# Oscar-W-Chen/gpu-ai-inference-server

Hardware: AMD Instinct MI355X
Metric: images/sec, DenseNet-121 fp32, batch 32 per GPU, device-resident inputs (higher is better)
Workload: dtype f32; 1 GPU; DenseNet-121 fp32 batch=32 per GPU, synthetic 3x224x224 inputs (BASELINE configs[1]); synthetic ONNX graph + seeded random weights (reference model file is not in the mount); global_batch=32, per_gpu_batch=32, parallelism=dp1 (independent batch shards)

## Files before the change

gpu-ai-inference-server_amd/build.py:

```python
from __future__ import annotations

import os
import shutil
import subprocess
import sys
from concurrent.futures import ThreadPoolExecutor

PKG = os.path.dirname(os.path.abspath(__file__))
ROOT = os.path.dirname(PKG)
CSRC = os.path.join(PKG, "csrc")
OBJ = os.path.join(PKG, "lib", "obj")
LIB = os.path.join(PKG, "lib", "libinference_engine.so")
HIPCC = os.environ.get("HIPCC", "/opt/rocm/bin/hipcc")
ARCH = "gfx950"

SOURCES = ["env.cpp", "onnx_reader.cpp", "plan.cpp", "repository.cpp", "config.cpp", "executor.cpp", "bridge.cpp", "bridge_load.cpp", "bridge_run.cpp", "kernels.hip", "kernels_f16.hip", "kernels_ws.hip", "kernels_ws32.hip", "kernels_stem.hip", "kernels_direct.hip", "kernels_f8.hip", "kernels_fused.hip", "kernels_wino.hip", "kernels_x6.hip", "kernels_block.hip", "kernels_ws8.hip", "kernels_dw.hip", "kernels_se.hip", "kernels_grouped.hip", "kernels_resize.hip", "kernels_convt.hip", "kernels_ln.hip", "kernels_attn.hip", "kernels_tokens.hip"]
COMMON = ["-std=c++17", "-O3", "-fPIC", "-Wall", "-Wextra", "-Wno-unused-parameter", "-Wno-unused-result",
          "-I" + os.path.join(ROOT, "include"), "-I" + CSRC]


def _deps(src: str) -> list[str]:
    d = [os.path.join(CSRC, src)]
    for f in os.listdir(CSRC):
        if f.endswith(".h"):
            d.append(os.path.join(CSRC, f))
    for f in os.listdir(os.path.join(ROOT, "include")):
        d.append(os.path.join(ROOT, "include", f))
    return d


def _stale(target: str, deps: list[str]) -> bool:
    if not os.path.exists(target):
        return True
    t = os.path.getmtime(target)
    return any(os.path.getmtime(d) > t for d in deps)


def _compile(src: str, force: bool) -> str:
    obj = os.path.join(OBJ, src + ".o")
    if force or _stale(obj, _deps(src)):
        cmd = [HIPCC, *COMMON, "-c", os.path.join(CSRC, src), "-o", obj]
        if src.endswith(".hip"):
            cmd[1:1] = ["--offload-arch=" + ARCH, "-mllvm", "-amdgpu-mfma-vgpr-form=1"]
        r = subprocess.run(cmd, capture_output=True, text=True)
        if r.returncode != 0:
            raise RuntimeError(f"hipcc failed for {src}:\n{r.stdout}\n{r.stderr}")
        if r.stderr.strip():
            sys.stderr.write(r.stderr)
    return obj


def build_library(force: bool = False) -> str:
    os.makedirs(OBJ, exist_ok=True)
    with ThreadPoolExecutor(max_workers=4) as ex:
        objs = list(ex.map(lambda s: _compile(s, force), SOURCES))
    if force or _stale(LIB, objs):
        cmd = [HIPCC, "--offload-arch=" + ARCH, "-shared", "-fPIC", *objs, "-o", LIB, "-lstdc++fs", "-lpthread",
               "-L/opt/rocm/lib", "-lrccl", "-Wl,-rpath,/opt/rocm/lib"]
        r = subprocess.run(cmd, capture_output=True, text=True)
        if r.returncode != 0:
            raise RuntimeError(f"link failed:\n{r.stdout}\n{r.stderr}")
        for d in (os.path.join(ROOT, "build", "inference_engine"), os.path.join(ROOT, "build", "inference_engine", "lib")):
            os.makedirs(d, exist_ok=True)
            shutil.copy2(LIB, os.path.join(d, "libinference_engine.so"))
    return LIB


def build_harness() -> str:
    src = os.path.join(CSRC, "harness", "replay_binding.c")
    out = os.path.join(PKG, "lib", "replay_binding")
    if _stale(out, [src, LIB, os.path.join(ROOT, "include", "inference_bridge.h")]):
        cmd = ["gcc", "-std=c11", "-O2", "-Wall", "-Wextra", "-I" + os.path.join(ROOT, "include"), src, "-o", out,
               "-L" + os.path.dirname(LIB), "-linference_engine", "-Wl,-rpath," + os.path.dirname(LIB), "-lm"]
        r = subprocess.run(cmd, capture_output=True, text=True)
        if r.returncode != 0:
            raise RuntimeError(f"harness build failed:\n{r.stdout}\n{r.stderr}")
    return out


if __name__ == "__main__":
    print(build_library("--force" in sys.argv))
    if os.path.exists(os.path.join(CSRC, "harness", "replay_binding.c")):
        print(build_harness())
```

gpu-ai-inference-server_amd/csrc/bridge.cpp:

```cpp
#include "bridge_internal.h"

static_assert(sizeof(Shape) == 16, "Shape layout");
static_assert(sizeof(TensorData) == 48 && offsetof(TensorData, data) == 32 && offsetof(TensorData, data_size) == 40, "TensorData layout");
static_assert(sizeof(ModelConfig) == 64 && offsetof(ModelConfig, dynamic_batching) == 56, "ModelConfig layout");
static_assert(sizeof(ModelMetadata) == 72 && offsetof(ModelMetadata, load_time_ns) == 64, "ModelMetadata layout");
static_assert(sizeof(ModelStats) == 32, "ModelStats layout");
static_assert(sizeof(CudaMemoryInfo) == 24, "CudaMemoryInfo layout");

using namespace ie_bridge;

extern "C" {

bool IsCudaAvailable(void) { return ie::HipDeviceCount() > 0; }
int GetDeviceCount(void) { return ie::HipDeviceCount(); }
const char* GetDeviceInfo(int device_id) {
    try { return dup_cstr(ie::HipDeviceInfo(device_id)); } catch (...) { return dup_cstr("Unknown device"); }
}
CudaMemoryInfo GetMemoryInfo(int device_id) {
    CudaMemoryInfo m{0, 0, 0};
    size_t total = 0, fr = 0;
    if (ie::HipMemoryInfo(device_id, &total, &fr)) { m.total = total; m.free = fr; m.used = total - fr; }
    return m;
}

// ... 138 lines not shown
bool ModelUnload(ModelHandle handle, ErrorMessage* error) {
    if (!handle) { set_error(error, "Invalid model handle"); return false; }
    try { handle->model->Unload(); return true; }
    catch (const std::exception& e) { set_error(error, e.what()); return false; }
    catch (...) { set_error(error, "unknown error"); return false; }
}

bool ModelIsLoaded(ModelHandle handle) {
    if (!handle) return false;
    try { return handle->model->loaded.load(); } catch (...) { return false; }
}

bool ModelInfer(ModelHandle handle, const TensorData* inputs, int num_inputs, TensorData* outputs, int num_outputs,
                ErrorMessage* error) {
    if (!handle) { set_error(error, "Invalid model handle"); return false; }
    ModelObj& M = *handle->model;
    if (!M.loaded.load()) { set_error(error, "Model not loaded"); return false; }
    if (!inputs || num_inputs <= 0 || !outputs || num_outputs <= 0) { set_error(error, "Invalid parameters"); return false; }
    try {
        ModelObj::Pending req;
        bool batched = false;
        {
            std::shared_lock<std::shared_mutex> g(M.life);
            if (!M.loaded.load() || M.lanes.empty()) { set_error(error, "Model not loaded"); return false; }
            auto failv = [&](const std::string& msg) { M.SetError(msg); set_error(error, msg); return false; };
            const auto& gin = M.info.inputs;
            if (size_t(num_inputs) != gin.size())
                return failv("Expected " + std::to_string(gin.size()) + " inputs, got " + std::to_string(num_inputs));
            for (int i = 0; i < num_inputs; ++i) {
                const std::string nm = inputs[i].name ? inputs[i].name : "";
                bool known = false;
                for (auto& vi : gin) if (vi.name == nm) known = true;
                if (!known) return failv("Unexpected input name: " + nm);
            }
            req.in_ptr.assign(gin.size(), nullptr);
            req.in_bytes.assign(gin.size(), 0);
            req.in_u8.assign(gin.size(), 0);
            req.shapes.assign(gin.size(), {});
            req.outputs = outputs;
            req.num_outputs = num_outputs;
            std::vector<char> provided(gin.size(), 0);
            for (int i = 0; i < num_inputs && req.err.empty(); ++i) {
                const TensorData& t = inputs[i];
                const std::string nm = t.name ? t.name : "";
                for (size_t k = 0; k < gin.size(); ++k) {
                    if (gin[k].name != nm) continue;
                    if (t.data_type != DATATYPE_FLOAT32 && t.data_type != DATATYPE_UINT8) { req.err = "Unsupported data type for input: " + nm; break; }
                    req.in_u8[k] = t.data_type == DATATYPE_UINT8 ? 1 : 0;
                    provided[k] = 1;
                    req.shapes[k].clear();
                    if (t.shape.dims && t.shape.num_dims > 0) req.shapes[k].assign(t.shape.dims, t.shape.dims + t.shape.num_dims);
                    req.in_ptr[k] = (t.data && t.data_size > 0) ? t.data : nullptr;
                    req.in_bytes[k] = req.in_ptr[k] ? t.data_size : 0;
                }
            }
            for (size_t k = 0; k < gin.size() && req.err.empty(); ++k)
                if (!provided[k]) req.err = "Required input tensor not provided: " + gin[k].name;
            batched = req.err.empty() && M.batchable && M.max_batch > 1;
            if (batched) {
                req.rows = req.shapes[0].empty() ? 0 : req.shapes[0][0];
                for (size_t k = 0; k < gin.size(); ++k)
                    if (req.shapes[k].size() != gin[k].dims.size() || req.shapes[k][0] != req.rows) batched = false;
                if (req.rows <= 0 || req.rows >= M.max_batch) batched = false;
                for (char u : req.in_u8) if (u) batched = false;
            }
            if (!batched) req.rows = 0;
        }
        const auto t0 = std::chrono::steady_clock::now();
        const RoctxRange range("ModelInfer:" + M.name);
        if (req.err.empty()) {
            if (batched) M.RunBatched(req);
            else { std::vector<ModelObj::Pending*> one{&req}; M.Execute(one); }
        }
        const int64_t ns = std::chrono::duration_cast<std::chrono::nanoseconds>(std::chrono::steady_clock::now() - t0).count();
        M.inference_count.fetch_add(1);
        M.total_ns.fetch_add(ns);
        M.last_ns.store(ns);
        if (!req.ok) {
            M.SetError(req.err);
            set_error(error, req.err);
            return false;
        }
        return true;
    } catch (const std::exception& e) { set_error(error, e.what()); return false; }
    catch (...) { set_error(error, "unknown error"); return false; }
}

}

namespace {
std::string describe_runtime(ModelObj& M, bool json, bool checksums = false) {
    double ms, fl, by;
    int64_t fw, im;
    { std::lock_guard<std::mutex> g(M.acct_mu); ms = M.acct_ms; fl = M.acct_flops; by = M.acct_bytes; fw = M.acct_forwards; im = M.acct_images; }
    const bool up = M.loaded.load() && !M.lanes.empty();
    const ie::Precision prec = up ? M.lanes[0]->precision() : ie::Precision::F32;
    const char* pname = prec == ie::Precision::F16 ? "fp16" : (prec == ie::Precision::F8 ? "fp8" : "fp32");
    const double mfma_peak = prec == ie::Precision::F16 ? 2500.0 : (prec == ie::Precision::F8 ? 5000.0 : 157.3);
    const double tflops = ms > 0 ? fl / (ms * 1e-3) / 1e12 : 0, gbs = ms > 0 ? by / (ms * 1e-3) / 1e9 : 0;
    int max_in_flight;
    { std::lock_guard<std::mutex> g(M.pool.mu); max_in_flight = M.pool.max_in_flight; }
    std::ostringstream o;
    o.precision(6);
    if (!json) {
        o << "mi355x-engine precision=" << pname << (up && !M.lanes.empty() && M.lanes[0]->fp32_split() ? "+bf16x6" : "") << " lanes=" << M.lanes.size() << " shards=" << (up ? M.num_shards : 0) << " forwards=" << fw
          << " images=" << im << " device_ms_avg=" << (fw ? ms / double(fw) : 0.0) << " achieved_tflops=" << tflops << " frac_mfma_peak=" << tflops / mfma_peak
          << " algorithmic_gbs=" << gbs << " frac_hbm_peak=" << gbs / 8000.0;
        return o.str();
    }
    o << "{\"loaded\":" << (up ? "true" : "false") << ",\"precision\":\"" << pname << "\",\"fp32_split\":" << (up && !M.lanes.empty() && M.lanes[0]->fp32_split() ? "true" : "false")
      << ",\"lanes\":" << M.lanes.size() << ",\"shards\":" << (up ? M.num_shards : 0)
      << ",\"lane_devices\":[";
    for (size_t i = 0; i < M.lanes.size(); ++i) o << (i ? "," : "") << M.lanes[i]->device();
    o << "],\"lane_shares_weights_with\":[";
    for (size_t i = 0; i < M.lanes.size(); ++i) {
        size_t first = i;
        for (size_t k = 0; k < i; ++k) if (M.lanes[k]->shared_weights() == M.lanes[i]->shared_weights()) { first = k; break; }
        o << (i ? "," : "") << first;
    }
    o << "],\"max_in_flight\":" << max_in_flight << ",\"rccl\":{\"used\":" << (M.rccl.used ? "true" : "false") << ",\"ranks\":" << M.rccl.ranks
      << ",\"weight_owners\":" << M.rccl.owners << ",\"bytes\":" << M.rccl.bytes << ",\"init_ms\":" << M.rccl.init_ms << ",\"broadcast_ms\":" << M.rccl.bcast_ms
      << "},\"forwards\":" << fw << ",\"images\":" << im << ",\"device_ms_total\":" << ms << ",\"achieved_tflops\":" << tflops
      << ",\"mfma_peak_tflops\":" << mfma_peak << ",\"algorithmic_gbs\":" << gbs << ",\"hbm_peak_gbs\":8000";
    if (up) {
        o << ",\"pipelined_calls\":[";
        for (size_t i = 0; i < M.lanes.size(); ++i) o << (i ? "," : "") << M.lanes[i]->pipelined_calls();
        o << "],\"last_chunks\":" << M.lanes[0]->last_chunks() << ",\"last_head_steps\":" << M.lanes[0]->last_head_steps();
    }
    if (up && prec == ie::Precision::F8) {
        const auto& W = *M.lanes[0]->shared_weights();
        o << ",\"f8_ready\":" << (W.f8_ready ? "true" : "false") << ",\"f8_act_scales\":[";
        o.precision(9);
        for (size_t i = 0; i < W.act_scale.size(); ++i) o << (i ? "," : "") << W.act_scale[i];
        o << "]";
        o.precision(6);
    }
    if (up && checksums) {
        o << ",\"weight_checksums\":[";
        for (size_t i = 0; i < M.lanes.size(); ++i) {
            std::vector<char> host(M.lanes[i]->weight_bytes());
            try { M.lanes[i]->CopySync(host.data(), M.lanes[i]->weights(), host.size(), hipMemcpyDeviceToHost, "hipMemcpy(weight checksum)"); }
            catch (const std::exception&) { (void)hipGetLastError(); host.clear(); }
            o << (i ? "," : "") << "\"" << std::hex << fnv1a64(host.data(), host.size()) << std::dec << "\"";
        }
        o << "],\"mirror_checksums\":[";
        for (size_t i = 0; i < M.lanes.size(); ++i) {
            o << (i ? "," : "") << "{";
            bool first = true;
            for (const auto& kv : M.lanes[i]->MirrorChecksums()) {
                o << (first ? "" : ",") << "\"" << kv.first << "\":\"" << std::hex << kv.second << std::dec << "\"";
                first = false;
            }
            o << "}";
        }
        o << "]";
    }
    o << "}";
    return o.str();
}

struct Lane0 {
    ModelObj& M;
    std::shared_lock<std::shared_mutex> lk;
    bool ok = false;
    explicit Lane0(ModelObj& m) : M(m), lk(m.life) {
        if (M.loaded.load() && !M.lanes.empty()) { M.pool.AcquireOne(0); ok = true; }
    }
    ~Lane0() { if (ok) M.pool.Release(0, 1); }
    ie::DeviceModel* dev() const { return ok ? M.lanes[0].get() : nullptr; }
};
}

extern "C" {

ModelMetadata* ModelGetMetadata(ModelHandle handle) {
    if (!handle) return nullptr;
    try {
        ModelObj& M = *handle->model;
        std::shared_lock<std::shared_mutex> g(M.life);
        auto* md = static_cast<ModelMetadata*>(std::calloc(1, sizeof(ModelMetadata)));
        md->name = dup_cstr(M.name);
        md->version = dup_cstr(M.version);
        md->model_type = M.type;
        md->description = dup_cstr(describe_runtime(M, false));
        md->load_time_ns = M.load_time_ns;
        auto fill = [](const std::vector<std::string>& v, const char*** arr, int* n) {
            *n = int(v.size());
            *arr = nullptr;
            if (v.empty()) return;
            *arr = static_cast<const char**>(std::malloc(sizeof(char*) * v.size()));
            for (size_t i = 0; i < v.size(); ++i) (*arr)[i] = dup_cstr(v[i]);
        };
        fill(M.input_names, &md->inputs, &md->num_inputs);
        fill(M.output_names, &md->outputs, &md->num_outputs);
        return md;
    } catch (...) { return nullptr; }
}

void ModelFreeMetadata(ModelMetadata* md) {
    if (!md) return;
    std::free(const_cast<char*>(md->name));
    std::free(const_cast<char*>(md->version));
    std::free(const_cast<char*>(md->description));
    if (md->inputs) { for (int i = 0; i < md->num_inputs; ++i) std::free(const_cast<char*>(md->inputs[i])); std::free(md->inputs); }
    if (md->outputs) { for (int i = 0; i < md->num_outputs; ++i) std::free(const_cast<char*>(md->outputs[i])); std::free(md->outputs); }
    std::free(md);
}

ModelStats* ModelGetStats(ModelHandle handle) {
    if (!handle) return nullptr;
    try {
        ModelObj& M = *handle->model;
        auto* s = static_cast<ModelStats*>(std::calloc(1, sizeof(ModelStats)));
        s->inference_count = M.inference_count.load();
        s->total_inference_time_ns = M.total_ns.load();
        s->last_inference_time_ns = M.last_ns.load();
        s->memory_usage_bytes = M.memory_usage_bytes.load();
        return s;
    } catch (...) { return nullptr; }
}

void ModelFreeStats(ModelStats* stats) { std::free(stats); }

void FreeErrorMessage(ErrorMessage error) { std::free(error); }

ModelHandle GetModelHandle(InferenceManagerHandle handle, const char* model_name, const char* , ErrorMessage* error) {
    if (!handle || !model_name) { set_error(error, "Invalid handle or model name"); return nullptr; }
    try {
        std::lock_guard<std::mutex> g(handle->mu);
        auto it = handle->models.find(model_name);
        if (it == handle->models.end()) { set_error(error, "Model not found in loaded models"); return nullptr; }
        return new Model_t{it->second};
    } catch (const std::exception& e) { set_error(error, e.what()); return nullptr; }
    catch (...) { set_error(error, "unknown error"); return nullptr; }
}

static void json_vi(std::ostringstream& o, const std::vector<ie::OnnxValueInfo>& v) {
    o << "[";
    for (size_t i = 0; i < v.size(); ++i) {
        o << (i ? "," : "") << "{\"name\":\"" << v[i].name << "\",\"elem_type\":" << v[i].elem_type << ",\"dims\":[";
        for (size_t k = 0; k < v[i].dims.size(); ++k) o << (k ? "," : "") << v[i].dims[k];
        o << "]}";
    }
    o << "]";
}

char* EngineDescribeModel(const char* path, int batch, ErrorMessage* error) {
    if (!path) { set_error(error, "Invalid parameters"); return nullptr; }
    try {
        std::string file = path;
        std::error_code ec;
        if (std::filesystem::is_directory(file, ec)) file += "/model.onnx";
        if (!std::filesystem::exists(file, ec)) { set_error(error, "ONNX model file not found: " + file); return nullptr; }
        ie::OnnxModel m = ie::LoadOnnxFile(file);
        ie::ModelInfo info = ie::DescribeModel(m);
        std::ostringstream o;
        o << "{\"ir_version\":" << m.ir_version << ",\"opset\":" << m.opset << ",\"producer\":\"" << m.producer
          << "\",\"num_nodes\":" << m.nodes.size() << ",\"num_initializers\":" << m.initializers.size()
          << ",\"memory_usage_bytes\":" << info.memory_usage_bytes << ",\"inputs\":";
        json_vi(o, info.inputs);
        o << ",\"outputs\":";
        json_vi(o, info.outputs);
        if (std::filesystem::is_directory(path, ec)) {
            const ie::EngineConfig c = ie::LoadEngineConfig(path);
            auto esc = [](const std::string& t) { std::string r; for (char ch : t) { if (ch == '"' || ch == '\\') r += '\\'; if (static_cast<unsigned char>(ch) >= 0x20) r += ch; } return r; };
            auto io = [&](const std::vector<ie::IoConfig>& v) {
                o << "[";
                for (size_t i = 0; i < v.size(); ++i) {
                    o << (i ? "," : "") << "{\"name\":\"" << esc(v[i].name) << "\",\"data_type\":\"" << esc(v[i].data_type) << "\",\"label_filename\":\""
                      << esc(v[i].label_filename) << "\",\"dims\":[";
                    for (size_t k = 0; k < v[i].dims.size(); ++k) o << (k ? "," : "") << v[i].dims[k];
                    o << "],\"shape\":[";
                    for (size_t k = 0; k < v[i].shape.size(); ++k) o << (k ? "," : "") << v[i].shape[k];
                    o << "]}";
                }
                o << "]";
            };
            o << ",\"config\":{\"present\":" << (c.present ? "true" : "false") << ",\"name\":\"" << esc(c.name) << "\",\"version\":\"" << esc(c.version)
              << "\",\"platform\":\"" << esc(c.platform) << "\",\"precision\":\"" << esc(c.precision) << "\",\"gpus\":" << c.gpus
              << ",\"uint8_scale\":" << c.uint8_scale << ",\"uint8_bias\":" << c.uint8_bias << ",\"dynamic_batching\":" << (c.dynamic_batching ? "true" : "false")
              << ",\"max_batch_size\":" << c.max_batch_size << ",\"batch_window_us\":" << c.batch_window_us << ",\"instance_count\":" << c.instance_count
              << ",\"fp32_split\":" << (c.fp32_split ? "true" : "false") << ",\"tune_batches\":[";
            for (size_t k = 0; k < c.tune_batches.size(); ++k) o << (k ? "," : "") << c.tune_batches[k];
            o << "],\"inputs\":";
            io(c.inputs);
            o << ",\"outputs\":";
            io(c.outputs);
            o << "}";
        }
        if (batch > 0) {
            std::vector<std::vector<int64_t>> shapes;
            for (auto& vi : info.inputs) {
                std::vector<int64_t> s = vi.dims;
                for (size_t k = 0; k < s.size(); ++k) if (s[k] <= 0) s[k] = (k == 0 ? batch : 1);
                shapes.push_back(s);
            }
            ie::Precision prec = ie::Precision::F32;
            const ie::Env env = ie::Env::Read();
            if (const char* e = env.get("IE_PRECISION")) {
                std::string w = e;
                if (w == "fp16" || w == "f16" || w == "half") prec = ie::Precision::F16;
                else if (w == "fp8" || w == "f8" || w == "e4m3") prec = ie::Precision::F8;
            }
            o << ",\"plan\":" << ie::PlanToJson(ie::BuildPlan(m, shapes, prec));
        }
        o << "}";
        return dup_cstr(o.str());
    } catch (const std::exception& e) { set_error(error, e.what()); return nullptr; }
    catch (...) { set_error(error, "unknown error"); return nullptr; }
}

float* EnginePlanWeights(const char* path, int batch, size_t* count, ErrorMessage* error) {
    if (!path || !count || batch <= 0) { set_error(error, "Invalid parameters"); return nullptr; }
    try {
        std::string file = path;
        std::error_code ec;
        if (std::filesystem::is_directory(file, ec)) file += "/model.onnx";
        if (!std::filesystem::exists(file, ec)) { set_error(error, "ONNX model file not found: " + file); return nullptr; }
        ie::OnnxModel m = ie::LoadOnnxFile(file);
        std::vector<std::vector<int64_t>> shapes;
        for (auto& vi : m.inputs) {
            std::vector<int64_t> s = vi.dims;
            for (size_t k = 0; k < s.size(); ++k) if (s[k] <= 0) s[k] = (k == 0 ? batch : 1);
            shapes.push_back(s);
        }
        ie::Plan p = ie::BuildPlan(m, shapes, ie::Precision::F32);
        float* out = static_cast<float*>(std::malloc(std::max<size_t>(p.weights.size(), 1) * sizeof(float)));
        if (!out) { set_error(error, "out of memory"); return nullptr; }
        std::memcpy(out, p.weights.data(), p.weights.size() * sizeof(float));
        *count = p.weights.size();
        return out;
    } catch (const std::exception& e) { set_error(error, e.what()); return nullptr; }
    catch (...) { set_error(error, "unknown error"); return nullptr; }
}

bool EnginePrepare(ModelHandle handle, const Shape* input_shapes, int num_inputs, void** d_inputs, void** d_outputs,
                   int num_outputs, ErrorMessage* error) {
    if (!handle) { set_error(error, "Invalid model handle"); return false; }
    try {
        ModelObj& M = *handle->model;
        Lane0 L0(M);
        if (!L0.dev()) { set_error(error, "Model not loaded"); return false; }
        if (!input_shapes || num_inputs <= 0) { set_error(error, "Invalid parameters"); return false; }
        std::vector<std::vector<int64_t>> shapes;
        for (int i = 0; i < num_inputs; ++i) {
            if (!input_shapes[i].dims || input_shapes[i].num_dims <= 0) { set_error(error, "Invalid parameters"); return false; }
            shapes.emplace_back(input_shapes[i].dims, input_shapes[i].dims + input_shapes[i].num_dims);
        }
        ie::PlanInstance& pi = L0.dev()->Prepare(shapes, true);
        for (int i = 0; d_inputs && i < num_inputs && size_t(i) < pi.plan.inputs.size(); ++i)
            d_inputs[i] = pi.buffers[size_t(pi.plan.inputs[size_t(i)].view.buf)];
        for (int i = 0; d_outputs && i < num_outputs && size_t(i) < pi.plan.outputs.size(); ++i)
            d_outputs[i] = pi.buffers[size_t(pi.plan.outputs[size_t(i)].view.buf)];
        return true;
    } catch (const std::exception& e) { set_error(error, e.what()); return false; }
    catch (...) { set_error(error, "unknown error"); return false; }
}

bool EngineRunPrepared(ModelHandle handle, int iters, int sync, ErrorMessage* error) {
    if (!handle) { set_error(error, "Invalid model handle"); return false; }
    try {
        ModelObj& M = *handle->model;
        Lane0 L0(M);
        if (!L0.dev() || !L0.dev()->current()) { set_error(error, "Model not prepared"); return false; }
        const int cap = L0.dev()->max_inflight_replays();
        for (int i = 0; i < iters; ++i) {
            L0.dev()->Enqueue(*L0.dev()->current());
            if (cap > 0 && (i + 1) % cap == 0) L0.dev()->Synchronize();
        }
        if (sync) L0.dev()->Synchronize();
        return true;
    } catch (const std::exception& e) { set_error(error, e.what()); return false; }
    catch (...) { set_error(error, "unknown error"); return false; }
}

bool EngineSynchronize(ModelHandle handle, ErrorMessage* error) {
    if (!handle) { set_error(error, "Invalid model handle"); return false; }
    try {
        ModelObj& M = *handle->model;
        Lane0 L0(M);
        if (!L0.dev()) { set_error(error, "Model not loaded"); return false; }
        L0.dev()->Synchronize();
        return true;
    } catch (const std::exception& e) { set_error(error, e.what()); return false; }
    catch (...) { set_error(error, "unknown error"); return false; }
}

void* EngineGetStream(ModelHandle handle) {
    if (!handle) return nullptr;
    try {
        ModelObj& M = *handle->model;
        std::shared_lock<std::shared_mutex> g(M.life);
        return M.lanes.empty() ? nullptr : static_cast<void*>(M.lanes[0]->stream());
    } catch (...) { return nullptr; }
}

char* EngineProfile(ModelHandle handle, int iters, ErrorMessage* error) {
    if (!handle) { set_error(error, "Invalid model handle"); return nullptr; }
    try {
        ModelObj& M = *handle->model;
        Lane0 L0(M);
        if (!L0.dev() || !L0.dev()->current()) { set_error(error, "Model not prepared"); return nullptr; }
        auto t = L0.dev()->Profile(*L0.dev()->current(), iters > 0 ? iters : 1);
        std::ostringstream o;
        o.precision(9);
        o << "[";
        for (size_t i = 0; i < t.size(); ++i) {
            std::string nm;
            for (char c : t[i].name) if (c != '"' && c != '\\') nm += c;
            o << (i ? "," : "") << "{\"name\":\"" << nm << "\",\"kernel\":\"" << t[i].kernel << "\",\"ms\":" << t[i].ms
              << ",\"flops\":" << t[i].flops << ",\"bytes\":" << t[i].bytes << "}";
        }
        o << "]";
        return dup_cstr(o.str());
    } catch (const std::exception& e) { set_error(error, e.what()); return nullptr; }
    catch (...) { set_error(error, "unknown error"); return nullptr; }
}

bool EngineGetWeightBlob(ModelHandle handle, void** d_ptr, size_t* bytes, ErrorMessage* error) {
    if (!handle || !d_ptr || !bytes) { set_error(error, "Invalid parameters"); return false; }
    try {
        ModelObj& M = *handle->model;
        Lane0 L0(M);
        if (!L0.dev()) { set_error(error, "Model not loaded"); return false; }
        *d_ptr = L0.dev()->weights();
        *bytes = L0.dev()->weight_bytes();
        return true;
    } catch (const std::exception& e) { set_error(error, e.what()); return false; }
    catch (...) { set_error(error, "unknown error"); return false; }
}

bool EngineWeightsUpdated(ModelHandle handle, ErrorMessage* error) {
    if (!handle) { set_error(error, "Invalid parameters"); return false; }
    try {
        ModelObj& M = *handle->model;
        std::shared_lock<std::shared_mutex> g(M.life);
        if (!M.loaded.load() || M.lanes.empty()) { set_error(error, "Model not loaded"); return false; }
        const int n = int(M.lanes.size());
        M.pool.AcquireRange(n);
        try {
            for (auto& l : M.lanes) l->Synchronize();
            M.lanes[0]->WeightsArrived();
            M.BroadcastWeights();
        } catch (...) { M.pool.Release(0, n); throw; }
        M.pool.Release(0, n);
        return true;
    } catch (const std::exception& e) { set_error(error, e.what()); return false; }
    catch (...) { set_error(error, "unknown error"); return false; }
}

int EngineGetPrecision(ModelHandle handle) {
    if (!handle) return -1;
    ModelObj& M = *handle->model;
    std::shared_lock<std::shared_mutex> g(M.life);
    if (!M.loaded.load() || M.lanes.empty()) return -1;
    return int(M.lanes[0]->precision());
}

bool EngineMemcpy(ModelHandle handle, void* dst, const void* src, size_t bytes, int kind, ErrorMessage* error) {
    if (!handle || !dst || !src || kind < 1 || kind > 3) { set_error(error, "Invalid parameters"); return false; }
    try {
        ModelObj& M = *handle->model;
        Lane0 L0(M);
        if (!L0.dev()) { set_error(error, "Model not loaded"); return false; }
        L0.dev()->Synchronize();
        hipMemcpyKind k = kind == 1 ? hipMemcpyHostToDevice : (kind == 2 ? hipMemcpyDeviceToHost : hipMemcpyDeviceToDevice);
        hipError_t e = hipMemcpy(dst, src, bytes, k);
        if (e != hipSuccess) { set_error(error, std::string("HIP error in hipMemcpy: ") + hipGetErrorString(e)); return false; }
        return true;
    } catch (const std::exception& e) { set_error(error, e.what()); return false; }
    catch (...) { set_error(error, "unknown error"); return false; }
}

double EngineMfmaPeak(int nacc, int blocks_per_cu, int iters) {
    if (ie::HipDeviceCount() <= 0) return -1.0;
    try { return ie::MfmaPeakTflops(nacc, blocks_per_cu, iters); } catch (...) { return -1.0; }
}

bool EngineGetBatcherStats(ModelHandle handle, int64_t* device_batches, int64_t* coalesced_requests, int* max_batch) {
    if (!handle) return false;
    ModelObj& M = *handle->model;
    if (device_batches) *device_batches = M.device_batches.load();
    if (coalesced_requests) *coalesced_requests = M.coalesced_requests.load();
    if (max_batch) *max_batch = (M.batchable && M.max_batch > 1) ? M.max_batch : 0;
    return true;
}

bool EngineGetShardStats(ModelHandle handle, int* num_shards, int64_t* sharded_calls) {
    if (!handle) return false;
    ModelObj& M = *handle->model;
    std::shared_lock<std::shared_mutex> g(M.life);
    if (num_shards) *num_shards = M.lanes.empty() ? 0 : M.num_shards;
    if (sharded_calls) *sharded_calls = M.shard_calls.load();
    return true;
}

char* EngineGetRuntimeInfo(ModelHandle handle, int with_checksums, ErrorMessage* error) {
    if (!handle) { set_error(error, "Invalid model handle"); return nullptr; }
    try {
        ModelObj& M = *handle->model;
        std::shared_lock<std::shared_mutex> g(M.life);
        if (with_checksums && M.loaded.load() && !M.lanes.empty()) {
            M.pool.AcquireRange(int(M.lanes.size()));
            std::string r;
            try { r = describe_runtime(M, true, true); } catch (...) { M.pool.Release(0, int(M.lanes.size())); throw; }
            M.pool.Release(0, int(M.lanes.size()));
            return dup_cstr(r);
        }
        return dup_cstr(describe_runtime(M, true, false));
    } catch (const std::exception& e) { set_error(error, e.what()); return nullptr; }
    catch (...) { set_error(error, "unknown error"); return nullptr; }
}

bool EngineE4m3RoundTrip(const float* src, float* dst, unsigned char* codes, size_t n, float scale, ErrorMessage* error) {
    if (!src || !dst || !(scale > 0.f)) { set_error(error, "Invalid parameters"); return false; }
    if (ie::HipDeviceCount() <= 0) { set_error(error, "No HIP device available"); return false; }
    if (n == 0) return true;
    float *ds = nullptr, *dd = nullptr;
    unsigned char* dc = nullptr;
    bool ok = hipMalloc(reinterpret_cast<void**>(&ds), n * 4) == hipSuccess && hipMalloc(reinterpret_cast<void**>(&dd), n * 4) == hipSuccess &&
              hipMalloc(reinterpret_cast<void**>(&dc), n) == hipSuccess && hipMemcpy(ds, src, n * 4, hipMemcpyHostToDevice) == hipSuccess &&
              ie::LaunchE4m3RoundTrip(ds, dd, dc, scale, int64_t(n), nullptr) == hipSuccess && hipDeviceSynchronize() == hipSuccess &&
              hipMemcpy(dst, dd, n * 4, hipMemcpyDeviceToHost) == hipSuccess && (!codes || hipMemcpy(codes, dc, n, hipMemcpyDeviceToHost) == hipSuccess);
    if (ds) (void)hipFree(ds);
    if (dd) (void)hipFree(dd);
    if (dc) (void)hipFree(dc);
    if (!ok) { (void)hipGetLastError(); set_error(error, "HIP error in EngineE4m3RoundTrip"); }
    return ok;
}

bool EngineVectorAdd(const float* a, const float* b, float* result, size_t n, ErrorMessage* error) {
    if (!a || !b || !result) { set_error(error, "Invalid parameters"); return false; }
    if (ie::HipDeviceCount() <= 0) { set_error(error, "No HIP device available"); return false; }
    float *da = nullptr, *db = nullptr, *dr = nullptr;
    bool ok = false;
    std::string msg;
    auto chk = [&](hipError_t e, const char* what) {
        if (e != hipSuccess) { msg = std::string("HIP error in ") + what + ": " + hipGetErrorString(e); return false; }
        return true;
    };
    const size_t bytes = n * sizeof(float);
    if (n == 0) return true;
    if (chk(hipMalloc(reinterpret_cast<void**>(&da), bytes), "hipMalloc") && chk(hipMalloc(reinterpret_cast<void**>(&db), bytes), "hipMalloc") &&
        chk(hipMalloc(reinterpret_cast<void**>(&dr), bytes), "hipMalloc") && chk(hipMemcpy(da, a, bytes, hipMemcpyHostToDevice), "hipMemcpy") &&
        chk(hipMemcpy(db, b, bytes, hipMemcpyHostToDevice), "hipMemcpy") && chk(ie::LaunchVectorAdd(da, db, dr, int64_t(n), nullptr), "vector_add") &&
        chk(hipDeviceSynchronize(), "hipDeviceSynchronize") && chk(hipMemcpy(result, dr, bytes, hipMemcpyDeviceToHost), "hipMemcpy"))
        ok = true;
    if (da) (void)hipFree(da);
    if (db) (void)hipFree(db);
    if (dr) (void)hipFree(dr);
    if (!ok) set_error(error, msg);
    return ok;
}

}
```

gpu-ai-inference-server_amd/csrc/env.cpp:

```cpp
#include "env.h"

#include <atomic>
#include <cstdlib>

namespace ie {

namespace {
const char* const kNames[] = {
    "IE_PRECISION",
    "IE_FP32_SPLIT",
    "IE_DEVICE_ID",
    "IE_GPUS",
    "IE_SHARD_DEVICES",
    "IE_SHARD_PRIVATE_WEIGHTS",
    "IE_INSTANCES",
    "IE_DYNAMIC_BATCH",
    "IE_BATCH_WINDOW_US",
    "IE_VERSION_ORDER",
    "IE_ROCTX",
    "IE_NO_POOL_SWAP", "IE_NO_DENSE_FUSE", "IE_NO_DENSE_BLOCK", "IE_DENSE_BAND", "IE_NO_DUAL_F8", "IE_NO_STEM_POOL", "IE_FUSE_MAX_M", "IE_FUSE_PB",
    "IE_NO_SE_FUSE",
    "IE_GROUPED_CONV",
    "IE_FORCE_ALGO", "IE_FORCE_TILE", "IE_FORCE_SPLITK",
    "IE_AUTOTUNE", "IE_TUNE_CACHE", "IE_TUNE_BATCHES", "IE_TUNE_ON_DEMAND", "IE_TUNE_HOT", "IE_TUNE_LOG",
    "IE_DISABLE_GRAPH", "IE_SPLITK_IN_LAUNCH", "IE_PIPELINE_CHUNKS", "IE_PIPELINE_HEAD", "IE_MAX_PLANS", "IE_NO_FRAG_WEIGHTS",
    "IE_F8_CALIB_BATCH", "IE_F8_MARGIN",
    "IE_MAX_INFLIGHT_REPLAYS",
    "IE_DEBUG_ABLATE", "IE_AS_PAD", "IE_NO_PERSISTENT",
    nullptr};

LaunchKnobs g_knobs;
std::atomic<bool> g_knobs_set{false};
}

Env Env::Read() {
    Env e;
    for (const char* const* n = kNames; *n; ++n)
        if (const char* v = std::getenv(*n)) e.kv_[*n] = v;
    return e;
}

int Env::integer(const char* name, int dflt) const {
    const char* v = get(name);
    return v ? std::atoi(v) : dflt;
}

const char* const* Env::Names() { return kNames; }

const LaunchKnobs& Knobs() { return g_knobs; }

void SetLaunchKnobs(const Env& env) {
    LaunchKnobs k;
    k.debug_ablate = env.integer("IE_DEBUG_ABLATE", 0);
    const int pad = env.integer("IE_AS_PAD", 8);
    k.as_pad = (pad >= 4 && pad <= 68 && pad % 4 == 0) ? pad : 8;
    k.no_persistent = env.flag("IE_NO_PERSISTENT");
    g_knobs = k;
    g_knobs_set.store(true);
}

}
```

gpu-ai-inference-server_amd/csrc/executor.cpp:

```cpp
#include "executor.h"
#include "env.h"

#include <algorithm>
#include <cstdint>
#include <cstdlib>
#include <cmath>
#include <cstdio>
#include <cstring>
#include <fstream>
#include <unistd.h>
#include <sstream>
#include <stdexcept>

#include "igemm_tiles.h"
#include "kernels.h"

namespace ie {
namespace {

void check(hipError_t e, const char* what) {
    if (e != hipSuccess) throw std::runtime_error(std::string("HIP error in ") + what + ": " + hipGetErrorString(e));
}

TensorArg make_arg(const PlanInstance& pi, const View& v) {
    TensorArg t;
    char* base = reinterpret_cast<char*>(pi.buffers.at(size_t(v.buf)));
    t.n = int(v.n); t.h = int(v.h); t.w = int(v.w); t.c = int(v.c);
    t.f16 = v.f16 ? 1 : 0;
    t.f8 = v.f8 ? 1 : 0;
    const int64_t esize = v.esize();
    if (v.nchw) {
        t.sw = 1; t.sh = v.w; t.sc = v.h * v.w; t.sn = v.c * v.h * v.w;
        t.p = reinterpret_cast<float*>(base + pi.batch_off * t.sn * esize);
    } else {
        t.sc = 1; t.sw = v.pitch; t.sh = v.w * v.pitch; t.sn = v.h * v.w * v.pitch;
        t.p = reinterpret_cast<float*>(base + (v.c_off + pi.batch_off * t.sn) * esize);
    }
    return t;
}

TensorArg view_strides(const View& v) {
    TensorArg t;
    t.n = int(v.n); t.h = int(v.h); t.w = int(v.w); t.c = int(v.c);
    t.f16 = v.f16 ? 1 : 0;
    t.f8 = v.f8 ? 1 : 0;
    if (v.nchw) { t.sw = 1; t.sh = v.w; t.sc = v.h * v.w; t.sn = v.c * v.h * v.w; }
    else { t.sc = 1; t.sw = v.pitch; t.sh = v.w * v.pitch; t.sn = v.h * v.w * v.pitch; }
    return t;
}

ResizeArgs MakeResizeArgs(const PlanInstance& pi, const Step& s) {
    ResizeArgs a;
    a.in = make_arg(pi, s.in);
    a.out = make_arg(pi, s.out);
    a.mode = int(s.rs_mode);
    a.coord = int(s.rs_coord);
    a.nearest = int(s.rs_nearest);
    a.scale_h = s.rs_scale_h;
    a.scale_w = s.rs_scale_w;
    return a;
}

LnArgs MakeLnArgs(const PlanInstance& pi, const Step& s, const float* weights) {
    LnArgs a;
    a.in = make_arg(pi, s.in);
    a.out = make_arg(pi, s.out);
    a.gamma = s.w_off >= 0 ? weights + s.w_off : nullptr;
    a.beta = s.bias_off >= 0 ? weights + s.bias_off : nullptr;
    a.eps = s.ln_eps;
    return a;
}

AttnArgs MakeAttnArgs(const PlanInstance& pi, const Step& s) {
    AttnArgs a;
    a.in = make_arg(pi, s.in);
    a.out = make_arg(pi, s.out);
    a.heads = s.heads;
    a.head_dim = s.head_dim;
    a.scale = s.attn_scale;
    return a;
}

constexpr size_t kPinnedBytes = size_t(4) << 20;
constexpr int64_t kTuneWorkspaceFloats = int64_t(16) << 20;
constexpr int kNumCounters = 1 << 16;
constexpr int kMaxChunks = 8;
constexpr const char* kTuneFileTag = "# ie-tune-v2";

std::once_flag g_kernels_once;
hipError_t g_kernels_err = hipSuccess;

}

int HipDeviceCount() {
    int n = 0;
    if (hipGetDeviceCount(&n) != hipSuccess) { (void)hipGetLastError(); return 0; }
    return n;
}

std::string HipDeviceInfo(int device_id) {
    hipDeviceProp_t p;
    if (hipGetDeviceProperties(&p, device_id) != hipSuccess) { (void)hipGetLastError(); return "Unknown device"; }
    return "Device " + std::to_string(device_id) + ": " + p.name + " (Compute Capability " + std::to_string(p.major) + "." +
           std::to_string(p.minor) + ")";
}

bool HipMemoryInfo(int device_id, size_t* total, size_t* free_b) {
    int prev = 0;
    if (hipGetDevice(&prev) != hipSuccess) { (void)hipGetLastError(); return false; }
    if (hipSetDevice(device_id) != hipSuccess) { (void)hipGetLastError(); return false; }
    bool ok = hipMemGetInfo(free_b, total) == hipSuccess;
    if (!ok) (void)hipGetLastError();
    (void)hipSetDevice(prev);
    return ok;
}

DeviceWeights::~DeviceWeights() {
    (void)hipSetDevice(device);
    if (d_weights) (void)hipFree(d_weights);
    if (d_weights16) (void)hipFree(d_weights16);
    if (d_weights16_frag) (void)hipFree(d_weights16_frag);
    if (d_weights_frag) (void)hipFree(d_weights_frag);
    if (d_weights8) (void)hipFree(d_weights8);
    if (d_f8_aux) (void)hipFree(d_f8_aux);
    if (d_weights_wino) (void)hipFree(d_weights_wino);
    if (d_weights_x6) (void)hipFree(d_weights_x6);
    if (d_weights_wino_x6) (void)hipFree(d_weights_wino_x6);
}

namespace {

std::string tune_file_header() {
    std::ostringstream o;
    o << kTuneFileTag << ' ' << kNumIgemmTiles << ' ' << kNumConvRasterTiles << ' ' << kNumConvWs32Tiles << ' ' << kNumConvWs16Tiles << ' ' << kNumConvWs3Tiles << ' '
      << kNumConvDirectTiles << ' ' << kNumConvWinoTiles << ' ' << kNumConvX6Tiles << ' ' << kNumConvWs8Tiles << ' ' << kNumConvWs38Tiles << ' ' << kNumConvDenseFusedTiles;
    return o.str();
}

constexpr int kLnTuneCode = 1000;
bool ln_tune_code(int t) { return t >= kLnTuneCode && t < kLnTuneCode + kNumLnTiles; }
struct TuneFamily { int base; ConvAlgo algo; int tiles; };
constexpr TuneFamily kTuneFamilies[] = {
    {0, ConvAlgo::IgemmVec, kNumIgemmTiles},          {100, ConvAlgo::Raster3x3, kNumConvRasterTiles},
    {200, ConvAlgo::Ws1x1, std::max(kNumConvWs16Tiles, kNumConvWs32Tiles)},
    {300, ConvAlgo::Ws3x3, kNumConvWs3Tiles},         {400, ConvAlgo::Direct, kNumConvDirectTiles},
    {500, ConvAlgo::Wino3x3, kNumConvWinoTiles},      {600, ConvAlgo::X6, kNumConvX6Tiles},
    {700, ConvAlgo::Depthwise, kNumConvDwTiles},      {800, ConvAlgo::Grouped, kNumConvGroupedTiles},
    {900, ConvAlgo::Transposed, kNumConvtTiles},
};

const TuneFamily& tune_family(int code) {
    const TuneFamily* f = &kTuneFamilies[0];
    for (const auto& g : kTuneFamilies) if (code >= g.base) f = &g;
    return *f;
}

int tune_code(ConvAlgo algo, int tile) {
    for (const auto& g : kTuneFamilies) if (g.base != 0 && g.algo == algo) return g.base + tile;
    return tile;
}

bool tune_code_valid(int t) {
    return (t >= 0 && t - tune_family(t).base < tune_family(t).tiles) || ln_tune_code(t) || (t >= kWs8Code && t < kWs8Code + kNumConvWs8Tiles) ||
           (t >= kWs38Code && t < kWs38Code + kNumConvWs38Tiles);
}

void load_tune_file(const std::string& path, std::map<std::vector<int64_t>, std::pair<int, int>>& cache) {
    std::ifstream f(path);
    std::string line;
    if (!f || !std::getline(f, line) || line != tune_file_header()) return;
    while (std::getline(f, line)) {
        std::istringstream is(line);
        std::vector<int64_t> key;
        std::string tok;
        bool ok = true;
        while (is >> tok && tok != ":") {
            char* endp = nullptr;
            const long long v = std::strtoll(tok.c_str(), &endp, 10);
            if (!endp || *endp) { ok = false; break; }
            key.push_back(v);
        }
        int t = -1, sp = 0;
        if (ok && (is >> t >> sp) && tune_code_valid(t) && sp >= 1 && sp <= 64 &&
            key.size() >= 6)
            cache[key] = {t, sp};
    }
}

}

DeviceModel::DeviceModel(std::shared_ptr<const OnnxModel> model, int device_id, const DeviceModelOptions& opt)
    : model_(std::move(model)), device_(device_id), precision_(opt.precision) {
    env_ = Env::Read();
    SetLaunchKnobs(env_);
    max_inflight_replays_ = std::max(0, env_.integer("IE_MAX_INFLIGHT_REPLAYS", 0));
    int n = HipDeviceCount();
    if (n <= 0) throw std::runtime_error("No HIP device available: the MI355X engine has no CPU fallback");
    if (device_id < 0 || device_id >= n) throw std::runtime_error("Invalid device id " + std::to_string(device_id));
    check(hipSetDevice(device_), "hipSetDevice");
    std::call_once(g_kernels_once, [] {
        g_kernels_err = InitKernels();
        if (g_kernels_err == hipSuccess) g_kernels_err = InitKernelsF16();
        if (g_kernels_err == hipSuccess) g_kernels_err = InitKernelsWs();
        if (g_kernels_err == hipSuccess) g_kernels_err = InitKernelsWs32();
        if (g_kernels_err == hipSuccess) g_kernels_err = InitKernelsWs3();
        if (g_kernels_err == hipSuccess) g_kernels_err = InitKernelsStem();
        if (g_kernels_err == hipSuccess) g_kernels_err = InitKernelsDirect();
        if (g_kernels_err == hipSuccess) g_kernels_err = InitKernelsF8();
        if (g_kernels_err == hipSuccess) g_kernels_err = InitKernelsFused();
        if (g_kernels_err == hipSuccess) g_kernels_err = InitKernelsWino();
        if (g_kernels_err == hipSuccess) g_kernels_err = InitKernelsX6();
        if (g_kernels_err == hipSuccess) g_kernels_err = InitKernelsBlock();
        if (g_kernels_err == hipSuccess) g_kernels_err = InitKernelsWs8();
        if (g_kernels_err == hipSuccess) g_kernels_err = InitKernelsAttn();
    });
    check(g_kernels_err, "InitKernels");
    fp32_split_ = opt.fp32_split && opt.precision == Precision::F32;
    if (const char* e = env_.get("IE_FP32_SPLIT")) fp32_split_ = std::atoi(e) != 0 && opt.precision == Precision::F32;
    if (opt.share) {
        if (opt.share->device != device_) throw std::runtime_error("internal error: shared weights live on another device");
        w_ = opt.share;
    } else {
        w_ = std::make_shared<DeviceWeights>();
        w_->device = device_;
        w_->uploaded = false;
        owns_weights_ = true;
        std::string path = opt.tune_cache_path;
        if (const char* tc = env_.get("IE_TUNE_CACHE")) path = (tc[0] == 0 || (tc[0] == '0' && tc[1] == 0)) ? std::string() : std::string(tc);
        if (fp32_split_ && !path.empty()) path += ".x6";
        w_->tune_cache_path = path;
        if (!path.empty()) load_tune_file(path, w_->tune_cache);
    }
    upload_weights_ = opt.upload_weights;
    check(hipStreamCreateWithFlags(&stream_, hipStreamNonBlocking), "hipStreamCreate");
    check(hipStreamCreateWithFlags(&copy_stream_, hipStreamNonBlocking), "hipStreamCreate");
    h2d_events_.resize(kMaxChunks, nullptr);
    for (auto& e : h2d_events_) check(hipEventCreateWithFlags(&e, hipEventDisableTiming), "hipEventCreate");
    check(hipEventCreate(&t0_event_), "hipEventCreate");
    check(hipEventCreate(&t1_event_), "hipEventCreate");
    const char* ng = env_.get("IE_DISABLE_GRAPH");
    use_graph_ = !(ng && ng[0] == '1');
    const char* at = env_.get("IE_AUTOTUNE");
    const char* tp = env_.get("IE_SPLITK_IN_LAUNCH");
    two_pass_splitk_ = !(tp && tp[0] == '1');
    autotune_ = !(at && at[0] == '0') && !env_.get("IE_FORCE_TILE") && !env_.get("IE_FORCE_SPLITK") && !env_.get("IE_FORCE_ALGO");
    if (const char* od = env_.get("IE_TUNE_ON_DEMAND")) tune_on_demand_ = od[0] == '1';
    if (const char* pc = env_.get("IE_PIPELINE_CHUNKS")) pipeline_chunks_ = std::max(0, std::min(kMaxChunks, std::atoi(pc)));
    if (const char* ph = env_.get("IE_PIPELINE_HEAD")) pipeline_head_ = std::max(0, std::atoi(ph));
    if (const char* mp = env_.get("IE_MAX_PLANS")) max_plans_ = size_t(std::max(1, std::atoi(mp)));
    pinned_bytes_ = kPinnedBytes;
    check(hipHostMalloc(&pinned_, pinned_bytes_, hipHostMallocDefault), "hipHostMalloc");
}

DeviceModel::~DeviceModel() {
    (void)hipSetDevice(device_);
    if (stream_) (void)hipStreamSynchronize(stream_);
    if (copy_stream_) (void)hipStreamSynchronize(copy_stream_);
    for (auto& kv : plans_) FreeInstance(*kv.second);
    for (auto e : h2d_events_) if (e) (void)hipEventDestroy(e);
    if (t0_event_) (void)hipEventDestroy(t0_event_);
    if (t1_event_) (void)hipEventDestroy(t1_event_);
    if (pinned_) (void)hipHostFree(pinned_);
    if (copy_stream_) (void)hipStreamDestroy(copy_stream_);
    if (stream_) (void)hipStreamDestroy(stream_);
}

void DeviceModel::FreeInstance(PlanInstance& pi) {
    for (auto& ch : pi.chunks) FreeInstance(*ch);
    pi.chunks.clear();
    if (pi.graph_exec) (void)hipGraphExecDestroy(pi.graph_exec);
    if (pi.tail_exec) (void)hipGraphExecDestroy(pi.tail_exec);
    pi.graph_exec = nullptr;
    pi.tail_exec = nullptr;
    for (size_t i = 0; i < pi.buffers.size(); ++i)
        if (pi.buffers[i] && pi.owned[i]) (void)hipFree(pi.buffers[i]);
    pi.buffers.clear();
    if (pi.workspace && pi.owns_workspace) (void)hipFree(pi.workspace);
    if (pi.counters && pi.owns_workspace) (void)hipFree(pi.counters);
    pi.workspace = nullptr;
    pi.counters = nullptr;
    for (void* p : pi.u8_stage) if (p) (void)hipFree(p);
    pi.u8_stage.clear();
}

void DeviceModel::CopySync(void* dst, const void* src, size_t bytes, hipMemcpyKind kind, const char* what) {
    if (bytes == 0) return;
    check(hipMemcpyAsync(dst, src, bytes, kind, stream_), what);
    check(hipStreamSynchronize(stream_), what);
}

void DeviceModel::ZeroSync(void* dst, size_t bytes, const char* what) {
    if (bytes == 0) return;
    check(hipMemsetAsync(dst, 0, bytes, stream_), what);
    check(hipStreamSynchronize(stream_), what);
}

void DeviceModel::BuildInstance(PlanInstance& pi, const std::vector<std::vector<int64_t>>& shapes) {
    pi.plan = BuildPlan(*model_, shapes, precision_);
    {
        std::lock_guard<std::mutex> g(w_->tune_mu);
        if (!w_->d_weights) {
            w_->weight_floats = pi.plan.weights.size();
            check(hipMalloc(reinterpret_cast<void**>(&w_->d_weights), std::max<size_t>(w_->weight_floats, 4) * sizeof(float)), "hipMalloc(weights)");
            w_->device_bytes += w_->weight_floats * sizeof(float);
            if (upload_weights_) {
                CopySync(w_->d_weights, pi.plan.weights.data(), w_->weight_floats * sizeof(float), hipMemcpyHostToDevice, "hipMemcpy(weights)");
                w_->uploaded = true;
            } else {
                ZeroSync(w_->d_weights, w_->weight_floats * sizeof(float), "hipMemset(weights)");
            }
            if (precision_ == Precision::F16 || precision_ == Precision::F8) {
                check(hipMalloc(&w_->d_weights16, std::max<size_t>(w_->weight_floats, 8) * 2), "hipMalloc(weights16)");
                w_->device_bytes += w_->weight_floats * 2;
                if (precision_ == Precision::F16) {
                    auto add16 = [&](const Step& st) {
                        if (st.kind != StepKind::Conv || IsGroupConv(st.algo) || st.w_off < 0 || st.in.nchw || st.sh != 1 || st.sw != 1) return;
                        const bool one = st.kh == 1 && st.kw == 1 && st.out.c == 128 && st.in.c % 32 == 0;
                        const bool three = st.kh == 3 && st.kw == 3 && st.out.c == 32 && st.in.c == 128;
                        if (one || three) w_->frag16_regions.push_back({st.w_off, int(st.out.c), int(st.kh * st.kw * st.in.c)});
                    };
                    for (const Step& st : pi.plan.steps) {
                        if (st.parts.empty()) add16(st);
                        else for (const Step& q : st.parts) add16(q);
                    }
                    if (!w_->frag16_regions.empty()) {
                        check(hipMalloc(&w_->d_weights16_frag, std::max<size_t>(w_->weight_floats, 8) * 2), "hipMalloc(weights16_frag)");
                        w_->device_bytes += w_->weight_floats * 2;
                    }
                }
                if (precision_ == Precision::F8) {
                    check(hipMalloc(&w_->d_weights8, std::max<size_t>(w_->weight_floats, 16)), "hipMalloc(weights8)");
                    ZeroSync(w_->d_weights8, std::max<size_t>(w_->weight_floats, 16), "hipMemset(weights8)");
                    w_->device_bytes += w_->weight_floats;
                    int64_t aux = 0;
                    auto add8 = [&](const Step& st, int i) {
                        if (st.kind != StepKind::Conv || st.algo != ConvAlgo::IgemmF8) return;
                        w_->f8_convs.push_back({i, st.w_off, int(st.out.c), int(st.kh * st.kw * st.in.c), st.in_src, aux});
                        aux += 2 * ((st.out.c + 3) / 4 * 4);
                    };
                    for (size_t i = 0; i < pi.plan.steps.size(); ++i) {
                        const Step& st = pi.plan.steps[i];
                        if (st.parts.empty()) add8(st, int(i));
                        else for (const Step& q : st.parts) add8(q, int(i));
                    }
                    check(hipMalloc(reinterpret_cast<void**>(&w_->d_f8_aux), size_t(std::max<int64_t>(aux, 4)) * sizeof(float)), "hipMalloc(f8 aux)");
                    w_->f8_aux_floats = size_t(aux);
                    w_->device_bytes += size_t(aux) * sizeof(float);
                    w_->act_scale.assign(pi.plan.steps.size(), 0.f);
                }
            } else if (const char* nf = env_.get("IE_NO_FRAG_WEIGHTS"); !(nf && std::atoi(nf) != 0)) {
                auto add_region = [&](const Step& st) {
                    if (st.kind == StepKind::Conv && !IsGroupConv(st.algo) && st.w_off >= 0 && st.out.c % 16 == 0 && st.in.c % 16 == 0 && st.kh * st.kw <= 49)
                        w_->frag_regions.push_back({st.w_off, int(st.out.c), st.kh * st.kw, int(st.in.c)});
                };
                for (const Step& st : pi.plan.steps) {
                    if (st.parts.empty()) add_region(st);
                    else for (const Step& q : st.parts) add_region(q);
                }
                if (!w_->frag_regions.empty()) {
                    check(hipMalloc(reinterpret_cast<void**>(&w_->d_weights_frag), w_->weight_floats * sizeof(float)), "hipMalloc(weights_frag)");
                    w_->device_bytes += w_->weight_floats * sizeof(float);
                }
                int64_t utot = 0;
                auto add_wino = [&](const Step& st) {
                    if (st.kind == StepKind::Conv && !IsGroupConv(st.algo) && st.w_off >= 0 && st.kh == 3 && st.kw == 3 && st.sh == 1 && st.sw == 1 && st.pt == 1 && st.pl == 1 &&
                        st.out.c == 32 && st.in.c % 32 == 0 && !st.in.nchw) {
                        w_->wino_regions.push_back({st.w_off, utot, 32, int(st.in.c)});
                        utot += int64_t(16) * 32 * st.in.c;
                    }
                };
                for (const Step& st : pi.plan.steps) {
                    if (st.parts.empty()) add_wino(st);
                    else for (const Step& q : st.parts) add_wino(q);
                }
                if (utot > 0) {
                    check(hipMalloc(reinterpret_cast<void**>(&w_->d_weights_wino), size_t(utot) * sizeof(float)), "hipMalloc(weights_wino)");
                    w_->wino_floats = size_t(utot);
                    w_->device_bytes += size_t(utot) * sizeof(float);
                }
                const bool split = fp32_split_;
                w_->fp32_split = split;
                if (split) {
                    int64_t xtot = 0;
                    auto add_x6 = [&](const Step& st) {
                        if (st.kind == StepKind::Conv && !IsGroupConv(st.algo) && st.w_off >= 0 && st.kh == 1 && st.kw == 1 && st.sh == 1 && st.sw == 1 && st.out.c % 128 == 0 && st.in.c % 32 == 0 &&
                            !st.in.nchw) {
                            w_->x6_regions.push_back({st.w_off, xtot, int(st.out.c), int(st.in.c)});
                            xtot += int64_t(3) * st.out.c * st.in.c * 2;
                        }
                    };
                    for (const Step& st : pi.plan.steps) {
                        if (st.parts.empty()) add_x6(st);
                        else for (const Step& q : st.parts) add_x6(q);
                    }
                    if (xtot > 0) {
                        check(hipMalloc(&w_->d_weights_x6, size_t(xtot)), "hipMalloc(weights_x6)");
                        w_->x6_bytes = size_t(xtot);
                        w_->device_bytes += size_t(xtot);
                    }
                    if (utot > 0) {
                        check(hipMalloc(&w_->d_weights_wino_x6, size_t(utot) * 6), "hipMalloc(weights_wino_x6)");
                        w_->device_bytes += size_t(utot) * 6;
                    }
                }
            }
            if (w_->uploaded) WeightsArrived();
        } else if (pi.plan.weights.size() != w_->weight_floats) {
            throw std::runtime_error("internal error: weight blob layout depends on the input shape");
        }
    }
    std::vector<float>().swap(pi.plan.weights);
    AllocInstance(pi);
}

void DeviceModel::AllocInstance(PlanInstance& pi) {
    pi.buffers.assign(pi.plan.buffer_floats.size(), nullptr);
    pi.owned.assign(pi.plan.buffer_floats.size(), 0);
    for (size_t i = 0; i < pi.plan.buffer_floats.size(); ++i) {
        float* p = nullptr;
        const int dt = pi.plan.buffer_f16[i];
        size_t bytes = size_t(std::max<int64_t>(pi.plan.buffer_floats[i], 16)) * (dt == 2 ? 1 : (dt == 1 ? 2 : 4));
        check(hipMalloc(reinterpret_cast<void**>(&p), bytes), "hipMalloc(activations)");
        check(hipMemsetAsync(p, 0, bytes, stream_), "hipMemset(activations)");
        device_bytes_ += bytes;
        pi.buffers[i] = p;
        pi.owned[i] = 1;
    }
    pi.workspace_floats = std::max<int64_t>(2 * pi.plan.workspace_floats, kTuneWorkspaceFloats);
    size_t bytes = size_t(pi.workspace_floats) * sizeof(float);
    check(hipMalloc(reinterpret_cast<void**>(&pi.workspace), bytes), "hipMalloc(workspace)");
    pi.owns_workspace = true;
    device_bytes_ += bytes;
    if (!two_pass_splitk_) {
        check(hipMalloc(reinterpret_cast<void**>(&pi.counters), kNumCounters * sizeof(int)), "hipMalloc(counters)");
        check(hipMemsetAsync(pi.counters, 0, kNumCounters * sizeof(int), stream_), "hipMemset(counters)");
    }
}

void DeviceModel::Capture(PlanInstance& pi, size_t first, size_t last, hipGraphExec_t* exec) {
    hipGraph_t graph = nullptr;
    check(hipStreamBeginCapture(stream_, hipStreamCaptureModeThreadLocal), "hipStreamBeginCapture");
    try {
        RunSteps(pi, first, last, nullptr);
    } catch (...) {
        (void)hipStreamEndCapture(stream_, &graph);
        if (graph) (void)hipGraphDestroy(graph);
        throw;
    }
    check(hipStreamEndCapture(stream_, &graph), "hipStreamEndCapture");
    hipError_t e = hipGraphInstantiate(exec, graph, nullptr, nullptr, 0);
    (void)hipGraphDestroy(graph);
    check(e, "hipGraphInstantiate");
}

PlanInstance& DeviceModel::Prepare(const std::vector<std::vector<int64_t>>& shapes, bool allow_tune) {
    std::vector<int64_t> key;
    for (auto& s : shapes) { key.push_back(int64_t(s.size())); key.insert(key.end(), s.begin(), s.end()); }
    auto touch = [&](const std::vector<int64_t>& k) {
        for (size_t i = 0; i < lru_.size(); ++i) if (lru_[i] == k) { lru_.erase(lru_.begin() + long(i)); break; }
        lru_.push_back(k);
    };
    check(hipSetDevice(device_), "hipSetDevice");
    auto it = plans_.find(key);
    if (it != plans_.end()) {
        touch(key);
        current_ = it->second.get();
        if (allow_tune) EnsurePipeline(*current_, true);
        return *current_;
    }
    while (plans_.size() >= max_plans_ && !lru_.empty()) {
        check(hipStreamSynchronize(stream_), "hipStreamSynchronize");
        auto old = plans_.find(lru_.front());
        if (old != plans_.end()) {
            if (current_ == old->second.get()) current_ = nullptr;
            FreeInstance(*old->second);
            plans_.erase(old);
        }
        lru_.erase(lru_.begin());
    }

    auto pi = std::make_unique<PlanInstance>();
    try {
        BuildInstance(*pi, shapes);
        check(hipStreamSynchronize(stream_), "hipStreamSynchronize");
        if (autotune_) Autotune(*pi, pi->plan.steps.size(), allow_tune || tune_on_demand_);
        if (use_graph_ && !(precision_ == Precision::F8 && !w_->f8_ready)) {
            pi->captured_gen = w_->f8_gen.load();
            Capture(*pi, 0, pi->plan.steps.size(), &pi->graph_exec);
            pi->graph_ready = true;
        }
        if (allow_tune) EnsurePipeline(*pi, true);
    } catch (...) {
        FreeInstance(*pi);
        throw;
    }
    current_ = pi.get();
    plans_[key] = std::move(pi);
    touch(key);
    return *current_;
}

void DeviceModel::WeightsArrived(const std::vector<float>* adopt_act_scales) {
    check(hipSetDevice(device_), "hipSetDevice");
    w_->uploaded = true;
    if (w_->d_weights_x6)
        for (const auto& xr : w_->x6_regions)
            check(LaunchSplitWeightsX6(w_->d_weights + xr.w_off, static_cast<char*>(w_->d_weights_x6) + xr.byte_off, xr.cout, xr.k, stream_), "split_weights_x6");
    if (w_->d_weights_wino) {
        check(hipSetDevice(device_), "hipSetDevice");
        for (const auto& wr : w_->wino_regions) {
            check(LaunchWinogradWeights(w_->d_weights + wr.w_off, w_->d_weights_wino + wr.u_off, wr.cout, wr.cin, stream_), "winograd_weights");
            if (w_->d_weights_wino_x6)
                check(LaunchWinogradWeightsX6(w_->d_weights + wr.w_off, static_cast<char*>(w_->d_weights_wino_x6) + wr.u_off * 6, wr.cout, wr.cin, stream_), "winograd_weights_x6");
        }
        check(hipStreamSynchronize(stream_), "hipStreamSynchronize");
    }
    if (!w_->d_weights16 && !w_->d_weights_frag) return;
    check(hipSetDevice(device_), "hipSetDevice");
    w_->f8_ready = false;
    if (w_->d_weights16) check(LaunchConvertF32ToF16(w_->d_weights, w_->d_weights16, int64_t(w_->weight_floats), stream_), "convert_f32_f16");
    if (w_->d_weights16_frag)
        for (const auto& fr : w_->frag16_regions)
            check(LaunchPermuteWeightsFrag16(static_cast<const char*>(w_->d_weights16) + fr.w_off * 2, static_cast<char*>(w_->d_weights16_frag) + fr.w_off * 2, fr.rows, fr.k,
                                             stream_), "permute_weights_frag16");
    if (w_->d_weights_frag)
        for (const DeviceWeights::FragRegion& fr : w_->frag_regions)
            check(LaunchPermuteWeightsFrag(w_->d_weights + fr.w_off, w_->d_weights_frag + fr.w_off, fr.cout, fr.kk, fr.cin, stream_), "permute_weights_frag");
    check(hipStreamSynchronize(stream_), "hipStreamSynchronize");
    if (precision_ == Precision::F8) PrepareF8(adopt_act_scales);
}

std::vector<std::pair<std::string, uint64_t>> DeviceModel::MirrorChecksums() {
    check(hipSetDevice(device_), "hipSetDevice");
    check(hipStreamSynchronize(stream_), "hipStreamSynchronize");
    const DeviceWeights& W = *w_;
    std::vector<std::pair<std::string, uint64_t>> out;
    std::vector<char> host;
    auto fnv = [](uint64_t h, const char* p, size_t n) { for (size_t i = 0; i < n; ++i) { h ^= uint8_t(p[i]); h *= 0x100000001B3ull; } return h; };
    auto pull = [&](const void* dev, size_t bytes) {
        host.resize(bytes);
        if (bytes) CopySync(host.data(), dev, bytes, hipMemcpyDeviceToHost, "hipMemcpy(mirror)");
    };
    constexpr uint64_t kBasis = 0xCBF29CE484222325ull;
    if (W.d_weights16) { pull(W.d_weights16, W.weight_floats * 2); out.push_back({"half", fnv(kBasis, host.data(), host.size())}); }
    if (W.d_weights16_frag) {
        uint64_t h = kBasis;
        for (const auto& fr : W.frag16_regions) { pull(static_cast<const char*>(W.d_weights16_frag) + fr.w_off * 2, size_t(fr.rows) * size_t(fr.k) * 2); h = fnv(h, host.data(), host.size()); }
        out.push_back({"half_fragment_major", h});
    }
    if (W.d_weights_frag) {
        uint64_t h = kBasis;
        for (const auto& fr : W.frag_regions) {
            pull(W.d_weights_frag + fr.w_off, size_t(fr.cout) * size_t(fr.kk) * size_t(fr.cin) * sizeof(float));
            h = fnv(h, host.data(), host.size());
        }
        out.push_back({"fragment_major", h});
    }
    if (W.d_weights_wino) { pull(W.d_weights_wino, W.wino_floats * sizeof(float)); out.push_back({"winograd_u", fnv(kBasis, host.data(), host.size())}); }
    if (W.d_weights_x6) { pull(W.d_weights_x6, W.x6_bytes); out.push_back({"bf16x6", fnv(kBasis, host.data(), host.size())}); }
    if (W.d_weights8) {
        uint64_t h = kBasis;
        for (const auto& fc : W.f8_convs) { pull(static_cast<const char*>(W.d_weights8) + fc.w_off, size_t(fc.cout) * size_t(fc.k)); h = fnv(h, host.data(), host.size()); }
        out.push_back({"e4m3", h});
        pull(W.d_f8_aux, W.f8_aux_floats * sizeof(float));
        out.push_back({"e4m3_scales", fnv(kBasis, host.data(), host.size())});
        out.push_back({"act_scales", fnv(kBasis, reinterpret_cast<const char*>(W.act_scale.data()), W.act_scale.size() * sizeof(float))});
    }
    return out;
}

namespace {

uint64_t rng_mix(uint64_t z) {
    z ^= z >> 30; z *= 0xBF58476D1CE4E5B9ull;
    z ^= z >> 27; z *= 0x94D049BB133111EBull;
    z ^= z >> 31;
    return z;
}
uint64_t rng_key(uint64_t seed, const std::string& stream) {
    uint64_t h = 0xCBF29CE484222325ull;
    for (unsigned char b : stream) { h ^= b; h *= 0x100000001B3ull; }
    return rng_mix(seed * 0x9E3779B97F4A7C15ull + h);
}
float rng_uniform(uint64_t key, uint64_t i) {
    return float(double(rng_mix(key + (i + 1) * 0x9E3779B97F4A7C15ull) >> 40) * (1.0 / 16777216.0));
}
std::vector<float> synthetic_images(int64_t b, int64_t c, int64_t h, int64_t w, const std::string& stream) {
    std::vector<float> x(size_t(b * c * h * w));
    const uint64_t kf = rng_key(20250704, stream), kc = rng_key(20250704, stream + "/coarse");
    if (h < 8 || w < 8) {
        for (size_t i = 0; i < x.size(); ++i) x[i] = rng_uniform(kf, i);
        return x;
    }
    const int64_t cell = std::max<int64_t>(h / 7, 1), gh = (h + cell - 1) / cell, gw = (w + cell - 1) / cell;
    for (int64_t n = 0; n < b; ++n)
        for (int64_t ch = 0; ch < c; ++ch)
            for (int64_t y = 0; y < h; ++y)
                for (int64_t xx = 0; xx < w; ++xx) {
                    const uint64_t i = uint64_t(((n * c + ch) * h + y) * w + xx);
                    const uint64_t j = uint64_t(((n * c + ch) * gh + y / cell) * gw + xx / cell);
                    x[i] = 0.6f * rng_uniform(kc, j) + 0.4f * rng_uniform(kf, i);
                }
    return x;
}

}

void DeviceModel::PrepareF8(const std::vector<float>* adopt) {
    DeviceWeights& W = *w_;
    if (W.f8_ready || !W.uploaded) return;
    if (adopt && adopt->size() != W.act_scale.size()) adopt = nullptr;
    check(hipSetDevice(device_), "hipSetDevice");
    for (const auto& fc : W.f8_convs)
        check(LaunchQuantizeRowsE4m3(W.d_weights + fc.w_off, static_cast<char*>(W.d_weights8) + fc.w_off, W.d_f8_aux + fc.aux_off, fc.cout, fc.k, stream_),
              "quantize_rows_e4m3");
    if (adopt) W.act_scale = *adopt;
    else {
    int64_t nc = 8;
    if (const char* e = env_.get("IE_F8_CALIB_BATCH")) nc = std::max(1, std::min(64, std::atoi(e)));
    float margin = 2.0f;
    if (const char* e = env_.get("IE_F8_MARGIN")) margin = std::max(1.0f, float(std::atof(e)));
    std::vector<std::vector<int64_t>> shapes;
    for (const auto& vi : model_->inputs) {
        std::vector<int64_t> sh = vi.dims;
        for (size_t k = 0; k < sh.size(); ++k) if (sh[k] <= 0) sh[k] = (k == 0 ? nc : 1);
        shapes.push_back(sh);
    }
    PlanInstance cal;
    cal.plan = BuildPlan(*model_, shapes, Precision::F16, true);
    if (cal.plan.steps.size() != W.act_scale.size()) throw std::runtime_error("fp8 calibration: the fp16 plan of the graph has a different step list");
    std::vector<float>().swap(cal.plan.weights);
    float* d_amax = nullptr;
    try {
        AllocInstance(cal);
        check(hipMalloc(reinterpret_cast<void**>(&d_amax), cal.plan.steps.size() * sizeof(float)), "hipMalloc(amax)");
        check(hipMemsetAsync(d_amax, 0, cal.plan.steps.size() * sizeof(float), stream_), "hipMemset(amax)");
        for (size_t i = 0; i < cal.plan.inputs.size(); ++i) {
            const View& v = cal.plan.inputs[i].view;
            const std::vector<float> x = synthetic_images(v.n, v.c, v.h, v.w, "calibration/" + cal.plan.inputs[i].name);
            check(hipMemcpyAsync(cal.buffers[size_t(v.buf)], x.data(), x.size() * sizeof(float), hipMemcpyHostToDevice, stream_), "hipMemcpy(calibration input)");
            check(hipStreamSynchronize(stream_), "hipStreamSynchronize");
        }
        for (size_t i = 0; i < cal.plan.steps.size(); ++i) {
            LaunchStep(cal, cal.plan.steps[i], stream_);
            check(LaunchAbsMax(make_arg(cal, cal.plan.steps[i].out), d_amax + i, stream_), "absmax");
        }
        std::vector<float> amax(cal.plan.steps.size());
        check(hipMemcpyAsync(amax.data(), d_amax, amax.size() * sizeof(float), hipMemcpyDeviceToHost, stream_), "hipMemcpy(amax)");
        check(hipStreamSynchronize(stream_), "hipStreamSynchronize");
        for (size_t i = 0; i < amax.size(); ++i) {
            const Step& st = cal.plan.steps[i];
            float sc = (amax[i] > 0.f ? amax[i] : 1.f) * margin / 448.0f;
            if (st.kind == StepKind::Pool && st.pool_max && st.in_src >= 0 && W.act_scale[size_t(st.in_src)] > 0.f) sc = W.act_scale[size_t(st.in_src)];
            W.act_scale[i] = sc;
        }
    } catch (...) {
        if (d_amax) (void)hipFree(d_amax);
        FreeInstance(cal);
        throw;
    }
    (void)hipFree(d_amax);
    FreeInstance(cal);
    }
    for (const auto& fc : W.f8_convs) {
        if (fc.in_src < 0) throw std::runtime_error("fp8 precision: a conv reads a tensor whose producer is unknown");
        const int64_t half = (fc.cout + 3) / 4 * 4;
        check(LaunchScaleVector(W.d_f8_aux + fc.aux_off, W.d_f8_aux + fc.aux_off + half, W.act_scale[size_t(fc.in_src)], fc.cout, stream_), "scale_vector");
    }
    check(hipStreamSynchronize(stream_), "hipStreamSynchronize");
    W.f8_gen.fetch_add(1);
    W.f8_ready = true;
}

void DeviceModel::EnsurePipeline(PlanInstance& pi, bool allow_tune) {
    if (pi.pipeline_tried) return;
    pi.pipeline_tried = true;
    if (pipeline_chunks_ < 2 || pi.plan.inputs.empty() || pi.plan.steps.size() < 4) return;
    const int64_t B = pi.plan.inputs[0].dims.empty() ? 0 : pi.plan.inputs[0].dims[0];
    for (auto& d : pi.plan.inputs) if (d.dims.empty() || d.dims[0] != B || d.view.n != B) return;
    for (auto& d : pi.plan.outputs) if (d.dims.empty() || d.dims[0] != B) return;
    int C = pipeline_chunks_;
    while (C > 1 && (B % C != 0 || B / C < 4)) C /= 2;
    if (C < 2) return;
    const int64_t Bc = B / C;
    std::vector<std::vector<int64_t>> sub_shapes;
    for (auto& d : pi.plan.inputs) { sub_shapes.push_back(d.dims); sub_shapes.back()[0] = Bc; }
    Plan sub;
    try {
        sub = BuildPlan(*model_, sub_shapes, precision_);
    } catch (const std::exception&) {
        return;
    }
    const Plan& full = pi.plan;
    if (sub.steps.size() != full.steps.size() || sub.weights.size() != w_->weight_floats || 2 * sub.workspace_floats > pi.workspace_floats) return;
    auto same_view = [&](const View& a, const View& b) {
        return a.buf == b.buf && a.c == b.c && a.h == b.h && a.w == b.w && a.c_off == b.c_off && a.pitch == b.pitch && a.nchw == b.nchw && a.f16 == b.f16 &&
               a.n * C == b.n;
    };
    auto image_stride = [](const View& v) { return v.nchw ? v.c * v.h * v.w : v.h * v.w * v.pitch; };
    size_t head = 0;
    {
        double in_bytes = 0;
        for (auto& d : full.inputs) in_bytes += double(d.view.numel()) * 4.0;
        const double t_h2d = in_bytes * double(C - 1) / double(C) / 40e9;
        const double peak = precision_ == Precision::F32 ? 0.45 * 157.3e12 : 0.3 * 2.5e15;
        double total = 0;
        std::vector<double> est(full.steps.size());
        for (size_t i = 0; i < full.steps.size(); ++i) { est[i] = std::max(full.steps[i].flops / peak, full.steps[i].bytes / 2.5e12) + 4e-6; total += est[i]; }
        const double want = std::min(t_h2d, 0.6 * total);
        double acc = 0;
        while (head < full.steps.size() - 1 && acc < want) acc += est[head++];
        if (pipeline_head_ >= 0) head = std::min<size_t>(size_t(pipeline_head_), full.steps.size() - 1);
    }
    auto valid = [&](size_t h) {
        for (size_t i = 0; i < h; ++i) {
            const Step &a = sub.steps[i], &b = full.steps[i];
            if (a.kind != b.kind || !same_view(a.in, b.in) || !same_view(a.out, b.out) || a.has_in2 != b.has_in2 || (a.has_in2 && !same_view(a.in2, b.in2)) ||
                a.w_off != b.w_off || a.bias_off != b.bias_off || a.pre_scale_off != b.pre_scale_off || a.pre_shift_off != b.pre_shift_off ||
                a.parts.size() != b.parts.size())
                return false;
            for (size_t q = 0; q < a.parts.size(); ++q)
                if (!same_view(a.parts[q].in, b.parts[q].in) || !same_view(a.parts[q].out, b.parts[q].out) || a.parts[q].w_off != b.parts[q].w_off) return false;
        }
        std::map<int, int64_t> head_stride;
        auto note = [&](const View& v) {
            auto f = head_stride.find(v.buf);
            if (f == head_stride.end()) head_stride[v.buf] = image_stride(v);
            else if (f->second != image_stride(v)) f->second = -1;
        };
        for (size_t i = 0; i < h; ++i) {
            note(full.steps[i].in); note(full.steps[i].out);
            if (full.steps[i].has_in2) note(full.steps[i].in2);
            for (const Step& q : full.steps[i].parts) { note(q.in); note(q.out); }
        }
        std::vector<const View*> tail_written;
        auto covered = [&](const View& v) {
            int64_t pos = v.c_off;
            const int64_t end = v.c_off + v.c;
            bool progress = true;
            while (pos < end && progress) {
                progress = false;
                for (const View* w : tail_written)
                    if (w->buf == v.buf && w->nchw == v.nchw && image_stride(*w) == image_stride(v) && w->c_off <= pos && w->c_off + w->c > pos) {
                        pos = w->c_off + w->c;
                        progress = true;
                    }
            }
            return pos >= end;
        };
        for (size_t i = h; i < full.steps.size(); ++i) {
            for (const View* v : {&full.steps[i].in, full.steps[i].has_in2 ? &full.steps[i].in2 : nullptr}) {
                if (!v || covered(*v)) continue;
                auto f = head_stride.find(v->buf);
                if (f != head_stride.end() && (f->second == -1 || f->second != image_stride(*v))) return false;
            }
            for (const Step& q : full.steps[i].parts) {
                if (!covered(q.in)) {
                    auto f = head_stride.find(q.in.buf);
                    if (f != head_stride.end() && (f->second == -1 || f->second != image_stride(q.in))) return false;
                }
                tail_written.push_back(&q.out);
            }
            tail_written.push_back(&full.steps[i].out);
        }
        return true;
    };
    while (head > 0 && !valid(head)) --head;
    if (head == 0) return;
    std::vector<float>().swap(sub.weights);
    for (int c = 0; c < C; ++c) {
        auto ch = std::make_unique<PlanInstance>();
        ch->plan = sub;
        ch->buffers = pi.buffers;
        ch->owned.assign(pi.buffers.size(), 0);
        ch->workspace = pi.workspace;
        ch->workspace_floats = pi.workspace_floats;
        ch->counters = pi.counters;
        ch->batch_off = int64_t(c) * Bc;
        pi.chunks.push_back(std::move(ch));
    }
    try {
        if (autotune_) {
            Autotune(*pi.chunks[0], head, allow_tune || tune_on_demand_);
            for (int c = 1; c < C; ++c)
                for (size_t i = 0; i < head; ++i) {
                    Step& d = pi.chunks[size_t(c)]->plan.steps[i];
                    const Step& s0 = pi.chunks[0]->plan.steps[i];
                    d.algo = s0.algo; d.tile = s0.tile; d.splitk = s0.splitk;
                }
        }
        if (use_graph_ && !(precision_ == Precision::F8 && !w_->f8_ready) && pi.graph_ready) {
            for (auto& ch : pi.chunks) { Capture(*ch, 0, head, &ch->graph_exec); ch->graph_ready = true; }
            Capture(pi, head, pi.plan.steps.size(), &pi.tail_exec);
        }
    } catch (...) {
        for (auto& ch : pi.chunks) FreeInstance(*ch);
        pi.chunks.clear();
        if (pi.tail_exec) { (void)hipGraphExecDestroy(pi.tail_exec); pi.tail_exec = nullptr; }
        throw;
    }
    pi.head_steps = int(head);
}

struct DeviceModel::TuneContext {
    DeviceWeights& w;
    bool allow_search, log;
    hipEvent_t e0 = nullptr, e1 = nullptr;
    void* scrub = nullptr;
    bool searched = false;
    static constexpr size_t kScrubBytes = size_t(64) << 20;
    ~TuneContext() {
        if (e0) (void)hipEventDestroy(e0);
        if (e1) (void)hipEventDestroy(e1);
        if (scrub) (void)hipFree(scrub);
    }
    bool lookup(const std::vector<int64_t>& key, std::pair<int, int>* choice) {
        std::lock_guard<std::mutex> g(w.tune_mu);
        auto hit = w.tune_cache.find(key);
        if (hit == w.tune_cache.end()) return false;
        *choice = hit->second;
        return true;
    }
    void store(const std::vector<int64_t>& key, int code, int splitk) {
        std::lock_guard<std::mutex> g(w.tune_mu);
        w.tune_cache[key] = {code, splitk};
        w.tune_dirty = true;
        searched = true;
    }
};

void DeviceModel::Autotune(PlanInstance& pi, size_t nsteps, bool allow_search) {
    TuneContext ctx{*w_, allow_search, env_.flag("IE_TUNE_LOG")};
    check(hipEventCreate(&ctx.e0), "hipEventCreate");
    check(hipEventCreate(&ctx.e1), "hipEventCreate");
    if (const char* e = env_.get("IE_TUNE_HOT"); allow_search && !(e && std::atoi(e) != 0))
        if (hipMalloc(&ctx.scrub, TuneContext::kScrubBytes) != hipSuccess) { ctx.scrub = nullptr; (void)hipGetLastError(); }
    for (size_t si = 0; si < nsteps && si < pi.plan.steps.size(); ++si) TuneStep(ctx, pi, pi.plan.steps[si]);
    if (ctx.searched) SaveTuneCache();
}

float DeviceModel::TimeTrial(TuneContext& ctx, const PlanInstance& pi, const Step& trial) {
    auto timed = [&](int launches) {
        check(hipEventRecord(ctx.e0, stream_), "hipEventRecord");
        for (int r = 0; r < launches; ++r) LaunchStep(pi, trial, stream_);
        check(hipEventRecord(ctx.e1, stream_), "hipEventRecord");
        check(hipEventSynchronize(ctx.e1), "hipEventSynchronize");
        float ms = 0;
        check(hipEventElapsedTime(&ms, ctx.e0, ctx.e1), "hipEventElapsedTime");
        return ms;
    };
    LaunchStep(pi, trial, stream_);
    float best = 1e30f;
    for (int rep = 0; rep < (ctx.scrub ? 3 : 2); ++rep) {
        if (ctx.scrub) check(hipMemsetAsync(ctx.scrub, 0, TuneContext::kScrubBytes, stream_), "hipMemsetAsync(scrub)");
        best = std::min(best, timed(ctx.scrub ? 1 : 3));
    }
    if (ctx.log)
        std::fprintf(stderr, "[ie-tune] M=%lld N=%lld K=%lld algo=%d tile=%d splitk=%d: %.4f ms\n", static_cast<long long>(trial.out.n * trial.out.h * trial.out.w),
                     static_cast<long long>(trial.out.c), static_cast<long long>(trial.kh * trial.kw * trial.in.c), int(trial.algo), trial.tile, trial.splitk, best);
    return best;
}

void DeviceModel::TuneStep(TuneContext& ctx, const PlanInstance& pi, Step& s) {
    if (s.kind == StepKind::LayerNorm) {
        const std::vector<int64_t> key = {s.in.n * s.in.h * s.in.w, s.in.c, s.in.pitch, s.out.pitch, s.in.c_off, s.out.c_off, int64_t(s.in.f16), int64_t(s.out.f16), kLnTuneCode,
                                          s.bias_off >= 0};
        std::pair<int, int> hit{-1, 0};
        if (ctx.lookup(key, &hit)) {
            if (ln_tune_code(hit.first)) s.tile = hit.first - kLnTuneCode;
            return;
        }
        if (!ctx.allow_search) return;
        const LnArgs a = MakeLnArgs(pi, s, w_->d_weights);
        float best = 1e30f;
        int best_t = s.tile;
        for (int t = 0; t < kNumLnTiles; ++t)
            if (LayerNormEligible(a, t)) {
                Step trial = s;
                trial.tile = t;
                if (const float ms = TimeTrial(ctx, pi, trial); ms < best) { best = ms; best_t = t; }
            }
        s.tile = best_t;
        ctx.store(key, kLnTuneCode + best_t, 1);
        return;
    }
    if (s.kind != StepKind::Conv || s.algo == ConvAlgo::Naive || s.algo == ConvAlgo::Stem) return;
    std::pair<int, int> hit{-1, 0};
    auto cached_tile = [&](const std::vector<int64_t>& key) { return ctx.lookup(key, &hit) ? hit.first : -1; };
    auto time_tile = [&](int t) {
        Step trial = s;
        trial.tile = t;
        return TimeTrial(ctx, pi, trial);
    };
    if (s.algo == ConvAlgo::DualF8) {
        if (!s.in.f8) return;
        const std::vector<int64_t> key = {s.out.n * s.out.h * s.out.w, s.out.c, s.in.c, s.parts.size() == 2 ? s.parts[0].in.c : 0, s.parts.size() == 2 ? s.parts[0].sh : 0,
                                          s.in.pitch, s.out.pitch, int64_t(ConvAlgo::DualF8), s.bias_off >= 0};
        if (ctx.lookup(key, &hit)) { s.tile = hit.first; return; }
        if (!ctx.allow_search || !w_->f8_ready) return;
        const ConvArgs a = MakeConvArgs(pi, s);
        float best = 1e30f;
        int best_t = kWs8Code + 1;
        for (int t = 1; t < kNumConvWs8Tiles; ++t)
            if (ConvWs8Eligible(a, t))
                if (const float ms = time_tile(kWs8Code + t); ms < best) { best = ms; best_t = kWs8Code + t; }
        s.tile = best_t;
        ctx.store(key, best_t, 1);
        return;
    }
    if (s.algo == ConvAlgo::StemPool) {
        const std::vector<int64_t> key = {s.in.n, s.in.h, s.in.w, s.out.c, s.out.pitch, s.out.f8 ? 2 : (s.out.f16 ? 1 : 0), int64_t(ConvAlgo::StemPool)};
        int choice = cached_tile(key);
        const bool can = ConvStemPoolEligible(MakeConvArgs(pi, s));
        if (choice < 0 && ctx.allow_search && can && !(s.out.f8 && !w_->f8_ready)) {
            const float two = time_tile(0), one = time_tile(1);
            choice = one <= two * 1.05f ? 1 : 0;
            ctx.store(key, choice, 1);
        }
        if (!can) choice = 0;
        if (choice >= 0) s.tile = choice;
        return;
    }
    if (s.algo == ConvAlgo::DenseBlock || s.algo == ConvAlgo::DenseFused)
        for (Step& q : s.parts) TuneStep(ctx, pi, q);
    if (s.algo == ConvAlgo::DenseBlock) {
        const std::vector<int64_t> key = {s.in.n * s.in.h * s.in.w, int64_t(s.parts.size()), s.in.c, s.in.h, s.in.w, s.in.pitch, s.in.c_off, int64_t(ConvAlgo::DenseBlock),
                                          s.pre_scale_off >= 0, s.bias_off >= 0};
        int choice = cached_tile(key);
        DenseBlockArgs b;
        const bool can = MakeBlockArgs(pi, s, &b) && DenseBlockEligible(b);
        if (choice < 0 && ctx.allow_search && can) {
            const float parts = time_tile(0), chain = time_tile(1);
            choice = chain <= parts ? 1 : 0;
            ctx.store(key, choice, 1);
        }
        if (!can) choice = 0;
        if (choice >= 0) s.tile = choice;
        return;
    }
    if (s.algo == ConvAlgo::DenseFused) {
        const Step& p3 = s.parts[0];
        const std::vector<int64_t> key = {s.out.n * s.out.h * s.out.w, s.out.c, s.in.c, 1, 1, 1, 1, 0, 0, s.in.h, s.in.w, s.in.pitch, s.out.pitch, 0, int64_t(ConvAlgo::DenseFused),
                                          s.pre_scale_off >= 0, s.bias_off >= 0, p3.in.c, p3.in.pitch};
        int choice = cached_tile(key);
        if (choice < 0 && ctx.allow_search) {
            FusedArgs f;
            f.in3 = make_arg(pi, p3.in);
            f.out3 = make_arg(pi, p3.out);
            f.wfrag3 = w_->d_weights_frag && p3.w_off >= 0 ? w_->d_weights_frag + p3.w_off : nullptr;
            const ConvArgs a1 = MakeConvArgs(pi, s);
            float best = 1e30f;
            choice = 0;
            for (int t = 0; t <= kNumConvDenseFusedTiles; ++t)
                if (t == 0 || ConvDenseFusedEligible(a1, f, t))
                    if (const float ms = time_tile(t); ms < best) { best = ms; choice = t; }
            ctx.store(key, choice, 1);
        }
        if (choice >= 0) s.tile = choice;
        return;
    }
    if (s.algo == ConvAlgo::Depthwise) {
        const std::vector<int64_t> key = {s.out.n * s.out.h * s.out.w, s.out.c, s.kh, s.kw, s.sh, s.sw, s.pt, s.pl, s.in.h, s.in.w, s.in.pitch, s.out.pitch,
                                          s.in.nchw ? 2 : int64_t(s.in.f16), int64_t(ConvAlgo::Depthwise), s.pre_scale_off >= 0, s.has_in2};
        if (ctx.lookup(key, &hit)) {
            if (tune_family(hit.first).algo == ConvAlgo::Depthwise) s.tile = hit.first - tune_family(hit.first).base;
            return;
        }
        if (!ctx.allow_search) return;
        const DwArgs a = MakeDwArgs(pi, s);
        float best = 1e30f;
        int best_t = s.tile;
        for (int t = 0; t < kNumConvDwTiles; ++t)
            if (ConvDwEligible(a, t))
                if (const float ms = time_tile(t); ms < best) { best = ms; best_t = t; }
        s.tile = best_t;
        ctx.store(key, tune_code(ConvAlgo::Depthwise, best_t), 1);
        return;
    }
    if (s.algo == ConvAlgo::Grouped) {
        const std::vector<int64_t> key = {s.out.n * s.out.h * s.out.w, s.out.c, s.in.c, s.group, s.kh, s.kw, s.sh, s.sw, s.pt, s.pl, s.in.h, s.in.w, s.in.pitch,
                                          s.out.pitch, s.in.nchw ? 2 : int64_t(s.in.f16), int64_t(ConvAlgo::Grouped), s.pre_scale_off >= 0, s.has_in2};
        if (ctx.lookup(key, &hit)) {
            if (tune_family(hit.first).algo == ConvAlgo::Grouped) s.tile = hit.first - tune_family(hit.first).base;
            return;
        }
        if (!ctx.allow_search) return;
        const GroupedArgs a = MakeGroupedArgs(pi, s);
        float best = 1e30f;
        int best_t = s.tile;
        for (int t = 0; t < kNumConvGroupedTiles; ++t)
            if (ConvGroupedEligible(a, t))
                if (const float ms = time_tile(t); ms < best) { best = ms; best_t = t; }
        s.tile = best_t;
        ctx.store(key, tune_code(ConvAlgo::Grouped, best_t), 1);
        return;
    }
    if (s.algo == ConvAlgo::Transposed) {
        const std::vector<int64_t> key = {s.in.n * s.in.h * s.in.w, s.out.c, s.in.c, s.kh, s.kw, s.sh, s.sw, s.pt, s.pl, s.pb, s.pr, s.oph, s.opw, s.in.h, s.in.w,
                                          s.in.pitch, s.out.pitch, s.in.nchw ? 2 : int64_t(s.in.f16), int64_t(ConvAlgo::Transposed), s.bias_off >= 0};
        if (ctx.lookup(key, &hit)) {
            if (tune_family(hit.first).algo == ConvAlgo::Transposed) s.tile = hit.first - tune_family(hit.first).base;
            return;
        }
        if (!ctx.allow_search) return;
        const ConvtArgs a = MakeConvtArgs(pi, s);
        float best = 1e30f;
        int best_t = s.tile;
        for (int t = 0; t < kNumConvtTiles; ++t)
            if (ConvTransposedEligible(a, t))
                if (const float ms = time_tile(t); ms < best) { best = ms; best_t = t; }
        s.tile = best_t;
        ctx.store(key, tune_code(ConvAlgo::Transposed, best_t), 1);
        return;
    }
    const int64_t M = s.out.n * s.out.h * s.out.w, N = s.out.c;
    if (s.algo == ConvAlgo::IgemmF8) {
        const std::vector<int64_t> key = {M, N, s.in.c, s.kh, s.kw, s.sh, s.sw, s.pt, s.pl, s.in.h, s.in.w, s.in.pitch, s.out.pitch, 0, int64_t(s.algo), 0,
                                          s.bias_off >= 0, 8, s.has_in2};
        if (ctx.lookup(key, &hit)) { s.tile = hit.first; return; }
        if (!ctx.allow_search || !w_->f8_ready) return;
        const ConvArgs a = MakeConvArgs(pi, s);
        float best = 1e30f;
        int best_t = s.tile;
        auto consider = [&](int t) { if (const float ms = time_tile(t); ms < best) { best = ms; best_t = t; } };
        for (int t = 0; t < kNumConvF8Tiles; ++t) if (!(kIgemmTiles[t].bn > 32 && N <= 32)) consider(t);
        for (int t = 0; t < kNumConvWs8Tiles; ++t) if (ConvWs8Eligible(a, t)) consider(kWs8Code + t);
        for (int t = 0; t < kNumConvWs38Tiles; ++t) if (ConvWs38Eligible(a, t)) consider(kWs38Code + t);
        s.tile = best_t;
        ctx.store(key, best_t, 1);
        return;
    }
    const Step planned = s;
    if (s.algo == ConvAlgo::Ws1x1 || s.algo == ConvAlgo::Ws3x3 || s.algo == ConvAlgo::Direct || s.algo == ConvAlgo::Raster3x3 || s.algo == ConvAlgo::Wino3x3 || s.algo == ConvAlgo::X6) {
        s.algo = ConvAlgo::IgemmVec;
        s.tile = s.base_tile;
        s.splitk = 1;
    }
    const int64_t bk = s.in.f16 ? 2 * kIgemmBK : kIgemmBK;
    const int64_t KT = s.algo == ConvAlgo::IgemmVec ? int64_t(s.kh) * s.kw * ((s.in.c + bk - 1) / bk)
                                                   : (int64_t(s.kh) * s.kw * s.in.c + kIgemmBK - 1) / kIgemmBK;
    std::vector<int64_t> key = {M, N, s.in.c, s.kh, s.kw, s.sh, s.sw, s.pt, s.pl, s.in.h, s.in.w, s.in.pitch, s.out.pitch,
                                s.in.nchw, int64_t(s.algo), s.pre_scale_off >= 0, s.bias_off >= 0};
    if (s.in.f16 || s.out.f16) { key.push_back(s.in.f16); key.push_back(s.out.f16); }
    if (s.has_in2) key.push_back(1);
    const bool dil = s.dh != 1 || s.dw != 1;
    if (dil) key.insert(key.end(), {-1, s.dh, s.dw});
    auto igemm_split_ok = [&](const IgemmTile& T, int sp) {
        const int64_t wgs = ((M + T.bm - 1) / T.bm) * ((N + T.bn - 1) / T.bn);
        if (T.kg > 1 && ((!two_pass_splitk_ && !s.in.f16) || KT / (sp * T.kg) < 2)) return false;
        return KT / sp >= 2 && int64_t(sp) * wgs * T.bm * T.bn <= pi.workspace_floats && wgs <= kNumCounters && wgs * sp <= 8192 && wgs < 1024;
    };
    auto raster_split_ok = [&](int sp) {
        const int64_t chunks = (s.in.c + kIgemmBK - 1) / kIgemmBK, Mr = s.in.n * (s.in.h + 1) * (s.in.w + 1);
        return sp <= chunks && Mr / 64 * sp <= 16384 && int64_t(sp) * (M + 256) * (N + 64) * 2 <= pi.workspace_floats;
    };
    bool exact = ctx.lookup(key, &hit);
    if (!exact && !ctx.allow_search) {
        double best_d = 1.0;
        std::lock_guard<std::mutex> g(w_->tune_mu);
        for (const auto& kv : w_->tune_cache) {
            if (kv.first.size() != key.size() || !std::equal(kv.first.begin() + 1, kv.first.end(), key.begin() + 1)) continue;
            const double d = std::fabs(std::log2(double(kv.first[0]) / double(M)));
            if (d <= best_d) { best_d = d; hit = kv.second; }
        }
    }
    if (exact || hit.first >= 0) {
        const TuneFamily& f = tune_family(hit.first);
        int sp = hit.second;
        if (!exact && sp > 1 && !(f.base == 0 ? igemm_split_ok(kIgemmTiles[hit.first], sp) : f.algo == ConvAlgo::Raster3x3 && raster_split_ok(sp)))
            sp = 1;
        if (f.base != 0) s.algo = f.algo;
        s.tile = hit.first - f.base;
        s.splitk = sp;
        return;
    }
    if (!ctx.allow_search) { s = planned; return; }
    float best = 1e30f;
    Step chosen = s;
    auto consider = [&](ConvAlgo algo, int t, int sp) {
        Step trial = s;
        trial.algo = algo;
        trial.tile = t;
        trial.splitk = sp;
        if (const float ms = TimeTrial(ctx, pi, trial); ms < best) { best = ms; chosen = trial; }
    };
    if (!dil && !s.in.f16 && !s.out.f16 && s.algo == ConvAlgo::IgemmVec && s.kh == 3 && s.kw == 3 && s.sh == 1 && s.sw == 1 && s.pt == 1 && s.pl == 1 && s.pb == 1 &&
        s.pr == 1 && s.pre_scale_off < 0) {
        ConvArgs probe;
        probe.in = make_arg(pi, s.in);
        probe.out = make_arg(pi, s.out);
        probe.w = w_->d_weights + s.w_off;
        probe.kh = 3; probe.kw = 3; probe.pt = 1; probe.pl = 1;
        for (int t = 0; t < kNumConvRasterTiles; ++t) {
            if (!ConvRasterEligible(probe, t) || (ConvRasterTileBn(t) > 32 && N <= 32)) continue;
            for (int sp : {1, 2, 4, 8})
                if (sp == 1 || raster_split_ok(sp)) consider(ConvAlgo::Raster3x3, t, sp);
        }
    }
    if (!dil && !s.in.f16 && !s.out.f16 && s.algo == ConvAlgo::IgemmVec && s.kh == 3 && s.kw == 3 && s.out.c == 32 && !s.has_in2) {
        Step probe_step = s;
        probe_step.algo = ConvAlgo::Wino3x3;
        ConvArgs probe = MakeConvArgs(pi, probe_step);
        for (int t = 0; t < kNumConvWinoTiles; ++t) {
            if (!ConvWinoEligible(probe, t)) {
                if (ctx.log)
                    std::fprintf(stderr, "[ie-tune] M=%lld wino tile %d ineligible: wfrag=%p in(c=%d h=%d w=%d sw=%lld sh=%lld sn=%lld p=%p) out(c=%d sw=%lld p=%p) bias=%p pre=%p\n",
                                 static_cast<long long>(M), t, (const void*)probe.wfrag, probe.in.c, probe.in.h, probe.in.w, (long long)probe.in.sw, (long long)probe.in.sh,
                                 (long long)probe.in.sn, (void*)probe.in.p, probe.out.c, (long long)probe.out.sw, (void*)probe.out.p, (const void*)probe.bias, (const void*)probe.pre_scale);
                continue;
            }
            consider(ConvAlgo::Wino3x3, t, 1);
        }
    }
    if (!dil && w_->d_weights_x6 && !s.in.f16 && !s.out.f16 && s.algo == ConvAlgo::IgemmVec && s.kh == 1 && s.kw == 1 && !s.has_in2) {
        Step probe_step = s;
        probe_step.algo = ConvAlgo::X6;
        ConvArgs probe = MakeConvArgs(pi, probe_step);
        for (int t = 0; t < kNumConvX6Tiles; ++t)
            if (ConvX6Eligible(probe, t)) consider(ConvAlgo::X6, t, 1);
    }
    if (!dil && s.algo == ConvAlgo::IgemmVec) {
        ConvArgs probe = MakeConvArgs(pi, s);
        probe.res = TensorArg();
        for (int t = 0; t < kNumConvDirectTiles; ++t)
            if (ConvDirectEligible(probe, t)) consider(ConvAlgo::Direct, t, 1);
    }
    if (!dil && s.algo == ConvAlgo::IgemmVec && s.kh == 1 && s.kw == 1) {
        ConvArgs probe = MakeConvArgs(pi, s);
        for (int t = 0; t < (s.in.f16 ? kNumConvWs16Tiles : kNumConvWs32Tiles); ++t)
            if (s.in.f16 ? ConvWsEligible(probe, t) : ConvWs32Eligible(probe, t)) consider(ConvAlgo::Ws1x1, t, 1);
    }
    if (!dil && s.in.f16 && s.algo == ConvAlgo::IgemmVec && s.kh == 3 && s.kw == 3) {
        ConvArgs probe = MakeConvArgs(pi, s);
        for (int t = 0; t < kNumConvWs3Tiles; ++t)
            if (ConvWs3Eligible(probe, t)) consider(ConvAlgo::Ws3x3, t, 1);
    }
    static const int kSplits[] = {1, 2, 3, 4, 6, 8, 12, 16, 24};
    for (int t = 0; t < kNumIgemmTiles; ++t) {
        const IgemmTile& T = kIgemmTiles[t];
        if (dil && t >= kNumIgemmBaseTiles) continue;
        if ((T.bn > 32 && N <= 32) || (T.bn > 64 && N <= 64)) continue;
        if ((T.kg > 1 || T.deep) && (s.algo != ConvAlgo::IgemmVec || KT < 2 * T.kg)) continue;
        if (T.deep && s.in.f16) continue;
        if (T.deep && ((M + T.bm - 1) / T.bm) * ((N + T.bn - 1) / T.bn) > 1024) continue;
        for (int sp : kSplits)
            if (sp == 1 || igemm_split_ok(T, sp)) consider(s.algo, t, sp);
    }
    s = chosen;
    ctx.store(key, tune_code(s.algo, s.tile), s.splitk);
}

void DeviceModel::SaveTuneCache() {
    std::lock_guard<std::mutex> g(w_->tune_mu);
    if (w_->tune_cache_path.empty() || !w_->tune_dirty) return;
    const std::string tmp = w_->tune_cache_path + ".tmp" + std::to_string(long(getpid())) + "." + std::to_string(device_);
    {
        std::ofstream f(tmp, std::ios::trunc);
        if (!f) return;
        f << tune_file_header() << '\n';
        for (auto& kv : w_->tune_cache) {
            for (auto v : kv.first) f << v << ' ';
            f << ": " << kv.second.first << ' ' << kv.second.second << '\n';
// ... 187 lines not shown
            return with_tile(ConvDwEligible(MakeDwArgs(pi, s), s.tile) ? s.tile : 0);
        case ConvAlgo::Grouped:
            return with_tile(ConvGroupedEligible(MakeGroupedArgs(pi, s), s.tile) ? s.tile : 0);
        case ConvAlgo::Transposed:
            return with_tile(ConvTransposedEligible(MakeConvtArgs(pi, s), s.tile) ? s.tile : 0);
        case ConvAlgo::StemPool:
            return with_tile(s.tile != 0 && ConvStemPoolEligible(MakeConvArgs(pi, s)) ? s.tile : 0);
        case ConvAlgo::DenseBlock: {
            DenseBlockArgs b;
            return with_tile(s.tile != 0 && MakeBlockArgs(pi, s, &b) && DenseBlockEligible(b) ? s.tile : 0);
        }
        case ConvAlgo::DenseFused: {
            if (s.tile == 0) return s;
            const Step& s3 = s.parts.at(0);
            FusedArgs f;
            f.in3 = make_arg(pi, s3.in);
            f.out3 = make_arg(pi, s3.out);
            f.wfrag3 = w_->d_weights_frag && s3.w_off >= 0 ? w_->d_weights_frag + s3.w_off : nullptr;
            f.bias3 = s3.bias_off >= 0 ? w_->d_weights + s3.bias_off : nullptr;
            f.relu3 = s3.relu;
            return with_tile(ConvDenseFusedEligible(MakeConvArgs(pi, s), f, s.tile) ? s.tile : 0);
        }
        case ConvAlgo::IgemmF8: {
            const int t8 = s.tile;
            if (t8 < kWs8Code) return s;
            const ConvArgs a = MakeConvArgs(pi, s);
            const bool ok = t8 >= kWs38Code ? ConvWs38Eligible(a, t8 - kWs38Code) : ConvWs8Eligible(a, t8 - kWs8Code);
            return with_tile(ok ? t8 : (s.base_tile < kNumConvF8Tiles ? s.base_tile : 3));
        }
        case ConvAlgo::Ws1x1: case ConvAlgo::Ws3x3: case ConvAlgo::Direct: case ConvAlgo::Raster3x3: case ConvAlgo::Wino3x3: case ConvAlgo::X6:
        case ConvAlgo::Stem: {
            const ConvArgs a = MakeConvArgs(pi, s);
            ConvArgs plain = a;
            plain.res = TensorArg();
            bool ok = true;
            switch (s.algo) {
                case ConvAlgo::Ws1x1: ok = s.in.f16 ? ConvWsEligible(a, s.tile) : ConvWs32Eligible(a, s.tile); break;
                case ConvAlgo::Ws3x3: ok = ConvWs3Eligible(plain, s.tile); break;
                case ConvAlgo::Direct: ok = ConvDirectEligible(plain, s.tile); break;
                case ConvAlgo::Raster3x3: ok = ConvRasterEligible(plain, s.tile); break;
                case ConvAlgo::Wino3x3: ok = ConvWinoEligible(plain, s.tile); break;
                case ConvAlgo::X6: ok = ConvX6Eligible(plain, s.tile); break;
                default: ok = ConvStemEligible(a); break;
            }
            if (ok) return s;
            scratch = s;
            scratch.algo = s.algo == ConvAlgo::Stem ? ConvAlgo::IgemmScalar : ConvAlgo::IgemmVec;
            scratch.tile = s.base_tile;
            scratch.splitk = 1;
            return scratch;
        }
        default: return s;
    }
}

void DeviceModel::LaunchStep(const PlanInstance& pi, const Step& s_in, hipStream_t stream_) {
    Step handed;
    const Step& s = LaunchedStep(pi, s_in, handed);
    const float* wb = w_->d_weights;
    auto wp = [&](int64_t off) -> const float* { return off >= 0 ? wb + off : nullptr; };
    switch (s.kind) {
        case StepKind::Conv: {
            if (s.algo == ConvAlgo::DualF8) {
                if (s.in.f8) {
                    if (!w_->f8_ready) throw std::runtime_error("fp8 precision: scales are not calibrated yet");
                    const ConvArgs a = MakeConvArgs(pi, s);
                    const int t = s.tile >= kWs8Code ? s.tile - kWs8Code : 1;
                    if (a.in2.p == nullptr || !ConvWs8Eligible(a, t)) throw std::runtime_error("fp8 precision: the projection-shortcut step " + s.name + " cannot run on the dual 1x1 kernel");
                    check(LaunchConvWs1x1F8(a, t, stream_), "conv1x1_ws_f8(dual)");
                } else {
                    for (const Step& q : s.parts) LaunchStep(pi, q, stream_);
                }
                break;
            }
            if (s.algo == ConvAlgo::Depthwise) {
                check(LaunchConvDw(MakeDwArgs(pi, s), s.tile, stream_), "conv_dw");
                break;
            }
            if (s.algo == ConvAlgo::Grouped) {
                check(LaunchConvGrouped(MakeGroupedArgs(pi, s), s.tile, stream_), "conv_grouped");
                break;
            }
            if (s.algo == ConvAlgo::Transposed) {
                if (s.has_in2 || s.pre_scale_off >= 0) throw std::runtime_error("internal error: transposed conv " + s.name + " with a prologue or a residual");
                check(LaunchConvTransposed(MakeConvtArgs(pi, s), s.tile, stream_), "conv_transposed");
                break;
            }
            if (s.algo == ConvAlgo::StemPool) {
                if (s.tile != 0) check(LaunchConvStemPool(MakeConvArgs(pi, s), stream_), "conv_stem_pool");
                else for (const Step& q : s.parts) LaunchStep(pi, q, stream_);
                break;
            }
            if (s.algo == ConvAlgo::DenseBlock) {
                DenseBlockArgs b;
                if (s.tile != 0 && MakeBlockArgs(pi, s, &b)) check(LaunchDenseBlockF16(b, stream_), "dense_block_f16");
                else for (const Step& q : s.parts) LaunchStep(pi, q, stream_);
                break;
            }
            if (s.algo == ConvAlgo::DenseFused) {
                const Step& s3 = s.parts.at(0);
                ConvArgs a1 = MakeConvArgs(pi, s);
                FusedArgs f;
                f.in3 = make_arg(pi, s3.in);
                f.out3 = make_arg(pi, s3.out);
                f.wfrag3 = w_->d_weights_frag && s3.w_off >= 0 ? w_->d_weights_frag + s3.w_off : nullptr;
                f.bias3 = wp(s3.bias_off);
                f.relu3 = s3.relu;
                if (s.tile != 0) check(LaunchConvDenseFused(a1, f, s.tile, stream_), "conv_dense_fused");
                else {
                    LaunchStep(pi, s.parts[0], stream_);
                    LaunchStep(pi, s.parts[1], stream_);
                }
                break;
            }
            ConvArgs a = MakeConvArgs(pi, s);
            if (s.algo == ConvAlgo::IgemmF8) {
                if (!w_->f8_ready) throw std::runtime_error("fp8 precision: scales are not calibrated yet");
                const int t8 = s.tile;
                if (t8 >= kWs38Code) check(LaunchConvWs3x3F8(a, t8 - kWs38Code, stream_), "conv3x3_ws_f8");
                else if (t8 >= kWs8Code) check(LaunchConvWs1x1F8(a, t8 - kWs8Code, stream_), "conv1x1_ws_f8");
                else check(LaunchConvIgemmF8(a, t8, stream_), "conv_igemm_f8");
                break;
            }
            if (a.in.f8 || a.res.f8 || (a.out.f8 && s_in.algo != ConvAlgo::Stem)) throw std::runtime_error("internal error: fp8 tensor reached a non-fp8 conv kernel");
            if ((s.dh != 1 || s.dw != 1) && !DilationOk(s.algo)) throw std::runtime_error("internal error: dilated conv " + s.name + " reached a kernel without dilation");
            const TensorArg res = a.res;
            const int relu = a.relu;
            const bool split_res = res.p != nullptr && s.algo != ConvAlgo::Ws1x1;
            if (split_res) { a.res = TensorArg(); a.relu = 0; }
            if (s.algo == ConvAlgo::Naive) check(LaunchConvNaive(a, stream_), "conv_naive");
            else if (s.algo == ConvAlgo::Raster3x3) check(LaunchConvRaster3x3(a, s.tile, s.splitk, stream_), "conv3x3_raster");
            else if (s.algo == ConvAlgo::Ws1x1 && s.in.f16) check(LaunchConvWs1x1F16(a, s.tile, stream_), "conv1x1_ws_f16");
            else if (s.algo == ConvAlgo::Ws1x1) check(LaunchConvWs1x1F32(a, s.tile, stream_), "conv1x1_ws_f32");
            else if (s.algo == ConvAlgo::Ws3x3) check(LaunchConvWs3x3F16(a, s.tile, stream_), "conv3x3_ws_f16");
            else if (s.algo == ConvAlgo::Stem) check(LaunchConvStem(a, stream_), "conv_stem");
            else if (s.algo == ConvAlgo::Wino3x3) check(LaunchConvWino3x3(a, s.tile, stream_), "conv3x3_wino");
            else if (s.algo == ConvAlgo::X6) check(LaunchConvX6(a, s.tile, stream_), "conv1x1_x6");
            else if (s.algo == ConvAlgo::Direct) check(LaunchConvDirect(a, s.tile, stream_), "conv_direct");
            else if (s.in.f16) check(LaunchConvIgemmF16(a, s.tile, s.splitk, stream_), "conv_igemm_f16");
            else check(LaunchConvIgemm(a, s.tile, s.algo == ConvAlgo::IgemmVec ? 1 : 0, s.splitk, stream_), "conv_igemm");
            if (split_res) {
                EltArgs e;
                e.a = a.out; e.b = res; e.out = a.out; e.relu = relu;
                check(LaunchEltwise(e, stream_), "eltwise(residual)");
            }
            break;
        }
        case StepKind::Pool: {
            PoolArgs a;
            a.in = make_arg(pi, s.in);
            a.out = make_arg(pi, s.out);
            a.kh = s.kh; a.kw = s.kw; a.sh = s.sh; a.sw = s.sw; a.pt = s.pt; a.pl = s.pl; a.pb = s.pb; a.pr = s.pr;
            a.is_max = s.pool_max; a.count_include_pad = s.count_include_pad;
            a.pre_scale = wp(s.pre_scale_off); a.pre_shift = wp(s.pre_shift_off); a.pre_relu = s.pre_relu;
            if (a.in.f8 || a.out.f8) {
                const DeviceWeights& W = *w_;
                auto scale_of = [&](int step) { return step >= 0 && size_t(step) < W.act_scale.size() && W.act_scale[size_t(step)] > 0.f ? W.act_scale[size_t(step)] : 1.f; };
                a.in_scale = scale_of(s.in_src);
                a.out_qscale = 1.0f / scale_of(s.idx);
                check(LaunchPoolF8(a, stream_), "pool_f8");
                break;
            }
            check(LaunchPool(a, stream_), "pool");
            break;
        }
        case StepKind::GlobalAvgPool:
            if (s.in.f8) {
                const DeviceWeights& W = *w_;
                const float sc = s.in_src >= 0 && size_t(s.in_src) < W.act_scale.size() && W.act_scale[size_t(s.in_src)] > 0.f ? W.act_scale[size_t(s.in_src)] : 1.f;
                check(LaunchGlobalAvgPoolF8(make_arg(pi, s.in), make_arg(pi, s.out), sc, stream_), "global_avg_pool_f8");
                break;
            }
            check(LaunchGlobalAvgPool(make_arg(pi, s.in), make_arg(pi, s.out), wp(s.pre_scale_off), wp(s.pre_shift_off),
                                      s.pre_relu, stream_, int(s.pre_act.kind), s.pre_act.a, s.pre_act.b), "global_avg_pool");
            break;
        case StepKind::Eltwise: {
            if (s.in.f8 || s.out.f8) throw std::runtime_error("internal error: fp8 tensor reached the eltwise kernel");
            EltArgs a;
            a.a = make_arg(pi, s.in);
            if (s.has_in2) a.b = make_arg(pi, s.in2);
            a.out = make_arg(pi, s.out);
            a.scale = wp(s.pre_scale_off);
            a.shift = wp(s.pre_shift_off);
            a.relu = s.relu;
            a.lo = s.lo;
            a.hi = s.hi;
            a.act = int(s.act.kind); a.act_a = s.act.a; a.act_b = s.act.b;
            a.b_mul = s.mul;
            a.b_bcast = s.has_in2 && s.in2.h * s.in2.w == 1 && s.out.h * s.out.w > 1;
            check(LaunchEltwise(a, stream_), "eltwise");
            break;
        }
        case StepKind::SqueezeExcite: {
            if (s.in.f8 || s.out.f8) throw std::runtime_error("internal error: fp8 tensor reached the squeeze-excite kernels");
            const SeArgs a = MakeSeArgs(pi, s);
            if (!SqueezeExciteEligible(a)) throw std::runtime_error("squeeze-excite step " + s.name + ": the kernels decline its operands");
            check(LaunchSqueezeExcite(a, stream_), "squeeze_excite");
            break;
        }
        case StepKind::Copy:
            if (s.in.f8 || s.out.f8) throw std::runtime_error("internal error: fp8 tensor reached the copy kernel");
            check(LaunchCopy(make_arg(pi, s.in), make_arg(pi, s.out), stream_), "copy");
            break;
        case StepKind::Resize: {
            if (s.in.f8 || s.out.f8) throw std::runtime_error("internal error: fp8 tensor reached the resize kernels");
            const ResizeArgs a = MakeResizeArgs(pi, s);
            check(LaunchResize(a, ResizePath(a), stream_), "resize");
            break;
        }
        case StepKind::LayerNorm:
            if (s.in.f8 || s.out.f8) throw std::runtime_error("internal error: fp8 tensor reached the layer-norm kernels");
            check(LaunchLayerNorm(MakeLnArgs(pi, s, wb), s.tile, stream_), "layer_norm");
            break;
        case StepKind::TokenAssemble: {
            if (s.in.f8 || s.out.f8) throw std::runtime_error("internal error: fp8 tensor reached the token kernels");
            TokenAssembleArgs a;
            a.in = make_arg(pi, s.in);
            a.out = make_arg(pi, s.out);
            a.cls = wp(s.w_off);
            a.pos = wp(s.bias_off);
            check(LaunchTokenAssemble(a, stream_), "token_assemble");
            break;
        }
        case StepKind::Attention:
            if (s.in.f8 || s.out.f8) throw std::runtime_error("internal error: fp8 tensor reached the attention kernels");
            check(LaunchAttention(MakeAttnArgs(pi, s), s.tile, stream_), "attention");
            break;
    }
}

static std::string kernel_label(const Step& s) {
    switch (s.kind) {
        case StepKind::Conv:
            if (s.algo == ConvAlgo::Naive) return "conv_naive_kernel";
            if (s.algo == ConvAlgo::Depthwise) {
                static const int px[kNumConvDwTiles] = {0, 1, 2, 4};
                const bool act = s.act.kind != ActKind::None || s.pre_act.kind != ActKind::None;
                return s.tile == 0 ? std::string("conv_dw_generic_kernel")
                                   : std::string("conv_dw_kernel<") + (s.out.f16 ? "f16,k" : "f32,k") + std::to_string(s.kh) + ",s" + std::to_string(s.sh) + ",px" +
                                         std::to_string(DwLanePixels(px[s.tile], s.out.f16, s.kh, s.sh, act)) + (act ? ",act>" : ">");
            }
            if (s.algo == ConvAlgo::Grouped) {
                const int cfg = GroupedCfgFor(s.in.c, s.out.c, s.group);
                if (s.tile == 0 || cfg < 0) return "conv_grouped_generic_kernel";
                const GroupedCfg& c = kGroupedCfgs[cfg];
                return std::string("conv_grouped_kernel<") + (s.out.f16 ? "f16,c" : "f32,c") + std::to_string(c.cpg) + ",o" + std::to_string(c.opb) + "x" +
                       std::to_string(c.gpb) + ",px" + std::to_string(kGroupedPx[s.tile]) + ">";
            }
            if (s.algo == ConvAlgo::Transposed)
                return s.tile == 0 ? std::string("convt_generic_kernel")
                                   : std::string("convt_phase_kernel<") + (s.out.f16 ? "f16,px" : "f32,px") + std::to_string(32 * kConvtPixelBlocks[s.tile]) + ">";
            if (s.algo == ConvAlgo::DenseBlock) return s.tile != 0 ? "dense_block_f16_kernel<" + std::to_string(s.parts.size() / 2) + " layers>" : "dense_block_parts<" + std::to_string(s.parts.size()) + " launches>";
            if (s.algo == ConvAlgo::DenseFused && s.tile == 0) return "dense_fused_parts<2 launches>";
            if (s.algo == ConvAlgo::DenseFused) return (s.tile == 4 || s.tile == 5 ? "conv_dense_fused_ws_kernel<t" : "conv_dense_fused_kernel<t") + std::to_string(s.tile) + ">";
            if (s.algo == ConvAlgo::DualF8) return s.in.f8 ? "conv1x1_ws_f8_kernel<dual,t" + std::to_string(s.tile >= kWs8Code ? s.tile - kWs8Code : 1) + ">" : "dual_f8_parts<2 launches>";
            if (s.algo == ConvAlgo::IgemmF8 && s.tile >= kWs38Code) return "conv3x3_ws_f8_kernel<t" + std::to_string(s.tile - kWs38Code) + ">";
            if (s.algo == ConvAlgo::IgemmF8 && s.tile >= kWs8Code) return "conv1x1_ws_f8_kernel<t" + std::to_string(s.tile - kWs8Code) + ">";
            if (s.algo == ConvAlgo::IgemmF8)
                return "conv_igemm_f8_kernel<" + std::to_string(kIgemmTiles[s.tile].bm) + "x" + std::to_string(kIgemmTiles[s.tile].bn) + ">";
            if (s.algo == ConvAlgo::Direct) {
                const char* k = s.tile >= 10 ? "conv1x1_as_kernel<f32,t" : s.tile >= kNumDirectBaseTiles ? "conv_win_kernel<f32,t"
                                             : s.in.f16 ? "conv_direct_kernel<f16,t" : "conv_direct_kernel<f32,t";
                return std::string(k) + std::to_string(s.tile) + ">";
            }
            if (s.algo == ConvAlgo::StemPool) return s.tile != 0 ? (s.out.f8 ? "conv_stem_kernel<f16,pool,e4m3 out>" : (s.out.f16 ? "conv_stem_kernel<f16,pool>" : "conv_stem_kernel<f32,pool>")) : "stem + pool (2 launches)";
            if (s.algo == ConvAlgo::Stem) return s.out.f8 ? "conv_stem_kernel<f16,e4m3 out>" : (s.out.f16 ? "conv_stem_kernel<f16>" : "conv_stem_kernel<f32>");
            if (s.algo == ConvAlgo::Ws1x1) return std::string(s.in.f16 ? "conv1x1_ws_f16_kernel<t" : "conv1x1_ws_f32_kernel<t") + std::to_string(s.tile) + ">";
            if (s.algo == ConvAlgo::Ws3x3) return "conv3x3_ws_f16_kernel<t" + std::to_string(s.tile) + ">";
            if (s.algo == ConvAlgo::Wino3x3) return std::string(s.tile >= 8 ? "conv3x3_wino_x6_kernel<t" : "conv3x3_wino_kernel<t") + std::to_string(s.tile) + ">";
            if (s.algo == ConvAlgo::X6) return "conv1x1_x6_kernel<t" + std::to_string(s.tile) + ">";
            if (s.algo == ConvAlgo::Raster3x3)
                return "conv3x3_raster_kernel<t" + std::to_string(s.tile) + (s.splitk > 1 ? ",splitk" + std::to_string(s.splitk) : std::string()) + ">";
            return std::string(s.in.f16 ? "conv_igemm_f16_kernel<" : "conv_igemm_kernel<") + std::to_string(kIgemmTiles[s.tile].bm) + "x" +
                   std::to_string(kIgemmTiles[s.tile].bn) + (kIgemmTiles[s.tile].kg > 1 ? "x" + std::to_string(kIgemmTiles[s.tile].kg) + "kg" : std::string()) +
                   (kIgemmTiles[s.tile].deep ? ",deep" : "") +
                   (s.algo == ConvAlgo::IgemmVec ? ",vec" : ",scalar") +
                   (s.splitk > 1 ? ",splitk" + std::to_string(s.splitk) : std::string()) + ">";
        case StepKind::Pool: return s.in.f8 ? "pool_f8_kernel" : "pool_kernel";
        case StepKind::GlobalAvgPool: return s.in.f8 ? "gap_f8_kernel" : "gap_kernel";
        case StepKind::Eltwise: return "eltwise_kernel";
        case StepKind::Copy: return "copy_kernel";
        case StepKind::Resize: {
            static const char* const names[3] = {"resize_generic_kernel", "resize_vec_kernel<", "resize_nchw_kernel<"};
            ResizeArgs a;
            a.in = view_strides(s.in);
            a.out = view_strides(s.out);
            if (s.in.c_off % (s.in.f16 ? 8 : 4)) a.in.p = reinterpret_cast<float*>(uintptr_t(4));
            if (s.out.c_off % (s.out.f16 ? 8 : 4)) a.out.p = reinterpret_cast<float*>(uintptr_t(4));
            const int path = ResizePath(a);
            return path == 0 ? std::string(names[0]) : std::string(names[path]) + (s.in.f16 ? "f16>" : "f32>");
        }
        case StepKind::LayerNorm:
            return s.tile == 0 ? std::string("layernorm_generic_kernel")
                               : std::string("layernorm_kernel<") + (s.out.f16 ? "f16," : "f32,") + std::to_string(kLnLanes[s.tile]) + ">";
        case StepKind::TokenAssemble: return std::string("token_assemble_kernel<") + (s.out.f16 ? "f16>" : "f32>");
        case StepKind::Attention:
            return s.tile == 0 ? std::string("attention_generic_kernel")
                               : std::string("attention_mfma_kernel<") + (s.out.f16 ? "f16," : "f32,") + std::to_string(s.head_dim) + ">";
        case StepKind::SqueezeExcite: return std::string("se_squeeze_kernel + se_fc1_kernel + se_fc2_kernel + se_apply_kernel<") + (s.out.f16 ? "f16>" : "f32>");
    }
    return "?";
}

void DeviceModel::RunSteps(PlanInstance& pi, size_t first, size_t last, std::vector<hipEvent_t>* events) {
    size_t k = 0;
    if (events) check(hipEventRecord((*events)[k++], stream_), "hipEventRecord");
    for (size_t i = first; i < last && i < pi.plan.steps.size(); ++i) {
        LaunchStep(pi, pi.plan.steps[i], stream_);
        if (events) check(hipEventRecord((*events)[k++], stream_), "hipEventRecord");
    }
}

void DeviceModel::RefreshGraphs(PlanInstance& pi) {
    if (!use_graph_) return;
    if (precision_ == Precision::F8 && !w_->f8_ready) throw std::runtime_error("fp8 precision: scales are not calibrated yet");
    const uint64_t gen = w_->f8_gen.load();
    if (pi.graph_ready && pi.captured_gen == gen) return;
    check(hipStreamSynchronize(stream_), "hipStreamSynchronize");
    auto drop = [](hipGraphExec_t& g) { if (g) (void)hipGraphExecDestroy(g); g = nullptr; };
    drop(pi.graph_exec);
    pi.graph_ready = false;
    Capture(pi, 0, pi.plan.steps.size(), &pi.graph_exec);
    pi.graph_ready = true;
    if (!pi.chunks.empty() && pi.head_steps > 0) {
        for (auto& ch : pi.chunks) {
            drop(ch->graph_exec);
            ch->graph_ready = false;
            Capture(*ch, 0, size_t(pi.head_steps), &ch->graph_exec);
            ch->graph_ready = true;
        }
        drop(pi.tail_exec);
        Capture(pi, size_t(pi.head_steps), pi.plan.steps.size(), &pi.tail_exec);
    }
    pi.captured_gen = gen;
}

void DeviceModel::Enqueue(PlanInstance& pi) {
    check(hipSetDevice(device_), "hipSetDevice");
    RefreshGraphs(pi);
    if (pi.graph_ready) check(hipGraphLaunch(pi.graph_exec, stream_), "hipGraphLaunch");
    else RunSteps(pi, 0, pi.plan.steps.size(), nullptr);
}

void DeviceModel::Synchronize() {
    check(hipSetDevice(device_), "hipSetDevice");
    check(hipStreamSynchronize(stream_), "hipStreamSynchronize");
}

std::vector<StepTiming> DeviceModel::Profile(PlanInstance& pi, int iters) {
    check(hipSetDevice(device_), "hipSetDevice");
    const size_t ns = pi.plan.steps.size();
    std::vector<hipEvent_t> ev(ns + 1);
    for (auto& e : ev) check(hipEventCreate(&e), "hipEventCreate");
    std::vector<StepTiming> out(ns);
    for (size_t i = 0; i < ns; ++i) {
        out[i].name = pi.plan.steps[i].name;
        Step handed;
        out[i].kernel = kernel_label(LaunchedStep(pi, pi.plan.steps[i], handed));
        out[i].flops = pi.plan.steps[i].flops;
        out[i].bytes = pi.plan.steps[i].bytes;
    }
    try {
        RunSteps(pi, 0, ns, nullptr);
        check(hipStreamSynchronize(stream_), "hipStreamSynchronize");
        std::vector<std::vector<float>> samples(ns);
        for (int it = 0; it < iters; ++it) {
            RunSteps(pi, 0, ns, &ev);
            check(hipStreamSynchronize(stream_), "hipStreamSynchronize");
            for (size_t i = 0; i < ns; ++i) {
                float ms = 0;
                check(hipEventElapsedTime(&ms, ev[i], ev[i + 1]), "hipEventElapsedTime");
                samples[i].push_back(ms);
            }
        }
        for (size_t i = 0; i < ns; ++i) {
            std::sort(samples[i].begin(), samples[i].end());
            const size_t n = samples[i].size();
            out[i].ms = n == 0 ? 0.0 : (n % 2 ? samples[i][n / 2] : 0.5 * (samples[i][n / 2 - 1] + samples[i][n / 2]));
        }
    } catch (...) {
        for (auto& e : ev) (void)hipEventDestroy(e);
        throw;
    }
    for (auto& e : ev) (void)hipEventDestroy(e);
    return out;
}

void DeviceModel::InferHost(PlanInstance& pi, const std::vector<const void*>& inputs, const std::vector<size_t>& in_bytes,
                            const std::vector<void*>& outputs, const std::vector<size_t>& out_bytes, const std::vector<char>& in_u8) {
    std::vector<std::vector<InSeg>> in(pi.plan.inputs.size());
    for (size_t i = 0; i < pi.plan.inputs.size(); ++i) {
        const bool u8 = i < in_u8.size() && in_u8[i];
        const size_t need = size_t(pi.plan.inputs[i].view.numel()) * (u8 ? 1 : sizeof(float));
        in[i].push_back({inputs[i], inputs[i] ? std::min(in_bytes[i], need) : 0, need, 0, u8});
    }
    std::vector<std::vector<OutSeg>> out(pi.plan.outputs.size());
    for (size_t i = 0; i < outputs.size() && i < pi.plan.outputs.size(); ++i) {
        if (!outputs[i] || out_bytes[i] == 0) continue;
        out[i].push_back({outputs[i], out_bytes[i], size_t(pi.plan.outputs[i].view.numel()) * sizeof(float), 0});
    }
    InferHostSegments(pi, in, out);
}

void DeviceModel::InferHostSegments(PlanInstance& pi, const std::vector<std::vector<InSeg>>& in, const std::vector<std::vector<OutSeg>>& out) {
    check(hipSetDevice(device_), "hipSetDevice");
    EnsurePipeline(pi, false);
    RefreshGraphs(pi);
    const int C = pi.chunks.empty() ? 1 : int(pi.chunks.size());
    struct Job { int chunk; char* dst; const char* src; size_t copy, zero; };
    std::vector<Job> jobs;
    struct U8 { size_t input; };
    std::vector<char> is_u8(pi.plan.inputs.size(), 0);
    try {
        for (size_t i = 0; i < pi.plan.inputs.size() && i < in.size(); ++i) {
            const View& v = pi.plan.inputs[i].view;
            char* base = reinterpret_cast<char*>(pi.buffers[size_t(v.buf)]);
            const bool u8 = !in[i].empty() && in[i][0].u8;
            is_u8[i] = u8 ? 1 : 0;
            if (u8) {
                if (pi.u8_stage.size() < pi.plan.inputs.size()) pi.u8_stage.resize(pi.plan.inputs.size(), nullptr);
                if (!pi.u8_stage[i]) {
                    check(hipMalloc(&pi.u8_stage[i], std::max<size_t>(size_t(v.numel()), 16)), "hipMalloc(u8 staging)");
                    device_bytes_ += size_t(v.numel());
                }
                base = static_cast<char*>(pi.u8_stage[i]);
            }
            const size_t total = size_t(v.numel()) * (u8 ? 1 : sizeof(float));
            const size_t per_chunk = total / size_t(C);
            for (const InSeg& sg : in[i]) {
                if (sg.u8 != u8) throw std::runtime_error("internal error: mixed UINT8 / FLOAT32 segments for one input");
                if (sg.dev_off + sg.need > total) throw std::runtime_error("internal error: input segment exceeds the planned tensor");
                const size_t have = sg.host ? std::min(sg.have, sg.need) : 0;
                size_t off = 0;
                while (off < sg.need) {
                    const size_t dev = sg.dev_off + off;
                    const int c = int(std::min<size_t>(dev / per_chunk, size_t(C - 1)));
                    const size_t end = std::min(sg.need, (size_t(c) + 1) * per_chunk - sg.dev_off);
                    const size_t nb = end - off;
                    const size_t cp = off < have ? std::min(nb, have - off) : 0;
                    jobs.push_back({c, base + dev, cp ? static_cast<const char*>(sg.host) + off : nullptr, cp, nb - cp});
                    off = end;
                }
            }
        }
        for (int c = 0; c < C; ++c) {
            for (const Job& j : jobs) {
                if (j.chunk != c) continue;
                if (j.copy) check(hipMemcpyAsync(j.dst, j.src, j.copy, hipMemcpyHostToDevice, copy_stream_), "hipMemcpyAsync(H2D)");
                if (j.zero) check(hipMemsetAsync(j.dst + j.copy, 0, j.zero, copy_stream_), "hipMemsetAsync");
            }
            for (size_t i = 0; i < pi.plan.inputs.size(); ++i) {
                if (!is_u8[i]) continue;
                const View& v = pi.plan.inputs[i].view;
                const int64_t n = v.numel() / C;
                check(LaunchConvertU8ToF32(static_cast<char*>(pi.u8_stage[i]) + int64_t(c) * n, pi.buffers[size_t(v.buf)] + int64_t(c) * n, n, u8_scale_, u8_bias_,
                                           copy_stream_), "convert_u8_f32");
            }
            check(hipEventRecord(h2d_events_[size_t(c)], copy_stream_), "hipEventRecord");
            check(hipStreamWaitEvent(stream_, h2d_events_[size_t(c)], 0), "hipStreamWaitEvent");
            if (c == 0) check(hipEventRecord(t0_event_, stream_), "hipEventRecord");
            if (C > 1) {
                PlanInstance& ch = *pi.chunks[size_t(c)];
                if (ch.graph_ready) check(hipGraphLaunch(ch.graph_exec, stream_), "hipGraphLaunch(head)");
                else RunSteps(ch, 0, size_t(pi.head_steps), nullptr);
            }
        }
        if (C > 1) {
            if (pi.tail_exec) check(hipGraphLaunch(pi.tail_exec, stream_), "hipGraphLaunch(tail)");
            else RunSteps(pi, size_t(pi.head_steps), pi.plan.steps.size(), nullptr);
            ++pipelined_calls_;
        } else {
            Enqueue(pi);
        }
        check(hipEventRecord(t1_event_, stream_), "hipEventRecord");
        last_chunks_ = C;
        last_head_steps_ = C > 1 ? pi.head_steps : 0;
        struct Scatter { size_t j, lo, stage_off; };
        std::vector<Scatter> staged;
        size_t stage_used = 0;
        for (size_t j = 0; j < pi.plan.outputs.size() && j < out.size(); ++j) {
            if (out[j].empty()) continue;
            const View& v = pi.plan.outputs[j].view;
            const char* src = reinterpret_cast<const char*>(pi.buffers[size_t(v.buf)]);
            const size_t total = size_t(v.numel()) * sizeof(float);
            size_t lo = SIZE_MAX, hi = 0;
            for (const OutSeg& sg : out[j]) {
                const size_t nb = std::min(sg.cap, sg.need);
                if (!nb) continue;
                if (sg.dev_off + nb > total) throw std::runtime_error("internal error: output segment exceeds the planned tensor");
                lo = std::min(lo, sg.dev_off);
                hi = std::max(hi, sg.dev_off + nb);
            }
            if (hi <= lo) continue;
            if (stage_used + (hi - lo) <= pinned_bytes_) {
                check(hipMemcpyAsync(static_cast<char*>(pinned_) + stage_used, src + lo, hi - lo, hipMemcpyDeviceToHost, stream_), "hipMemcpyAsync(D2H)");
                staged.push_back({j, lo, stage_used});
                stage_used += (hi - lo + 63) & ~size_t(63);
            } else {
                for (const OutSeg& sg : out[j]) {
                    const size_t nb = std::min(sg.cap, sg.need);
                    if (nb) check(hipMemcpyAsync(sg.host, src + sg.dev_off, nb, hipMemcpyDeviceToHost, stream_), "hipMemcpyAsync(D2H)");
                }
            }
        }
        check(hipStreamSynchronize(stream_), "hipStreamSynchronize");
        {
            float ms = 0;
            last_forward_ms_ = hipEventElapsedTime(&ms, t0_event_, t1_event_) == hipSuccess ? double(ms) : 0.0;
        }
        for (const Scatter& sc : staged)
            for (const OutSeg& sg : out[sc.j]) {
                const size_t nb = std::min(sg.cap, sg.need);
                if (nb) std::memcpy(sg.host, static_cast<char*>(pinned_) + sc.stage_off + (sg.dev_off - sc.lo), nb);
            }
        for (size_t j = 0; j < out.size(); ++j)
            for (const OutSeg& sg : out[j]) {
                const size_t nb = std::min(sg.cap, sg.need);
                if (sg.cap > nb) std::memset(static_cast<char*>(sg.host) + nb, 0, sg.cap - nb);
            }
    } catch (...) {
        (void)hipStreamSynchronize(copy_stream_);
        (void)hipStreamSynchronize(stream_);
        throw;
    }
}

}
```

gpu-ai-inference-server_amd/csrc/executor.h:

```cpp
#pragma once
#include <hip/hip_runtime.h>

#include <atomic>
#include <map>
#include <memory>
#include <mutex>
#include <string>
#include <utility>
#include <vector>

#include "kernels.h"
#include "onnx_reader.h"
#include "env.h"
#include "plan.h"

namespace ie {

struct StepTiming {
    std::string name, kernel;
    double ms = 0, flops = 0, bytes = 0;
};

struct DeviceWeights {
    int device = 0;
    float* d_weights = nullptr;
    void* d_weights16 = nullptr;
    void* d_weights16_frag = nullptr;
    struct Frag16Region { int64_t w_off; int rows, k; };
    std::vector<Frag16Region> frag16_regions;
    float* d_weights_frag = nullptr;
    void* d_weights8 = nullptr;
    float* d_f8_aux = nullptr;
    struct F8Conv { int step; int64_t w_off; int cout, k; int in_src; int64_t aux_off; };
    std::vector<F8Conv> f8_convs;
    std::vector<float> act_scale;
    bool f8_ready = false;
    std::atomic<uint64_t> f8_gen{0};
    float* d_weights_wino = nullptr;
    struct WinoRegion { int64_t w_off, u_off; int cout, cin; };
    std::vector<WinoRegion> wino_regions;
    void* d_weights_x6 = nullptr;
    void* d_weights_wino_x6 = nullptr;
    struct X6Region { int64_t w_off, byte_off; int cout, k; };
    std::vector<X6Region> x6_regions;
    bool fp32_split = false;
    struct FragRegion { int64_t w_off; int cout, kk, cin; };
    std::vector<FragRegion> frag_regions;
    size_t weight_floats = 0;
    size_t wino_floats = 0, x6_bytes = 0, f8_aux_floats = 0;
    bool uploaded = false;
    std::atomic<size_t> device_bytes{0};
    std::mutex tune_mu;
    std::map<std::vector<int64_t>, std::pair<int, int>> tune_cache;
    std::string tune_cache_path;
    bool tune_dirty = false;
    ~DeviceWeights();
};

struct PlanInstance {
    Plan plan;
    std::vector<float*> buffers;
    std::vector<char> owned;
    float* workspace = nullptr;
    bool owns_workspace = false;
    int64_t workspace_floats = 0;
    int* counters = nullptr;
    hipGraphExec_t graph_exec = nullptr;
    bool graph_ready = false;
    uint64_t captured_gen = 0;
    std::vector<void*> u8_stage;
    std::vector<std::unique_ptr<PlanInstance>> chunks;
    int64_t batch_off = 0;
    int head_steps = 0;
    hipGraphExec_t tail_exec = nullptr;
    bool pipeline_tried = false;
};

struct DeviceModelOptions {
    Precision precision = Precision::F32;
    std::shared_ptr<DeviceWeights> share;
    bool upload_weights = true;
    std::string tune_cache_path;
    bool fp32_split = false;
};

class DeviceModel {
public:
    DeviceModel(std::shared_ptr<const OnnxModel> model, int device_id, const DeviceModelOptions& opt);
    ~DeviceModel();
    DeviceModel(const DeviceModel&) = delete;
    DeviceModel& operator=(const DeviceModel&) = delete;

    PlanInstance& Prepare(const std::vector<std::vector<int64_t>>& shapes, bool allow_tune);
    void Enqueue(PlanInstance& pi);
    std::vector<StepTiming> Profile(PlanInstance& pi, int iters);
    void Synchronize();

    void InferHost(PlanInstance& pi, const std::vector<const void*>& inputs, const std::vector<size_t>& in_bytes,
                   const std::vector<void*>& outputs, const std::vector<size_t>& out_bytes, const std::vector<char>& in_u8 = {});
    void SetU8Transform(float scale, float bias) { u8_scale_ = scale; u8_bias_ = bias; }
    struct InSeg { const void* host; size_t have, need, dev_off; bool u8 = false; };
    struct OutSeg { void* host; size_t cap, need, dev_off; };
    void InferHostSegments(PlanInstance& pi, const std::vector<std::vector<InSeg>>& in, const std::vector<std::vector<OutSeg>>& out);

    hipStream_t stream() const { return stream_; }
    int device() const { return device_; }
    float* weights() const { return w_->d_weights; }
    const std::shared_ptr<DeviceWeights>& shared_weights() const { return w_; }
    Precision precision() const { return precision_; }
    bool fp32_split() const { return fp32_split_; }
    void WeightsArrived(const std::vector<float>* adopt_act_scales = nullptr);
    std::vector<float> f8_act_scales() const { return w_->act_scale; }
    std::vector<std::pair<std::string, uint64_t>> MirrorChecksums();
    void CopySync(void* dst, const void* src, size_t bytes, hipMemcpyKind kind, const char* what);
    void ZeroSync(void* dst, size_t bytes, const char* what);
    size_t weight_bytes() const { return w_->weight_floats * sizeof(float); }
    size_t device_bytes() const { return device_bytes_ + w_->device_bytes.load(); }
    PlanInstance* current() { return current_; }
    int64_t pipelined_calls() const { return pipelined_calls_; }
    int last_chunks() const { return last_chunks_; }
    int last_head_steps() const { return last_head_steps_; }
    double last_forward_ms() const { return last_forward_ms_; }
    int max_inflight_replays() const { return max_inflight_replays_; }

private:
    void RunSteps(PlanInstance& pi, size_t first, size_t last, std::vector<hipEvent_t>* events);
    void BuildInstance(PlanInstance& pi, const std::vector<std::vector<int64_t>>& shapes);
    void FreeInstance(PlanInstance& pi);
    void Capture(PlanInstance& pi, size_t first, size_t last, hipGraphExec_t* exec);
    void Autotune(PlanInstance& pi, size_t nsteps, bool allow_search);
    struct TuneContext;
    void TuneStep(TuneContext& ctx, const PlanInstance& pi, Step& s);
    float TimeTrial(TuneContext& ctx, const PlanInstance& pi, const Step& trial);
    void SaveTuneCache();
    void EnsurePipeline(PlanInstance& pi, bool allow_tune);
    void AllocInstance(PlanInstance& pi);
    void RefreshGraphs(PlanInstance& pi);
    void PrepareF8(const std::vector<float>* adopt_act_scales = nullptr);
    void LaunchStep(const PlanInstance& pi, const Step& s, hipStream_t stream);
    const Step& LaunchedStep(const PlanInstance& pi, const Step& s, Step& scratch) const;
    ConvArgs MakeConvArgs(const PlanInstance& pi, const Step& s) const;
    DwArgs MakeDwArgs(const PlanInstance& pi, const Step& s) const;
    GroupedArgs MakeGroupedArgs(const PlanInstance& pi, const Step& s) const;
    ConvtArgs MakeConvtArgs(const PlanInstance& pi, const Step& s) const;
    SeArgs MakeSeArgs(const PlanInstance& pi, const Step& s) const;
    bool MakeBlockArgs(const PlanInstance& pi, const Step& s, DenseBlockArgs* out) const;

    Env env_;
    std::shared_ptr<const OnnxModel> model_;
    int device_ = 0;
    hipStream_t stream_ = nullptr;
    hipStream_t copy_stream_ = nullptr;
    std::vector<hipEvent_t> h2d_events_;
    hipEvent_t t0_event_ = nullptr, t1_event_ = nullptr;
    std::shared_ptr<DeviceWeights> w_;
    bool owns_weights_ = false;
    bool upload_weights_ = true;
    bool fp32_split_ = false;
    Precision precision_ = Precision::F32;
    size_t device_bytes_ = 0;
    float u8_scale_ = 1.0f / 255.0f, u8_bias_ = 0.0f;
    bool use_graph_ = true;
    bool autotune_ = true;
    bool tune_on_demand_ = false;
    int pipeline_chunks_ = 2;
    int pipeline_head_ = -1;
    bool two_pass_splitk_ = true;
    std::map<std::vector<int64_t>, std::unique_ptr<PlanInstance>> plans_;
    std::vector<std::vector<int64_t>> lru_;
    size_t max_plans_ = 8;
    PlanInstance* current_ = nullptr;
    void* pinned_ = nullptr;
    size_t pinned_bytes_ = 0;
    int64_t pipelined_calls_ = 0;
    int last_chunks_ = 1, last_head_steps_ = 0;
    double last_forward_ms_ = 0;
    int max_inflight_replays_ = 0;
};

int HipDeviceCount();
std::string HipDeviceInfo(int device_id);
bool HipMemoryInfo(int device_id, size_t* total, size_t* free_b);

}
```

gpu-ai-inference-server_amd/csrc/kernels.h:

```cpp
#pragma once
#include <hip/hip_runtime.h>

#include <cmath>
#include <cstddef>
#include <cstdint>

namespace ie {

struct TensorArg {
    float* p = nullptr;
    int n = 0, h = 0, w = 0, c = 0;
    int64_t sn = 0, sh = 0, sw = 0, sc = 0;
    int f16 = 0;
    int f8 = 0;
};

__host__ __device__ inline float ApplyActBasic(int kind, float a, float b, float x) {
    switch (kind) {
        case 1: return 1.f / (1.f + expf(-x));
        case 2: return fminf(fmaxf(a * x + b, 0.f), 1.f);
        case 3: return x / (1.f + expf(-x));
        case 4: return x * fminf(fmaxf(a * x + b, 0.f), 1.f);
        case 5: return fmaxf(x, 0.f);
        default: return x;
    }
}
__host__ __device__ inline float ApplyAct(int kind, float a, float b, float x) {
    switch (kind) {
        case 6: return 0.5f * x * (1.f + erff(x * 0.70710678f));
        case 7: return 0.5f * x * (1.f + tanhf(0.79788456f * (x + 0.044715f * x * x * x)));
        default: return ApplyActBasic(kind, a, b, x);
    }
}

struct ConvArgs {
    TensorArg in, out;
    TensorArg res;
    const float* w = nullptr;
    const void* w16 = nullptr;
    const float* wfrag = nullptr;
    const float* bias = nullptr;
    const float* pre_scale = nullptr;
    const float* pre_shift = nullptr;
    const void* pre_scale16 = nullptr;
    const void* pre_shift16 = nullptr;
    int kh = 1, kw = 1, sh = 1, sw = 1, pt = 0, pl = 0;
    int pre_relu = 0, relu = 0;
    float* workspace = nullptr;
    int64_t workspace_floats = 0;
    int* counters = nullptr;
    int num_counters = 0;
    const void* w8 = nullptr;
    const float* escale = nullptr;
    float res_scale = 1.f, out_qscale = 1.f;
    TensorArg in2;
    const void* w8b = nullptr;
    const float* escale_b = nullptr;
    const float* bias_b = nullptr;
    int sh2 = 1, sw2 = 1;
    int64_t in2_bytes = 0;
    int debug = 0;
    int16_t dh = 1, dw = 1;
    int64_t in_bytes = 0;
};
static_assert(sizeof(ConvArgs) == 464 && offsetof(ConvArgs, in_bytes) == 456, "ConvArgs layout: the dilation must stay in the padding");

struct FusedConsts {
    unsigned mg20_c4n3 = 0, mg20_c4n = 0, mg20_w = 0, mg20_h = 0;
    unsigned hbig = 0x7fffffff;
    unsigned mg32_hw = 0, mg32_w = 0, mg32_cpt3 = 0;
    int wrpp = 0, wfull = 0, wlast = 0;
    int rpp = 0, xfull = 0, xlast = 0;
};

struct FusedArgs {
    TensorArg in3, out3;
    const float* wfrag3 = nullptr;
    const float* bias3 = nullptr;
    int relu3 = 0;
    FusedConsts k;
};

struct PoolArgs {
    TensorArg in, out;
    int kh = 1, kw = 1, sh = 1, sw = 1, pt = 0, pl = 0, pb = 0, pr = 0;
    int is_max = 0, count_include_pad = 0;
    const float* pre_scale = nullptr;
    const float* pre_shift = nullptr;
    int pre_relu = 0;
    float in_scale = 1.f, out_qscale = 1.f;
};

struct EltArgs {
    TensorArg a, b, out;
    const float* scale = nullptr;
    const float* shift = nullptr;
    int relu = 0;
    float lo = -__builtin_huge_valf(), hi = __builtin_huge_valf();
    int act = 0;
    float act_a = 0.f, act_b = 0.f;
    int b_mul = 0;
    int b_bcast = 0;
};

struct DwArgs {
    TensorArg in, out, res;
    const float* w = nullptr;
    const float* bias = nullptr;
    const float* pre_scale = nullptr;
    const float* pre_shift = nullptr;
    int pre_relu = 0;
    float pre_hi = __builtin_huge_valf();
    int kh = 1, kw = 1, sh = 1, sw = 1, pt = 0, pl = 0;
    int relu = 0;
    float lo = -__builtin_huge_valf(), hi = __builtin_huge_valf();
    int act = 0, pre_act = 0;
    float act_a = 0.f, act_b = 0.f, pre_act_a = 0.f, pre_act_b = 0.f;
};
constexpr int kNumConvDwTiles = 4;
constexpr int DwLanePixels(int px, bool f16, int k, int s, bool act) {
    return !act ? px : (px >= 4 && k * (3 * s + k) * (f16 ? 8 : 4) <= 200 ? 4 : (px >= 2 && k * (s + k) * (f16 ? 8 : 4) <= 200 ? 2 : 1));
}
bool ConvDwEligible(const DwArgs& a, int tile);
hipError_t LaunchConvDw(const DwArgs& a, int tile, hipStream_t stream);

struct GroupedArgs : DwArgs {
    const void* w16 = nullptr;
    int groups = 1;
};
struct GroupedCfg { int cpg, opb, gpb; };
inline constexpr GroupedCfg kGroupedCfgs[] = {{1, 2, 8}, {2, 2, 8}, {4, 4, 4}, {8, 8, 2}, {8, 8, 1}, {16, 16, 1}, {32, 16, 1}, {64, 16, 1}};
inline constexpr int kNumGroupedCfgs = int(sizeof(kGroupedCfgs) / sizeof(kGroupedCfgs[0]));
constexpr int kNumConvGroupedTiles = 4;
inline constexpr int kGroupedPx[kNumConvGroupedTiles] = {0, 1, 2, 4};
constexpr int GroupedCfgFor(int64_t cin, int64_t cout, int64_t groups) {
    if (groups < 2 || cin % groups || cout % groups) return -1;
    const int64_t cpg = cin / groups, opg = cout / groups;
    for (int i = 0; i < kNumGroupedCfgs; ++i) {
        const GroupedCfg& c = kGroupedCfgs[i];
        if (c.cpg == cpg && (c.gpb > 1 ? opg == c.opb && groups % c.gpb == 0 : opg % c.opb == 0)) return i;
    }
    return -1;
}
constexpr bool GroupedTileFits(int cfg, bool f16, int tile) {
    if (cfg < 0 || tile < 1 || tile >= kNumConvGroupedTiles) return false;
    const GroupedCfg& c = kGroupedCfgs[cfg];
    const int in_regs = f16 && c.cpg % 2 == 0 ? c.cpg * c.gpb / 2 : c.cpg * c.gpb;
    return kGroupedPx[tile] * (c.opb * c.gpb + in_regs) <= 128;
}
bool ConvGroupedEligible(const GroupedArgs& a, int tile);
hipError_t LaunchConvGrouped(const GroupedArgs& a, int tile, hipStream_t stream);

struct ConvtArgs {
    TensorArg in, out;
    const float* w = nullptr;
    const void* w16 = nullptr;
    const float* bias = nullptr;
    int kh = 1, kw = 1, sh = 1, sw = 1, pt = 0, pl = 0, pb = 0, pr = 0, oph = 0, opw = 0;
    int relu = 0;
};
constexpr int kNumConvtTiles = 3;
inline constexpr int kConvtPixelBlocks[kNumConvtTiles] = {0, 1, 2};
bool ConvTransposedEligible(const ConvtArgs& a, int tile);
hipError_t LaunchConvTransposed(const ConvtArgs& a, int tile, hipStream_t stream);

struct LnArgs {
    TensorArg in, out;
    const float* gamma = nullptr;
    const float* beta = nullptr;
    float eps = 1e-5f;
};
constexpr int kNumLnTiles = 5;
inline constexpr int kLnLanes[kNumLnTiles] = {0, 8, 16, 32, 64};
constexpr int kLnMaxVectors = 6;
constexpr bool LnTileFits(int64_t c, bool f16, int tile) {
    const int64_t V = f16 ? 8 : 4;
    return tile >= 1 && tile < kNumLnTiles && c % V == 0 && c / V <= int64_t(kLnLanes[tile]) * kLnMaxVectors;
}
constexpr int LnDefaultTile(int64_t c, bool f16) {
    for (int t = 1; t < kNumLnTiles; ++t) if (LnTileFits(c, f16, t) && c / (f16 ? 8 : 4) <= 3 * kLnLanes[t]) return t;
    for (int t = 1; t < kNumLnTiles; ++t) if (LnTileFits(c, f16, t)) return t;
    return 0;
}
bool LayerNormEligible(const LnArgs& a, int tile);
hipError_t LaunchLayerNorm(const LnArgs& a, int tile, hipStream_t stream);

struct AttnArgs {
    TensorArg in, out;
    int heads = 0, head_dim = 0;
    float scale = 1.f;
};
constexpr int kNumAttnTiles = 2;
constexpr int64_t kAttnLdsBudget = 160 * 1024;
constexpr int64_t AttnLdsBytes(int64_t L, int hd, bool f16) {
    return 2 * ((L + 31) / 32 * 32) * (int64_t(hd) * (f16 ? 2 : 4) + 16);
}
constexpr bool AttnMfmaFits(int64_t L, int hd, bool f16, int64_t c_in, int64_t pitch_in, int64_t off_in, int64_t c_out, int64_t pitch_out, int64_t off_out) {
    const int64_t V = f16 ? 8 : 4;
    return (hd == 32 || hd == 64) && L >= 1 && c_in % V == 0 && pitch_in % V == 0 && off_in % V == 0 && c_out % V == 0 && pitch_out % V == 0 && off_out % V == 0 &&
           AttnLdsBytes(L, hd, f16) <= kAttnLdsBudget;
}
bool AttentionEligible(const AttnArgs& a, int tile);
hipError_t LaunchAttention(const AttnArgs& a, int tile, hipStream_t stream);
hipError_t InitKernelsAttn();

struct TokenAssembleArgs {
    TensorArg in, out;
    const float* cls = nullptr;
    const float* pos = nullptr;
};
hipError_t LaunchTokenAssemble(const TokenAssembleArgs& a, hipStream_t stream);
bool TokenAssembleVectorised(const TokenAssembleArgs& a);

struct SeArgs {
    TensorArg in, out;
    const float* w1 = nullptr;
    const float* b1 = nullptr;
    const float* w2t = nullptr;
    const float* b2 = nullptr;
    int mid = 0;
    int act1 = 0, act = 0;
    float act1_a = 0.f, act1_b = 0.f, act_a = 0.f, act_b = 0.f;
    int chunks = 1;
    float* workspace = nullptr;
    int64_t workspace_floats = 0;
};
inline int SeSqueezeChunks(int64_t n, int64_t hw) {
    int64_t want = (1024 + n - 1) / n;
    int64_t by_px = hw / 64;
    int64_t c = want < by_px ? want : by_px;
    return int(c < 1 ? 1 : (c > 64 ? 64 : c));
}
inline int64_t SeWorkspaceFloats(int64_t n, int64_t c, int64_t mid, int chunks) { return int64_t(chunks) * n * c + n * mid + n * c + 64; }
bool SqueezeExciteEligible(const SeArgs& a);
hipError_t LaunchSqueezeExcite(const SeArgs& a, hipStream_t stream);
hipError_t LaunchSqueezeExcitePhase(const SeArgs& a, int phase, hipStream_t stream);

bool SplitKWorkspaceOk(int64_t workspace_floats, int num_counters, int splitk, int64_t num_tiles, int tile_elems);
struct ResizeArgs {
    TensorArg in, out;
    int mode = 0;
    int coord = 0;
    int nearest = 0;
    double scale_h = 1.0, scale_w = 1.0;
};
int ResizePath(const ResizeArgs& a);
hipError_t LaunchResize(const ResizeArgs& a, int path, hipStream_t stream);
hipError_t LaunchConvIgemm(const ConvArgs& a, int tile, int vec, int splitk, hipStream_t stream);
constexpr int kNumConvRasterTiles = 8;
bool ConvRasterEligible(const ConvArgs& a, int tile);
int ConvRasterTileBn(int tile);
hipError_t LaunchConvRaster3x3(const ConvArgs& a, int tile, int splitk, hipStream_t stream);
hipError_t LaunchConvNaive(const ConvArgs& a, hipStream_t stream);
hipError_t LaunchSplitKReduce(const ConvArgs& a, int splitk, hipStream_t stream);
hipError_t LaunchConvIgemmF16(const ConvArgs& a, int tile, int splitk, hipStream_t stream);
hipError_t InitKernelsF16();
constexpr int kNumConvWsTiles = 12;
constexpr int kNumConvWs16Tiles = 18;
bool ConvWsEligible(const ConvArgs& a, int tile);
hipError_t LaunchConvWs1x1F16(const ConvArgs& a, int tile, hipStream_t stream);
hipError_t InitKernelsWs();
constexpr int kNumConvWs32Tiles = kNumConvWsTiles + 2 + 6;
bool ConvWs32Eligible(const ConvArgs& a, int tile);
hipError_t LaunchConvWs1x1F32(const ConvArgs& a, int tile, hipStream_t stream);
hipError_t InitKernelsWs32();
constexpr int kNumConvWs3Tiles = 5;
bool ConvWs3Eligible(const ConvArgs& a, int tile);
hipError_t LaunchConvWs3x3F16(const ConvArgs& a, int tile, hipStream_t stream);
hipError_t InitKernelsWs3();
constexpr int kNumDirectBaseTiles = 6;
constexpr int kNumConvDirectTiles = 15;
hipError_t LaunchPermuteWeightsFrag(const float* src, float* dst, int Cout, int KK, int Cin, hipStream_t stream);
bool ConvDirectEligible(const ConvArgs& a, int tile);
hipError_t LaunchConvDirect(const ConvArgs& a, int tile, hipStream_t stream);
hipError_t InitKernelsDirect();
int ResidentPerCu(const void* kernel, int block, size_t lds);

bool ConvStemEligible(const ConvArgs& a);
hipError_t LaunchConvStem(const ConvArgs& a, hipStream_t stream);
bool ConvStemPoolEligible(const ConvArgs& a);
hipError_t LaunchConvStemPool(const ConvArgs& a, hipStream_t stream);
hipError_t InitKernelsStem();
constexpr int kNumConvWinoTiles = 12;
bool ConvWinoEligible(const ConvArgs& a, int tile);
hipError_t LaunchConvWino3x3(const ConvArgs& a, int tile, hipStream_t stream);
hipError_t LaunchWinogradWeights(const float* w, float* u, int Cout, int Cin, hipStream_t stream);
hipError_t LaunchWinogradWeightsX6(const float* w, void* dst, int Cout, int Cin, hipStream_t stream);
hipError_t InitKernelsWino();
constexpr int kNumConvX6Tiles = 2;
bool ConvX6Eligible(const ConvArgs& a, int tile);
hipError_t LaunchConvX6(const ConvArgs& a, int tile, hipStream_t stream);
hipError_t LaunchSplitWeightsX6(const float* w, void* dst, int Cout, int K, hipStream_t stream);
hipError_t InitKernelsX6();
constexpr int kNumConvDenseFusedTiles = 6;
bool ConvDenseFusedEligible(const ConvArgs& a, const FusedArgs& f, int tile);
hipError_t LaunchConvDenseFused(const ConvArgs& a, const FusedArgs& f, int tile, hipStream_t stream);
hipError_t InitKernelsFused();
struct DenseBlockLayer {
    int K = 0;
    int out_coff = 0;
    unsigned w1 = 0, w3 = 0;
    unsigned ps = 0xffffffffu, pt = 0xffffffffu;
    unsigned b1 = 0xffffffffu, b3 = 0xffffffffu;
    int flags = 0;
};
constexpr int kMaxBlockLayers = 24;
struct DenseBlockArgs {
    _Float16* x = nullptr;
    int pitch = 0, in_coff = 0;
    int n = 0, h = 0, w = 0;
    const _Float16* wfrag16 = nullptr;
    const _Float16* w16 = nullptr;
    uint64_t w16_bytes = 0;
    const float* w32 = nullptr;
    int nlayers = 0;
    int band_rows = 0;
    int strip_rows = 0;
    long long* dbg = nullptr;
    DenseBlockLayer layer[kMaxBlockLayers];
};
bool DenseBlockEligible(const DenseBlockArgs& a);
hipError_t LaunchDenseBlockF16(const DenseBlockArgs& a, hipStream_t stream);
hipError_t LaunchPermuteWeightsFrag16(const void* src, void* dst, int rows, int K, hipStream_t stream);
hipError_t InitKernelsBlock();
constexpr int kNumConvF8Tiles = 7;
bool ConvF8Eligible(const ConvArgs& a, int tile);
hipError_t LaunchConvIgemmF8(const ConvArgs& a, int tile, hipStream_t stream);
hipError_t InitKernelsF8();
constexpr int kNumConvWs8Tiles = 10;
bool ConvWs8Eligible(const ConvArgs& a, int tile);
hipError_t LaunchConvWs1x1F8(const ConvArgs& a, int tile, hipStream_t stream);
hipError_t InitKernelsWs8();
constexpr int kNumConvWs38Tiles = 8;
constexpr int kWs8Code = 100;
constexpr int kWs38Code = 200;
bool ConvWs38Eligible(const ConvArgs& a, int tile);
hipError_t LaunchConvWs3x3F8(const ConvArgs& a, int tile, hipStream_t stream);
hipError_t LaunchQuantizeRowsE4m3(const float* w, void* w8, float* wscale, int rows, int K, hipStream_t stream);
hipError_t LaunchScaleVector(const float* src, float* dst, float s, int n, hipStream_t stream);
hipError_t LaunchPoolF8(const PoolArgs& a, hipStream_t stream);
hipError_t LaunchGlobalAvgPoolF8(const TensorArg& in, const TensorArg& out, float in_scale, hipStream_t stream);
hipError_t LaunchAbsMax(const TensorArg& t, float* result, hipStream_t stream);
hipError_t LaunchE4m3RoundTrip(const float* src, float* dst, void* codes, float scale, int64_t n, hipStream_t stream);
hipError_t LaunchConvertF32ToF16(const float* src, void* dst, int64_t n, hipStream_t stream);
hipError_t LaunchConvertU8ToF32(const void* src, float* dst, int64_t n, float scale, float bias, hipStream_t stream);
hipError_t LaunchPool(const PoolArgs& a, hipStream_t stream);
hipError_t LaunchGlobalAvgPool(const TensorArg& in, const TensorArg& out, const float* pre_scale, const float* pre_shift,
                               int pre_relu, hipStream_t stream, int pre_act = 0, float pre_act_a = 0.f, float pre_act_b = 0.f);
hipError_t LaunchEltwise(const EltArgs& a, hipStream_t stream);
hipError_t LaunchCopy(const TensorArg& in, const TensorArg& out, hipStream_t stream);
hipError_t LaunchVectorAdd(const float* a, const float* b, float* result, int64_t n, hipStream_t stream);

double MfmaPeakTflops(int nacc, int blocks_per_cu, int iters);

hipError_t InitKernels();

}
```

Before: 16170 images/sec.

## Fuse DenseNet transition avg-pool into following 1x1 conv and chain next conv

Adds a new kernel family that computes a 2x2 stride-2 average pool, with an optional BN/ReLU prologue, directly inside a 1x1 fp32 conv. It can also chain the next block's first 1x1 conv, with its BN prologue, in the same launch. A plan analysis finds eligible pool→conv(→conv) step runs, and PairTransitions assigns them launch roles, either through autotuning or through the IE_POOL_CONV override. The aim is to remove the pooled tensor's round trip through memory and the extra launches at each transition. The cost is a large amount of new, complex kernel code and extra tune-cache codes.

```diff
diff --git a/gpu-ai-inference-server_amd/build.py b/gpu-ai-inference-server_amd/build.py
--- a/gpu-ai-inference-server_amd/build.py
+++ b/gpu-ai-inference-server_amd/build.py
@@ -14,7 +14,7 @@
 HIPCC = os.environ.get("HIPCC", "/opt/rocm/bin/hipcc")
 ARCH = "gfx950"
 
-SOURCES = ["env.cpp", "onnx_reader.cpp", "plan.cpp", "repository.cpp", "config.cpp", "executor.cpp", "bridge.cpp", "bridge_load.cpp", "bridge_run.cpp", "kernels.hip", "kernels_f16.hip", "kernels_ws.hip", "kernels_ws32.hip", "kernels_stem.hip", "kernels_direct.hip", "kernels_f8.hip", "kernels_fused.hip", "kernels_wino.hip", "kernels_x6.hip", "kernels_block.hip", "kernels_ws8.hip", "kernels_dw.hip", "kernels_se.hip", "kernels_grouped.hip", "kernels_resize.hip", "kernels_convt.hip", "kernels_ln.hip", "kernels_attn.hip", "kernels_tokens.hip"]
+SOURCES = ["env.cpp", "onnx_reader.cpp", "plan.cpp", "repository.cpp", "config.cpp", "executor.cpp", "bridge.cpp", "bridge_load.cpp", "bridge_run.cpp", "kernels.hip", "kernels_f16.hip", "kernels_ws.hip", "kernels_ws32.hip", "kernels_stem.hip", "kernels_direct.hip", "kernels_f8.hip", "kernels_fused.hip", "kernels_wino.hip", "kernels_x6.hip", "kernels_block.hip", "kernels_ws8.hip", "kernels_dw.hip", "kernels_se.hip", "kernels_grouped.hip", "kernels_resize.hip", "kernels_convt.hip", "kernels_ln.hip", "kernels_attn.hip", "kernels_tokens.hip", "kernels_trans.hip"]
 COMMON = ["-std=c++17", "-O3", "-fPIC", "-Wall", "-Wextra", "-Wno-unused-parameter", "-Wno-unused-result",
           "-I" + os.path.join(ROOT, "include"), "-I" + CSRC]
 
diff --git a/gpu-ai-inference-server_amd/csrc/bridge.cpp b/gpu-ai-inference-server_amd/csrc/bridge.cpp
--- a/gpu-ai-inference-server_amd/csrc/bridge.cpp
+++ b/gpu-ai-inference-server_amd/csrc/bridge.cpp
@@ -464,7 +464,9 @@
                 if (w == "fp16" || w == "f16" || w == "half") prec = ie::Precision::F16;
                 else if (w == "fp8" || w == "f8" || w == "e4m3") prec = ie::Precision::F8;
             }
-            o << ",\"plan\":" << ie::PlanToJson(ie::BuildPlan(m, shapes, prec));
+            const ie::Plan plan = ie::BuildPlan(m, shapes, prec);
+            o << ",\"paired_launches\":" << ie::PairedLaunchesToJson(ie::FindPairedLaunches(plan));
+            o << ",\"plan\":" << ie::PlanToJson(plan);
         }
         o << "}";
         return dup_cstr(o.str());
diff --git a/gpu-ai-inference-server_amd/csrc/env.cpp b/gpu-ai-inference-server_amd/csrc/env.cpp
--- a/gpu-ai-inference-server_amd/csrc/env.cpp
+++ b/gpu-ai-inference-server_amd/csrc/env.cpp
@@ -25,6 +25,7 @@
     "IE_AUTOTUNE", "IE_TUNE_CACHE", "IE_TUNE_BATCHES", "IE_TUNE_ON_DEMAND", "IE_TUNE_HOT", "IE_TUNE_LOG",
     "IE_DISABLE_GRAPH", "IE_SPLITK_IN_LAUNCH", "IE_PIPELINE_CHUNKS", "IE_PIPELINE_HEAD", "IE_MAX_PLANS", "IE_NO_FRAG_WEIGHTS",
     "IE_F8_CALIB_BATCH", "IE_F8_MARGIN",
+    "IE_POOL_CONV",
     "IE_MAX_INFLIGHT_REPLAYS",
     "IE_DEBUG_ABLATE", "IE_AS_PAD", "IE_NO_PERSISTENT",
     nullptr};
diff --git a/gpu-ai-inference-server_amd/csrc/executor.cpp b/gpu-ai-inference-server_amd/csrc/executor.cpp
--- a/gpu-ai-inference-server_amd/csrc/executor.cpp
+++ b/gpu-ai-inference-server_amd/csrc/executor.cpp
@@ -133,12 +133,14 @@
 std::string tune_file_header() {
     std::ostringstream o;
     o << kTuneFileTag << ' ' << kNumIgemmTiles << ' ' << kNumConvRasterTiles << ' ' << kNumConvWs32Tiles << ' ' << kNumConvWs16Tiles << ' ' << kNumConvWs3Tiles << ' '
-      << kNumConvDirectTiles << ' ' << kNumConvWinoTiles << ' ' << kNumConvX6Tiles << ' ' << kNumConvWs8Tiles << ' ' << kNumConvWs38Tiles << ' ' << kNumConvDenseFusedTiles;
+      << kNumConvDirectTiles << ' ' << kNumConvWinoTiles << ' ' << kNumConvX6Tiles << ' ' << kNumConvWs8Tiles << ' ' << kNumConvWs38Tiles << ' ' << kNumConvDenseFusedTiles << ' ' << kNumConvPooledTiles;
     return o.str();
 }
 
 constexpr int kLnTuneCode = 1000;
 bool ln_tune_code(int t) { return t >= kLnTuneCode && t < kLnTuneCode + kNumLnTiles; }
+constexpr int kPoolConvTuneCode = 1100;
+bool pool_conv_tune_code(int t) { return t >= kPoolConvTuneCode && t <= kPoolConvTuneCode + 2 * kNumConvPooledTiles; }
 struct TuneFamily { int base; ConvAlgo algo; int tiles; };
 constexpr TuneFamily kTuneFamilies[] = {
     {0, ConvAlgo::IgemmVec, kNumIgemmTiles},          {100, ConvAlgo::Raster3x3, kNumConvRasterTiles},
@@ -161,7 +163,7 @@
 }
 
 bool tune_code_valid(int t) {
-    return (t >= 0 && t - tune_family(t).base < tune_family(t).tiles) || ln_tune_code(t) || (t >= kWs8Code && t < kWs8Code + kNumConvWs8Tiles) ||
+    return (t >= 0 && t - tune_family(t).base < tune_family(t).tiles) || ln_tune_code(t) || pool_conv_tune_code(t) || (t >= kWs8Code && t < kWs8Code + kNumConvWs8Tiles) ||
            (t >= kWs38Code && t < kWs38Code + kNumConvWs38Tiles);
 }
 
@@ -213,6 +215,7 @@
         if (g_kernels_err == hipSuccess) g_kernels_err = InitKernelsBlock();
         if (g_kernels_err == hipSuccess) g_kernels_err = InitKernelsWs8();
         if (g_kernels_err == hipSuccess) g_kernels_err = InitKernelsAttn();
+        if (g_kernels_err == hipSuccess) g_kernels_err = InitKernelsTrans();
     });
     check(g_kernels_err, "InitKernels");
     fp32_split_ = opt.fp32_split && opt.precision == Precision::F32;
@@ -244,6 +247,10 @@
     const char* tp = env_.get("IE_SPLITK_IN_LAUNCH");
     two_pass_splitk_ = !(tp && tp[0] == '1');
     autotune_ = !(at && at[0] == '0') && !env_.get("IE_FORCE_TILE") && !env_.get("IE_FORCE_SPLITK") && !env_.get("IE_FORCE_ALGO");
+    if (const char* pc = env_.get("IE_POOL_CONV"); pc && pc[0] >= '0' && pc[0] <= '2') {
+        pool_conv_mode_ = pc[0] - '0';
+        if (pc[1] == ':' && pc[2] >= '0' && pc[2] <= '9') pool_conv_tile_ = std::atoi(pc + 2);
+    }
     if (const char* od = env_.get("IE_TUNE_ON_DEMAND")) tune_on_demand_ = od[0] == '1';
     if (const char* pc = env_.get("IE_PIPELINE_CHUNKS")) pipeline_chunks_ = std::max(0, std::min(kMaxChunks, std::atoi(pc)));
     if (const char* ph = env_.get("IE_PIPELINE_HEAD")) pipeline_head_ = std::max(0, std::atoi(ph));
@@ -484,6 +491,7 @@
         BuildInstance(*pi, shapes);
         check(hipStreamSynchronize(stream_), "hipStreamSynchronize");
         if (autotune_) Autotune(*pi, pi->plan.steps.size(), allow_tune || tune_on_demand_);
+        else PairTransitions(nullptr, *pi);
         if (use_graph_ && !(precision_ == Precision::F8 && !w_->f8_ready)) {
             pi->captured_gen = w_->f8_gen.load();
             Capture(*pi, 0, pi->plan.steps.size(), &pi->graph_exec);
@@ -836,28 +844,34 @@
     if (const char* e = env_.get("IE_TUNE_HOT"); allow_search && !(e && std::atoi(e) != 0))
         if (hipMalloc(&ctx.scrub, TuneContext::kScrubBytes) != hipSuccess) { ctx.scrub = nullptr; (void)hipGetLastError(); }
     for (size_t si = 0; si < nsteps && si < pi.plan.steps.size(); ++si) TuneStep(ctx, pi, pi.plan.steps[si]);
+    if (nsteps >= pi.plan.steps.size()) PairTransitions(&ctx, pi);
     if (ctx.searched) SaveTuneCache();
 }
 
 float DeviceModel::TimeTrial(TuneContext& ctx, const PlanInstance& pi, const Step& trial) {
+    const float best = TimeLaunches(ctx, [&] { LaunchStep(pi, trial, stream_); });
+    if (ctx.log)
+        std::fprintf(stderr, "[ie-tune] M=%lld N=%lld K=%lld algo=%d tile=%d splitk=%d: %.4f ms\n", static_cast<long long>(trial.out.n * trial.out.h * trial.out.w),
+                     static_cast<long long>(trial.out.c), static_cast<long long>(trial.kh * trial.kw * trial.in.c), int(trial.algo), trial.tile, trial.splitk, best);
+    return best;
+}
+
+float DeviceModel::TimeLaunches(TuneContext& ctx, const std::function<void()>& launch) {
     auto timed = [&](int launches) {
         check(hipEventRecord(ctx.e0, stream_), "hipEventRecord");
-        for (int r = 0; r < launches; ++r) LaunchStep(pi, trial, stream_);
+        for (int r = 0; r < launches; ++r) launch();
         check(hipEventRecord(ctx.e1, stream_), "hipEventRecord");
         check(hipEventSynchronize(ctx.e1), "hipEventSynchronize");
         float ms = 0;
         check(hipEventElapsedTime(&ms, ctx.e0, ctx.e1), "hipEventElapsedTime");
         return ms;
     };
-    LaunchStep(pi, trial, stream_);
+    launch();
     float best = 1e30f;
     for (int rep = 0; rep < (ctx.scrub ? 3 : 2); ++rep) {
         if (ctx.scrub) check(hipMemsetAsync(ctx.scrub, 0, TuneContext::kScrubBytes, stream_), "hipMemsetAsync(scrub)");
         best = std::min(best, timed(ctx.scrub ? 1 : 3));
     }
-    if (ctx.log)
-        std::fprintf(stderr, "[ie-tune] M=%lld N=%lld K=%lld algo=%d tile=%d splitk=%d: %.4f ms\n", static_cast<long long>(trial.out.n * trial.out.h * trial.out.w),
-                     static_cast<long long>(trial.out.c), static_cast<long long>(trial.kh * trial.kw * trial.in.c), int(trial.algo), trial.tile, trial.splitk, best);
     return best;
 }
 
@@ -1651,11 +1665,248 @@
     return "?";
 }
 
+
+namespace {
+
+bool same_view(const View& a, const View& b) {
+    return a.buf == b.buf && a.n == b.n && a.c == b.c && a.h == b.h && a.w == b.w && a.c_off == b.c_off && a.pitch == b.pitch && a.nchw == b.nchw && a.f16 == b.f16 &&
+           a.f8 == b.f8;
+}
+bool views_overlap(const View& a, const View& b) {
+    return a.buf == b.buf && (a.nchw || b.nchw || (a.c_off < b.c_off + b.c && b.c_off < a.c_off + a.c));
+}
+bool view_kills(const View& w, const View& v) {
+    if (w.buf != v.buf) return false;
+    if (w.nchw || v.nchw || w.pitch != v.pitch || w.n != v.n || w.h != v.h || w.w != v.w) return true;
+    return w.c_off <= v.c_off && w.c_off + w.c >= v.c_off + v.c;
+}
+void step_views(const Step& s, std::vector<const View*>& reads, std::vector<const View*>& writes) {
+    reads.push_back(&s.in);
+    if (s.has_in2) reads.push_back(&s.in2);
+    writes.push_back(&s.out);
+    for (const Step& q : s.parts) step_views(q, reads, writes);
+}
+const char* plain_1x1(const Step& c) {
+    if (c.kind != StepKind::Conv) return "is not a conv";
+    if (!c.parts.empty() || IsGroupConv(c.algo) || c.group != 1 || c.algo == ConvAlgo::Stem) return "is a fused or grouped conv step";
+    if (c.kh != 1 || c.kw != 1 || c.sh != 1 || c.sw != 1 || c.pt || c.pl || c.pb || c.pr || c.dh != 1 || c.dw != 1) return "is not a 1x1 / stride-1 conv";
+    if (c.has_in2) return "has a residual";
+    if (c.act.kind != ActKind::None || c.lo != -__builtin_huge_valf() || c.hi != __builtin_huge_valf()) return "has an activation other than ReLU";
+    if (c.in.nchw || c.out.nchw || c.in.f16 || c.out.f16 || c.in.f8 || c.out.f8) return "is not fp32 NHWC";
+    return nullptr;
+}
+
+}
+
+std::vector<PairedLaunch> FindPairedLaunches(const Plan& plan) {
+    std::vector<PairedLaunch> found;
+    if (plan.precision != Precision::F32) return found;
+    const std::vector<Step>& st = plan.steps;
+    for (size_t i = 0; i + 1 < st.size(); ++i) {
+        const Step& pl = st[i];
+        const Step& cv = st[i + 1];
+        if (pl.kind != StepKind::Pool || cv.kind != StepKind::Conv || cv.in.buf != pl.out.buf) continue;
+        PairedLaunch c;
+        c.steps = {int(i), int(i + 1)};
+        auto miss = [&](const std::string& why) { c.reason = why; found.push_back(c); };
+        if (pl.pool_max) { miss("the pool is a max pool"); continue; }
+        if (pl.kh != 2 || pl.kw != 2 || pl.sh != 2 || pl.sw != 2) {
+            miss("the pool is " + std::to_string(pl.kh) + "x" + std::to_string(pl.kw) + " / stride " + std::to_string(pl.sh) + ", not 2x2 / stride 2");
+            continue;
+        }
+        if (pl.pt || pl.pl || pl.pb || pl.pr) { miss("the pool has padding"); continue; }
+        if (pl.in.nchw || pl.out.nchw || pl.in.f16 || pl.out.f16 || pl.in.f8 || pl.out.f8) { miss("the pool is not fp32 NHWC"); continue; }
+        if (pl.in.h != 2 * pl.out.h || pl.in.w != 2 * pl.out.w) { miss("the pool's windows do not tile its input"); continue; }
+        if (pl.act.kind != ActKind::None || pl.pre_act.kind != ActKind::None) { miss("the pool has an activation other than ReLU"); continue; }
+        if (const char* why = plain_1x1(cv)) { miss(std::string("the conv ") + why); continue; }
+        if (cv.pre_scale_off >= 0) { miss("the conv has a prologue of its own"); continue; }
+        if (!same_view(cv.in, pl.out)) { miss("the conv reads another view than the pool writes"); continue; }
+        bool other = false, dead = false;
+        for (size_t j = i + 2; j < st.size() && !other && !dead; ++j) {
+            std::vector<const View*> reads, writes;
+            step_views(st[j], reads, writes);
+            for (const View* r : reads) other = other || views_overlap(*r, pl.out);
+            for (const View* w : writes) dead = dead || view_kills(*w, pl.out);
+        }
+        if (other) { miss("a later step also reads the pooled tensor"); continue; }
+        if (!dead) {
+            bool is_out = false;
+            for (const IoDesc& o : plan.outputs) is_out = is_out || views_overlap(o.view, pl.out);
+            if (is_out) { miss("the pooled tensor is a graph output"); continue; }
+        }
+        if (cv.out.buf == pl.in.buf) { miss("the conv's output shares the pool input's buffer"); continue; }
+        for (int t = 0; t < kNumConvPooledTiles; ++t)
+            if (ConvPooledShapeOk(t, false, cv.in.c, cv.out.c, 0)) c.tiles.push_back(t);
+        if (c.tiles.empty()) { miss("no tile takes " + std::to_string(cv.in.c) + " -> " + std::to_string(cv.out.c) + " channels"); continue; }
+        c.pairable = true;
+        if (i + 2 < st.size()) {
+            const Step& en = st[i + 2];
+            std::string why;
+            if (const char* w = plain_1x1(en)) why = std::string("the entry step ") + w;
+            else if (en.pre_scale_off < 0) why = "the entry conv has no prologue";
+            else if (!same_view(en.in, cv.out)) why = "the entry conv reads another view than the conv writes";
+            else if (en.out.c != 128) why = "the entry conv has " + std::to_string(en.out.c) + " output channels, not 128";
+            else if (en.out.buf == pl.in.buf || en.out.buf == cv.out.buf) why = "the entry conv's output shares a buffer the launch still reads";
+            else {
+                for (int t = 0; t < kNumConvPooledTiles; ++t)
+                    if (ConvPooledShapeOk(t, true, cv.in.c, cv.out.c, en.out.c)) c.chain_tiles.push_back(t);
+                if (c.chain_tiles.empty()) why = "no chain tile holds " + std::to_string(cv.out.c) + " channels";
+            }
+            if (why.empty()) {
+                c.chainable = true;
+                c.steps.push_back(int(i + 2));
+            } else {
+                c.reason = "chain: " + why;
+            }
+        } else {
+            c.reason = "chain: no step behind the conv";
+        }
+        found.push_back(c);
+    }
+    return found;
+}
+
+std::string PairedLaunchesToJson(const std::vector<PairedLaunch>& v) {
+    std::ostringstream o;
+    auto list = [&](const std::vector<int>& l) {
+        o << "[";
+        for (size_t k = 0; k < l.size(); ++k) o << (k ? "," : "") << l[k];
+        o << "]";
+    };
+    o << "[";
+    for (size_t i = 0; i < v.size(); ++i) {
+        const PairedLaunch& c = v[i];
+        o << (i ? "," : "") << "{\"steps\":";
+        list(c.steps);
+        o << ",\"kind\":" << (!c.pairable ? "null" : (c.chainable ? "\"pool_conv_chain\"" : "\"pool_conv\"")) << ",\"tiles\":";
+        list(c.tiles);
+        o << ",\"chain_tiles\":";
+        list(c.chain_tiles);
+        o << ",\"reason\":\"" << c.reason << "\"}";
+    }
+    o << "]";
+    return o.str();
+}
+
+bool DeviceModel::MakePooledArgs(const PlanInstance& pi, size_t i, int count, bool chain, ConvArgs* a, PooledArgs* p) const {
+    const std::vector<Step>& st = pi.plan.steps;
+    if (i + size_t(count) > st.size() || count < (chain ? 3 : 2)) return false;
+    const float* wb = w_->d_weights;
+    auto wp = [&](int64_t off) -> const float* { return off >= 0 ? wb + off : nullptr; };
+    const Step& pl = st[i];
+    *a = MakeConvArgs(pi, st[i + 1]);
+    *p = PooledArgs();
+    p->pin = make_arg(pi, pl.in);
+    p->pool_scale = wp(pl.pre_scale_off);
+    p->pool_shift = wp(pl.pre_shift_off);
+    p->pool_relu = pl.pre_relu;
+    if (chain) {
+        const Step& en = st[i + 2];
+        p->out2 = make_arg(pi, en.out);
+        p->wfrag2 = w_->d_weights_frag && en.w_off >= 0 ? w_->d_weights_frag + en.w_off : nullptr;
+        p->bias2 = wp(en.bias_off);
+        p->scale2 = wp(en.pre_scale_off);
+        p->shift2 = wp(en.pre_shift_off);
+        p->pre_relu2 = en.pre_relu;
+        p->relu2 = en.relu;
+    }
+    return true;
+}
+
+int DeviceModel::PairedCount(const PlanInstance& pi, size_t i, size_t last, ConvArgs* a, PooledArgs* p, LaunchRole* role) const {
+    if (i >= pi.roles.size()) return 1;
+    const LaunchRole& r = pi.roles[i];
+    if (r.count <= 1 || i + size_t(r.count) > last) return 1;
+    if (!MakePooledArgs(pi, i, r.count, r.chain, a, p) || !ConvPooledEligible(*a, *p, r.tile, r.chain)) return 1;
+    *role = r;
+    return r.count;
+}
+
+void DeviceModel::PairTransitions(TuneContext* ctx, PlanInstance& pi) {
+    pi.roles.clear();
+    const int mode = pool_conv_mode_;
+    if (mode == 0 || precision_ != Precision::F32 || pi.batch_off != 0) return;
+    if (mode < 0 && (!autotune_ || ctx == nullptr)) return;
+    const std::vector<Step>& st = pi.plan.steps;
+    std::vector<LaunchRole> roles(st.size());
+    bool any = false;
+    for (const PairedLaunch& c : FindPairedLaunches(pi.plan)) {
+        if (!c.pairable) continue;
+        const size_t i = size_t(c.steps[0]);
+        ConvArgs a;
+        PooledArgs p;
+        auto can = [&](int t, bool chain) {
+            return t >= 0 && t < kNumConvPooledTiles && (!chain || c.chainable) && MakePooledArgs(pi, i, chain ? 3 : 2, chain, &a, &p) && ConvPooledEligible(a, p, t, chain);
+        };
+        int tile = -1;
+        bool chain = false;
+        if (mode > 0) {
+            if (pool_conv_tile_ >= 0) {
+                if (mode == 2 && can(pool_conv_tile_, true)) { tile = pool_conv_tile_; chain = true; }
+                else if (can(pool_conv_tile_, false)) tile = pool_conv_tile_;
+            } else {
+                for (int t = 0; mode == 2 && tile < 0 && t < kNumConvPooledTiles; ++t) if (can(t, true)) { tile = t; chain = true; }
+                for (int t = 0; tile < 0 && t < kNumConvPooledTiles; ++t) if (can(t, false)) tile = t;
+            }
+        } else {
+            const Step& pl = st[i];
+            const Step& cv = st[i + 1];
+            const size_t span = c.chainable ? 3 : 2;
+            const std::vector<int64_t> key = {cv.out.n * cv.out.h * cv.out.w, cv.out.c, cv.in.c, pl.in.h, pl.in.w, pl.in.pitch, cv.out.pitch, kPoolConvTuneCode,
+                                              pl.pre_scale_off >= 0, cv.bias_off >= 0, span == 3 ? st[i + 2].out.pitch : 0};
+            std::pair<int, int> hit{-1, 0};
+            int code = -1;
+            if (ctx->lookup(key, &hit)) {
+                if (pool_conv_tune_code(hit.first)) code = hit.first - kPoolConvTuneCode;
+            } else if (ctx->allow_search) {
+                auto alone = [&](size_t from) { for (size_t j = from; j < i + span; ++j) LaunchStep(pi, st[j], stream_); };
+                float best = TimeLaunches(*ctx, [&] { alone(i); });
+                code = 0;
+                auto consider = [&](int t, bool ch) {
+                    if (!can(t, ch)) return;
+                    const ConvArgs ta = a;
+                    const PooledArgs tp = p;
+                    const float ms = TimeLaunches(*ctx, [&] {
+                        check(LaunchConvPooled(ta, tp, t, ch, stream_), "conv1x1_pooled");
+                        if (!ch) alone(i + 2);
+                    });
+                    if (ctx->log) std::fprintf(stderr, "[ie-tune] transition at step %zu: pooled tile %d%s %.4f ms (split %.4f ms)\n", i, t, ch ? " chain" : "", ms, best);
+                    if (ms < best) { best = ms; code = 1 + (ch ? kNumConvPooledTiles : 0) + t; }
+                };
+                for (int t = 0; t < kNumConvPooledTiles; ++t) consider(t, false);
+                for (int t = 0; t < kNumConvPooledTiles; ++t) consider(t, true);
+                ctx->store(key, kPoolConvTuneCode + code, 1);
+            }
+            if (code >= 1) {
+                const bool ch = code > kNumConvPooledTiles;
+                const int t = code - 1 - (ch ? kNumConvPooledTiles : 0);
+                if (can(t, ch)) { tile = t; chain = ch; }
+            }
+        }
+        if (tile < 0) continue;
+        roles[i].count = chain ? 3 : 2;
+        roles[i].tile = tile;
+        roles[i].chain = chain;
+        roles[i + 1].count = 0;
+        if (chain) roles[i + 2].count = 0;
+        any = true;
+    }
+    if (any) pi.roles = std::move(roles);
+}
+
 void DeviceModel::RunSteps(PlanInstance& pi, size_t first, size_t last, std::vector<hipEvent_t>* events) {
     size_t k = 0;
     if (events) check(hipEventRecord((*events)[k++], stream_), "hipEventRecord");
+    ConvArgs pa;
+    PooledArgs pp;
+    LaunchRole role;
     for (size_t i = first; i < last && i < pi.plan.steps.size(); ++i) {
-        LaunchStep(pi, pi.plan.steps[i], stream_);
+        if (const int n = PairedCount(pi, i, std::min(last, pi.plan.steps.size()), &pa, &pp, &role); n > 1) {
+            check(LaunchConvPooled(pa, pp, role.tile, role.chain, stream_), "conv1x1_pooled");
+            i += size_t(n - 1);
+        } else {
+            LaunchStep(pi, pi.plan.steps[i], stream_);
+        }
         if (events) check(hipEventRecord((*events)[k++], stream_), "hipEventRecord");
     }
 }
@@ -1702,30 +1953,45 @@
     std::vector<hipEvent_t> ev(ns + 1);
     for (auto& e : ev) check(hipEventCreate(&e), "hipEventCreate");
     std::vector<StepTiming> out(ns);
-    for (size_t i = 0; i < ns; ++i) {
-        out[i].name = pi.plan.steps[i].name;
-        Step handed;
-        out[i].kernel = kernel_label(LaunchedStep(pi, pi.plan.steps[i], handed));
-        out[i].flops = pi.plan.steps[i].flops;
-        out[i].bytes = pi.plan.steps[i].bytes;
+    std::vector<std::pair<size_t, int>> groups;
+    for (size_t i = 0; i < ns;) {
+        ConvArgs pa;
+        PooledArgs pp;
+        LaunchRole role;
+        const int n = PairedCount(pi, i, ns, &pa, &pp, &role);
+        groups.emplace_back(i, n);
+        for (size_t j = i; j < i + size_t(n); ++j) {
+            out[j].name = pi.plan.steps[j].name;
+            Step handed;
+            out[j].kernel = n > 1 ? "conv1x1_pooled_kernel<f32,t" + std::to_string(role.tile) + (role.chain ? ",chain>" : ">")
+                                  : kernel_label(LaunchedStep(pi, pi.plan.steps[j], handed));
+            out[j].flops = pi.plan.steps[j].flops;
+            out[j].bytes = pi.plan.steps[j].bytes;
+        }
+        i += size_t(n);
     }
     try {
         RunSteps(pi, 0, ns, nullptr);
         check(hipStreamSynchronize(stream_), "hipStreamSynchronize");
-        std::vector<std::vector<float>> samples(ns);
+        const size_t ng = groups.size();
+        std::vector<std::vector<float>> samples(ng);
         for (int it = 0; it < iters; ++it) {
             RunSteps(pi, 0, ns, &ev);
             check(hipStreamSynchronize(stream_), "hipStreamSynchronize");
-            for (size_t i = 0; i < ns; ++i) {
+            for (size_t i = 0; i < ng; ++i) {
                 float ms = 0;
                 check(hipEventElapsedTime(&ms, ev[i], ev[i + 1]), "hipEventElapsedTime");
                 samples[i].push_back(ms);
             }
         }
-        for (size_t i = 0; i < ns; ++i) {
-            std::sort(samples[i].begin(), samples[i].end());
-            const size_t n = samples[i].size();
-            out[i].ms = n == 0 ? 0.0 : (n % 2 ? samples[i][n / 2] : 0.5 * (samples[i][n / 2 - 1] + samples[i][n / 2]));
+        for (size_t g = 0; g < ng; ++g) {
+            std::sort(samples[g].begin(), samples[g].end());
+            const size_t n = samples[g].size();
+            const double ms = n == 0 ? 0.0 : (n % 2 ? samples[g][n / 2] : 0.5 * (samples[g][n / 2 - 1] + samples[g][n / 2]));
+            auto bound = [&](size_t j) { return std::max({out[j].bytes / 8e12, out[j].flops / 157.3e12, 1e-12}); };
+            double sum = 0;
+            for (size_t j = groups[g].first; j < groups[g].first + size_t(groups[g].second); ++j) sum += bound(j);
+            for (size_t j = groups[g].first; j < groups[g].first + size_t(groups[g].second); ++j) out[j].ms = ms * bound(j) / sum;
         }
     } catch (...) {
         for (auto& e : ev) (void)hipEventDestroy(e);
diff --git a/gpu-ai-inference-server_amd/csrc/executor.h b/gpu-ai-inference-server_amd/csrc/executor.h
--- a/gpu-ai-inference-server_amd/csrc/executor.h
+++ b/gpu-ai-inference-server_amd/csrc/executor.h
@@ -2,6 +2,7 @@
 #include <hip/hip_runtime.h>
 
 #include <atomic>
+#include <functional>
 #include <map>
 #include <memory>
 #include <mutex>
@@ -57,8 +58,24 @@
     ~DeviceWeights();
 };
 
+struct PairedLaunch {
+    std::vector<int> steps;
+    bool pairable = false, chainable = false;
+    std::vector<int> tiles, chain_tiles;
+    std::string reason;
+};
+std::vector<PairedLaunch> FindPairedLaunches(const Plan& plan);
+std::string PairedLaunchesToJson(const std::vector<PairedLaunch>& v);
+
+struct LaunchRole {
+    int count = 1;
+    int tile = 0;
+    bool chain = false;
+};
+
 struct PlanInstance {
     Plan plan;
+    std::vector<LaunchRole> roles;
     std::vector<float*> buffers;
     std::vector<char> owned;
     float* workspace = nullptr;
@@ -132,6 +149,10 @@
     struct TuneContext;
     void TuneStep(TuneContext& ctx, const PlanInstance& pi, Step& s);
     float TimeTrial(TuneContext& ctx, const PlanInstance& pi, const Step& trial);
+    float TimeLaunches(TuneContext& ctx, const std::function<void()>& launch);
+    void PairTransitions(TuneContext* ctx, PlanInstance& pi);
+    int PairedCount(const PlanInstance& pi, size_t i, size_t last, ConvArgs* a, PooledArgs* p, LaunchRole* role) const;
+    bool MakePooledArgs(const PlanInstance& pi, size_t i, int count, bool chain, ConvArgs* a, PooledArgs* p) const;
     void SaveTuneCache();
     void EnsurePipeline(PlanInstance& pi, bool allow_tune);
     void AllocInstance(PlanInstance& pi);
@@ -165,6 +186,8 @@
     bool tune_on_demand_ = false;
     int pipeline_chunks_ = 2;
     int pipeline_head_ = -1;
+    int pool_conv_mode_ = -1;
+    int pool_conv_tile_ = -1;
     bool two_pass_splitk_ = true;
     std::map<std::vector<int64_t>, std::unique_ptr<PlanInstance>> plans_;
     std::vector<std::vector<int64_t>> lru_;
diff --git a/gpu-ai-inference-server_amd/csrc/kernels.h b/gpu-ai-inference-server_amd/csrc/kernels.h
--- a/gpu-ai-inference-server_amd/csrc/kernels.h
+++ b/gpu-ai-inference-server_amd/csrc/kernels.h
@@ -274,6 +274,28 @@
 bool ConvDirectEligible(const ConvArgs& a, int tile);
 hipError_t LaunchConvDirect(const ConvArgs& a, int tile, hipStream_t stream);
 hipError_t InitKernelsDirect();
+struct PooledConsts {
+    unsigned mg20_ow = 0, mg20_oh = 0;
+    unsigned mg32_ohw = 0, mg32_ow = 0;
+};
+struct PooledArgs {
+    TensorArg pin;
+    const float* pool_scale = nullptr;
+    const float* pool_shift = nullptr;
+    int pool_relu = 0;
+    TensorArg out2;
+    const float* wfrag2 = nullptr;
+    const float* bias2 = nullptr;
+    const float* scale2 = nullptr;
+    const float* shift2 = nullptr;
+    int pre_relu2 = 0, relu2 = 0;
+    PooledConsts k;
+};
+constexpr int kNumConvPooledTiles = 8;
+bool ConvPooledShapeOk(int tile, bool chain, int64_t k, int64_t cout, int64_t cout2);
+bool ConvPooledEligible(const ConvArgs& a, const PooledArgs& p, int tile, bool chain);
+hipError_t LaunchConvPooled(const ConvArgs& a, const PooledArgs& p, int tile, bool chain, hipStream_t stream);
+hipError_t InitKernelsTrans();
 int ResidentPerCu(const void* kernel, int block, size_t lds);
 
 bool ConvStemEligible(const ConvArgs& a);
diff --git a/gpu-ai-inference-server_amd/csrc/kernels_trans.hip b/gpu-ai-inference-server_amd/csrc/kernels_trans.hip
--- /dev/null
+++ b/gpu-ai-inference-server_amd/csrc/kernels_trans.hip
@@ -0,0 +1,420 @@
+#include <hip/hip_runtime.h>
+
+#include <algorithm>
+#include <cstdlib>
+#include <type_traits>
+
+#include "env.h"
+#include "kernels.h"
+
+namespace ie {
+
+typedef float f32x4 __attribute__((ext_vector_type(4)));
+typedef unsigned u32x4 __attribute__((ext_vector_type(4)));
+
+namespace {
+
+__device__ __forceinline__ unsigned udiv_uniform(unsigned n, unsigned d, unsigned mg) {
+    unsigned q = __umulhi(n, mg);
+    if (n - q * d >= d) ++q;
+    return q;
+}
+
+__device__ __forceinline__ unsigned mul24(unsigned v, unsigned s) {
+    unsigned r;
+    asm("v_mul_u32_u24 %0, %1, %2" : "=v"(r) : "s"(s), "v"(v));
+    return r;
+}
+
+template <int TNW, int PB, int D>
+struct AsLoop {
+    u32x4 ring[D][TNW];
+    int c_l = 0;
+    __device__ __forceinline__ void issue(const __amdgpu_buffer_rsrc_t rs_w, unsigned wlane, int nb, int CH, int slot) {
+        const int c = c_l < CH ? c_l : CH - 1;
+#pragma unroll
+        for (int j = 0; j < TNW; ++j) ring[slot][j] = __builtin_amdgcn_raw_buffer_load_b128(rs_w, wlane, ((nb + j) * CH + c) * 1024, 0);
+        ++c_l;
+    }
+    __device__ __forceinline__ void run(const __amdgpu_buffer_rsrc_t rs_w, unsigned wlane, int nb, int CH, const float* sA, int P, int r, int gk, f32x4 (&acc)[PB][TNW]) {
+        const float* abase[PB];
+#pragma unroll
+        for (int pb = 0; pb < PB; ++pb) abase[pb] = sA + (mul24(r, P) + pb * 16 * P + gk * 4);
+        f32x4 avn[PB];
+#pragma unroll
+        for (int pb = 0; pb < PB; ++pb) avn[pb] = *reinterpret_cast<const f32x4*>(abase[pb]);
+        auto compute = [&](int slot) {
+            f32x4 av[PB];
+#pragma unroll
+            for (int pb = 0; pb < PB; ++pb) av[pb] = avn[pb];
+#pragma unroll
+            for (int pb = 0; pb < PB; ++pb) avn[pb] = *reinterpret_cast<const f32x4*>(abase[pb] + (slot + 1) * 16);
+#pragma unroll
+            for (int e = 0; e < 4; ++e)
+#pragma unroll
+                for (int j = 0; j < TNW; ++j)
+#pragma unroll
+                    for (int pb = 0; pb < PB; ++pb)
+                        acc[pb][j] = __builtin_amdgcn_mfma_f32_16x16x4f32(__builtin_bit_cast(f32x4, ring[slot][j])[e], av[pb][e], acc[pb][j], 0, 0, 0);
+            __builtin_amdgcn_sched_group_barrier(0x100, PB, 0);
+            __builtin_amdgcn_sched_group_barrier(0x008, 4 * PB * TNW, 0);
+        };
+        const int full = CH / D, rem = CH - full * D;
+        for (int it = 0; it < full; ++it) {
+#pragma unroll
+            for (int s = 0; s < D; ++s) {
+                compute(s);
+                issue(rs_w, wlane, nb, CH, s);
+            }
+#pragma unroll
+            for (int pb = 0; pb < PB; ++pb) abase[pb] += D * 16;
+        }
+#pragma unroll
+        for (int s = 0; s < D; ++s)
+            if (s < rem) compute(s);
+    }
+};
+
+}
+
+template <int WAVES, int TNW, int PB, bool PRE, bool CHAIN>
+__global__ __launch_bounds__(64 * WAVES) void conv1x1_pooled_kernel(const ConvArgs a, const PooledArgs p) {
+    constexpr int NT = 64 * WAVES, D = PB == 1 ? 16 : 8, BNW = 16 * TNW, BN = BNW * WAVES;
+    extern __shared__ __attribute__((aligned(16))) unsigned char smem_trans[];
+    float* const sA = reinterpret_cast<float*>(smem_trans);
+
+    const int tid = threadIdx.x;
+    const int wave = __builtin_amdgcn_readfirstlane(tid >> 6);
+    const int pad = (a.debug >> 8) & 0xff;
+    const int K = a.in.c, P = K + pad, CH = K >> 4, Cout = a.out.c;
+    const int M = a.out.n * a.out.h * a.out.w;
+    const int m0 = blockIdx.x * (16 * PB), n0 = blockIdx.y * BN + wave * BNW;
+    const int ipitch = int(p.pin.sw), opitch = int(a.out.sw);
+
+    const __amdgpu_buffer_rsrc_t rs_w = __builtin_amdgcn_make_buffer_rsrc(const_cast<float*>(a.wfrag), 0, Cout * K * 4, 0x00020000);
+    const int nb = n0 >> 4;
+    AsLoop<TNW, PB, D> loop;
+    unsigned wlane = unsigned(tid & 63) * 16u;
+    constexpr int DLATE = D / 4;
+#pragma unroll
+    for (int s = 0; s < D - DLATE; ++s) loop.issue(rs_w, wlane, nb, CH, s);
+
+    {
+        constexpr int R = 16 * PB;
+        static_assert(R * 64 >= NT, "the widest column block (64 columns) must not span more rows than the tile has");
+        const int cs = a.debug >> 16, CT = 1 << cs;
+        const int rstep = NT >> cs, npass = R / rstep;
+        const int col = tid & (CT - 1), row0 = tid >> cs;
+        const unsigned IH = unsigned(p.pin.h), IW = unsigned(p.pin.w), OH = unsigned(a.out.h), OW = unsigned(a.out.w);
+        const int in_px = p.pin.n * p.pin.h * p.pin.w;
+        const __amdgpu_buffer_rsrc_t rs_in = __builtin_amdgcn_make_buffer_rsrc(p.pin.p, 0, ((in_px - 1) * ipitch + K) * 4, 0x00020000);
+        const __amdgpu_buffer_rsrc_t rs_sc = __builtin_amdgcn_make_buffer_rsrc(const_cast<float*>(p.pool_scale), 0, PRE ? K * 4 : 0, 0x00020000);
+        const __amdgpu_buffer_rsrc_t rs_sf = __builtin_amdgcn_make_buffer_rsrc(const_cast<float*>(p.pool_shift), 0, PRE ? K * 4 : 0, 0x00020000);
+        const unsigned ohw = OH * OW;
+        const unsigned b0 = udiv_uniform(unsigned(m0), ohw, p.k.mg32_ohw), rem0 = unsigned(m0) - b0 * ohw;
+        const unsigned oy0 = udiv_uniform(rem0, OW, p.k.mg32_ow), ox0 = rem0 - oy0 * OW;
+        const unsigned pitch4 = unsigned(ipitch) * 4u;
+        const int tap_x = int(pitch4), tap_y = int(IW * pitch4);
+        const unsigned c16 = unsigned(col) * 16u;
+        auto window = [&](unsigned row) {
+            const unsigned n = ox0 + row;
+            const unsigned q = mul24(n, p.k.mg20_ow) >> 20;
+            const unsigned ox = n - mul24(q, OW);
+            const unsigned y = oy0 + q;
+            const unsigned q2 = mul24(y, p.k.mg20_oh) >> 20;
+            const unsigned oy = y - mul24(q2, OH);
+            const unsigned ipx = mul24(mul24(b0 + q2, IH) + 2u * oy, IW) + 2u * ox;
+            return mul24(ipx, pitch4);
+        };
+        unsigned row = unsigned(row0);
+        unsigned cb = c16;
+        unsigned char* l = smem_trans + (mul24(row0, P) * 4u + c16);
+        const int lstep = rstep * P * 4, lnext = CT * 16 - npass * lstep;
+        const f32x4 zero = {0.f, 0.f, 0.f, 0.f};
+        auto stage = [&](auto relu_) {
+            constexpr bool RELU = decltype(relu_)::value;
+            for (int left = K * 4; left > 0; left -= CT * 16) {
+                if (c16 < unsigned(left)) {
+                    f32x4 sc = zero, sf = zero;
+                    if constexpr (PRE) {
+                        sc = __builtin_bit_cast(f32x4, __builtin_amdgcn_raw_buffer_load_b128(rs_sc, c16, K * 4 - left, 0));
+                        sf = __builtin_bit_cast(f32x4, __builtin_amdgcn_raw_buffer_load_b128(rs_sf, c16, K * 4 - left, 0));
+                    }
+                    auto group = [&](auto n_) {
+                        constexpr int N = decltype(n_)::value;
+                        asm volatile("; ie-mark pooled-stage n=%0 relu=%1" ::"n"(N), "n"(int(RELU)));
+                        u32x4 v[N][4];
+#pragma unroll
+                        for (int u = 0; u < N; ++u) {
+                            const unsigned g = window(row) + cb;
+                            v[u][0] = __builtin_amdgcn_raw_buffer_load_b128(rs_in, g, 0, 0);
+                            v[u][1] = __builtin_amdgcn_raw_buffer_load_b128(rs_in, g, tap_x, 0);
+                            v[u][2] = __builtin_amdgcn_raw_buffer_load_b128(rs_in, g, tap_y, 0);
+                            v[u][3] = __builtin_amdgcn_raw_buffer_load_b128(rs_in, g, tap_y + tap_x, 0);
+                            row += unsigned(rstep);
+                        }
+#pragma unroll
+                        for (int u = 0; u < N; ++u) {
+                            f32x4 acc = zero;
+#pragma unroll
+                            for (int t = 0; t < 4; ++t) {
+                                f32x4 x = __builtin_bit_cast(f32x4, v[u][t]);
+                                if constexpr (PRE) x = __builtin_elementwise_fma(x, sc, sf);
+                                if constexpr (PRE && RELU) x = __builtin_elementwise_max(x, zero);
+                                acc = acc + x;
+                            }
+                            *reinterpret_cast<f32x4*>(l) = acc * 0.25f;
+                            l += lstep;
+                        }
+                        asm volatile("; ie-mark pooled-stage-end n=%0 relu=%1" ::"n"(N), "n"(int(RELU)));
+                    };
+                    if (npass >= 2) {
+                        for (int p0 = 0; p0 < npass; p0 += 2) group(std::integral_constant<int, 2>{});
+                    } else {
+                        group(std::integral_constant<int, 1>{});
+                    }
+                    row = unsigned(row0);
+                    cb += unsigned(CT) * 16u;
+                    l += lnext;
+                }
+            }
+        };
+        if (PRE && __builtin_amdgcn_readfirstlane(p.pool_relu) != 0) stage(std::true_type{});
+        else stage(std::false_type{});
+    }
+#pragma unroll
+    for (int s = D - DLATE; s < D; ++s) loop.issue(rs_w, wlane, nb, CH, s);
+    __syncthreads();
+
+    int lane = __builtin_amdgcn_mbcnt_hi(~0u, __builtin_amdgcn_mbcnt_lo(~0u, 0u));
+    asm volatile("" : "+v"(lane));
+    const int r = lane & 15, gk = lane >> 4;
+    wlane = unsigned(lane) * 16u;
+    f32x4 acc[PB][TNW];
+#pragma unroll
+    for (int pb = 0; pb < PB; ++pb)
+#pragma unroll
+        for (int j = 0; j < TNW; ++j) acc[pb][j] = f32x4{0.f, 0.f, 0.f, 0.f};
+    loop.run(rs_w, wlane, nb, CH, sA, P, r, gk, acc);
+
+    const f32x4 zero = {0.f, 0.f, 0.f, 0.f};
+    {
+        const __amdgpu_buffer_rsrc_t rs_out =
+            __builtin_amdgcn_make_buffer_rsrc(a.out.p, 0, int((int64_t(M - 1) * opitch + Cout) * 4), 0x00020000);
+        const __amdgpu_buffer_rsrc_t rs_b = __builtin_amdgcn_make_buffer_rsrc(const_cast<float*>(a.bias), 0, a.bias != nullptr ? Cout * 4 : 0, 0x00020000);
+        const unsigned o0 = (unsigned(m0) * unsigned(opitch) + mul24(r, opitch) + 4 * gk) * 4u;
+        const unsigned ostep = unsigned(opitch) * 64u;
+        auto finish = [&](auto relu_, auto bias_) {
+            constexpr bool RELU = decltype(relu_)::value, BIAS = decltype(bias_)::value;
+            asm volatile("; ie-mark pooled-finish relu=%0 bias=%1" ::"n"(int(RELU)), "n"(int(BIAS)));
+#pragma unroll
+            for (int j = 0; j < TNW; ++j) {
+                f32x4 bq = zero;
+                if constexpr (BIAS) bq = __builtin_bit_cast(f32x4, __builtin_amdgcn_raw_buffer_load_b128(rs_b, unsigned(gk) * 16u, (n0 + j * 16) * 4, 0));
+#pragma unroll
+                for (int pb = 0; pb < PB; ++pb) {
+                    f32x4 v = acc[pb][j];
+                    if constexpr (BIAS) v += bq;
+                    if constexpr (RELU) v = __builtin_elementwise_max(v, zero);
+                    acc[pb][j] = v;
+                    __builtin_amdgcn_raw_buffer_store_b128(__builtin_bit_cast(u32x4, v), rs_out, o0 + pb * ostep, (n0 + j * 16) * 4, 0);
+                }
+            }
+        };
+        switch (__builtin_amdgcn_readfirstlane((a.relu ? 1 : 0) | (a.bias != nullptr ? 2 : 0))) {
+            case 0: finish(std::false_type{}, std::false_type{}); break;
+            case 1: finish(std::true_type{}, std::false_type{}); break;
+            case 2: finish(std::false_type{}, std::true_type{}); break;
+            default: finish(std::true_type{}, std::true_type{}); break;
+        }
+    }
+
+    if constexpr (CHAIN) {
+        const int K2 = Cout, P2 = K2 + pad, CH2 = K2 >> 4, Cout2 = p.out2.c;
+        const __amdgpu_buffer_rsrc_t rs_w2 = __builtin_amdgcn_make_buffer_rsrc(const_cast<float*>(p.wfrag2), 0, Cout2 * K2 * 4, 0x00020000);
+        AsLoop<1, PB, D> loop2;
+#pragma unroll
+        for (int s = 0; s < D; ++s) loop2.issue(rs_w2, wlane, wave, CH2, s);
+        __syncthreads();
+        {
+            const __amdgpu_buffer_rsrc_t rs_s2 = __builtin_amdgcn_make_buffer_rsrc(const_cast<float*>(p.scale2), 0, K2 * 4, 0x00020000);
+            const __amdgpu_buffer_rsrc_t rs_t2 = __builtin_amdgcn_make_buffer_rsrc(const_cast<float*>(p.shift2), 0, K2 * 4, 0x00020000);
+            const bool relu2 = __builtin_amdgcn_readfirstlane(p.pre_relu2) != 0;
+#pragma unroll
+            for (int j = 0; j < TNW; ++j) {
+                const f32x4 s2 = __builtin_bit_cast(f32x4, __builtin_amdgcn_raw_buffer_load_b128(rs_s2, unsigned(gk) * 16u, (n0 + j * 16) * 4, 0));
+                const f32x4 t2 = __builtin_bit_cast(f32x4, __builtin_amdgcn_raw_buffer_load_b128(rs_t2, unsigned(gk) * 16u, (n0 + j * 16) * 4, 0));
+#pragma unroll
+                for (int pb = 0; pb < PB; ++pb) {
+                    f32x4 x = __builtin_elementwise_fma(acc[pb][j], s2, t2);
+                    if (relu2) x = __builtin_elementwise_max(x, zero);
+                    *reinterpret_cast<f32x4*>(sA + (mul24(r, P2) + pb * 16 * P2 + n0 + j * 16 + 4 * gk)) = x;
+                }
+            }
+        }
+        __syncthreads();
+        f32x4 acc2[PB][1];
+#pragma unroll
+        for (int pb = 0; pb < PB; ++pb) acc2[pb][0] = zero;
+        loop2.run(rs_w2, wlane, wave, CH2, sA, P2, r, gk, acc2);
+        const int opitch2 = int(p.out2.sw);
+        const __amdgpu_buffer_rsrc_t rs_out2 =
+            __builtin_amdgcn_make_buffer_rsrc(p.out2.p, 0, int((int64_t(M - 1) * opitch2 + Cout2) * 4), 0x00020000);
+        const __amdgpu_buffer_rsrc_t rs_b2 = __builtin_amdgcn_make_buffer_rsrc(const_cast<float*>(p.bias2), 0, p.bias2 != nullptr ? Cout2 * 4 : 0, 0x00020000);
+        const unsigned o2 = (unsigned(m0) * unsigned(opitch2) + mul24(r, opitch2) + 4 * gk) * 4u;
+        f32x4 bq = zero;
+        if (p.bias2 != nullptr) bq = __builtin_bit_cast(f32x4, __builtin_amdgcn_raw_buffer_load_b128(rs_b2, unsigned(gk) * 16u, wave * 64, 0));
+        const bool relu_out2 = __builtin_amdgcn_readfirstlane(p.relu2) != 0;
+#pragma unroll
+        for (int pb = 0; pb < PB; ++pb) {
+            f32x4 v = acc2[pb][0];
+            if (p.bias2 != nullptr) v += bq;
+            if (relu_out2) v = __builtin_elementwise_max(v, zero);
+            __builtin_amdgcn_raw_buffer_store_b128(__builtin_bit_cast(u32x4, v), rs_out2, o2 + pb * unsigned(opitch2) * 64u, wave * 64, 0);
+        }
+    }
+}
+
+namespace {
+
+struct TransTile { int waves, tnw, pb; bool chain; };
+constexpr TransTile kTransTiles[kNumConvPooledTiles] = {{8, 1, 2, true}, {4, 1, 2, false}, {8, 2, 2, true}, {4, 1, 1, false}, {2, 2, 1, false}, {1, 1, 2, false},
+                                                        {8, 1, 1, true}, {8, 2, 1, true}};
+
+unsigned mg20(unsigned d) { return ((1u << 20) + d - 1) / d; }
+unsigned mg32(unsigned d) { return d == 1 ? 0xffffffffu : unsigned((uint64_t(1) << 32) / d); }
+
+bool aligned16(const void* q) { return (reinterpret_cast<uintptr_t>(q) & 15) == 0; }
+
+int col_shift(int K, int threads, int rows) {
+    const int c4n = K / 4;
+    int best = 6;
+    long best_key = -1;
+    for (int s = 6; s >= 4 && (threads >> s) <= rows; --s) {
+        const int ct = 1 << s, blocks = (c4n + ct - 1) / ct, npass = rows * ct / threads;
+        const long key = (long(blocks * ((npass + 1) / 2)) << 24) + blocks * npass;
+        if (best_key < 0 || key < best_key) best = s, best_key = key;
+    }
+    return best;
+}
+
+size_t lds_bytes(const ConvArgs& a, const TransTile& t, bool chain, int pad) {
+    const size_t rows = size_t(16 * t.pb);
+    const size_t first = rows * (a.in.c + pad) * 4 + 64, second = chain ? rows * (a.out.c + pad) * 4 + 64 : 0;
+    return std::max(first, second);
+}
+
+template <int T>
+hipError_t launch_t(const ConvArgs& a_in, const PooledArgs& p_in, bool chain, hipStream_t stream) {
+    constexpr TransTile t = kTransTiles[T];
+    ConvArgs a = a_in;
+    PooledArgs p = p_in;
+    const int pad = Knobs().as_pad;
+    a.debug = (pad << 8) | (col_shift(a.in.c, 64 * t.waves, 16 * t.pb) << 16);
+    p.k.mg20_ow = mg20(unsigned(a.out.w));
+    p.k.mg20_oh = mg20(unsigned(a.out.h));
+    p.k.mg32_ohw = mg32(unsigned(a.out.h) * unsigned(a.out.w));
+    p.k.mg32_ow = mg32(unsigned(a.out.w));
+    const int64_t M = int64_t(a.out.n) * a.out.h * a.out.w;
+    const dim3 grid(unsigned((M + 16 * t.pb - 1) / (16 * t.pb)), unsigned(a.out.c / (16 * t.tnw * t.waves)));
+    const size_t lds = lds_bytes(a, t, chain, pad);
+    if (lds > size_t(160) * 1024) return hipErrorInvalidValue;
+    const bool pre = p.pool_scale != nullptr;
+    if constexpr (t.chain) {
+        if (chain) {
+            if (pre) conv1x1_pooled_kernel<t.waves, t.tnw, t.pb, true, true><<<grid, dim3(64 * t.waves), lds, stream>>>(a, p);
+            else conv1x1_pooled_kernel<t.waves, t.tnw, t.pb, false, true><<<grid, dim3(64 * t.waves), lds, stream>>>(a, p);
+            return hipGetLastError();
+        }
+    }
+    if (chain) return hipErrorInvalidValue;
+    if (pre) conv1x1_pooled_kernel<t.waves, t.tnw, t.pb, true, false><<<grid, dim3(64 * t.waves), lds, stream>>>(a, p);
+    else conv1x1_pooled_kernel<t.waves, t.tnw, t.pb, false, false><<<grid, dim3(64 * t.waves), lds, stream>>>(a, p);
+    return hipGetLastError();
+}
+
+template <int T>
+hipError_t init_t() {
+    constexpr TransTile t = kTransTiles[T];
+    hipError_t e = hipFuncSetAttribute(reinterpret_cast<const void*>(&conv1x1_pooled_kernel<t.waves, t.tnw, t.pb, true, false>), hipFuncAttributeMaxDynamicSharedMemorySize, 160 * 1024);
+    if (e != hipSuccess) return e;
+    e = hipFuncSetAttribute(reinterpret_cast<const void*>(&conv1x1_pooled_kernel<t.waves, t.tnw, t.pb, false, false>), hipFuncAttributeMaxDynamicSharedMemorySize, 160 * 1024);
+    if constexpr (t.chain) {
+        if (e != hipSuccess) return e;
+        e = hipFuncSetAttribute(reinterpret_cast<const void*>(&conv1x1_pooled_kernel<t.waves, t.tnw, t.pb, true, true>), hipFuncAttributeMaxDynamicSharedMemorySize, 160 * 1024);
+        if (e != hipSuccess) return e;
+        e = hipFuncSetAttribute(reinterpret_cast<const void*>(&conv1x1_pooled_kernel<t.waves, t.tnw, t.pb, false, true>), hipFuncAttributeMaxDynamicSharedMemorySize, 160 * 1024);
+    }
+    return e;
+}
+
+}
+
+bool ConvPooledShapeOk(int tile, bool chain, int64_t k, int64_t cout, int64_t cout2) {
+    if (tile < 0 || tile >= kNumConvPooledTiles) return false;
+    const TransTile t = kTransTiles[tile];
+    const int64_t bn = 16 * t.tnw * t.waves;
+    if (k <= 0 || (k % 16) || cout <= 0 || (cout % bn)) return false;
+    if (size_t(16 * t.pb) * (k + 8) * 4 + 64 > size_t(160) * 1024) return false;
+    if (!chain) return true;
+    return t.chain && cout == bn && cout2 == 16 * t.waves;
+}
+
+bool ConvPooledEligible(const ConvArgs& a, const PooledArgs& p, int tile, bool chain) {
+    if (!ConvPooledShapeOk(tile, chain, a.in.c, a.out.c, chain ? p.out2.c : 0)) return false;
+    const TransTile t = kTransTiles[tile];
+    if (a.in.f16 || a.out.f16 || a.in.f8 || a.out.f8 || a.wfrag == nullptr || a.res.p != nullptr || a.pre_scale != nullptr) return false;
+    if (a.kh != 1 || a.kw != 1 || a.sh != 1 || a.sw != 1 || a.pt != 0 || a.pl != 0) return false;
+    if (a.out.h != a.in.h || a.out.w != a.in.w || a.out.n != a.in.n) return false;
+    if (a.out.sc != 1 || (a.out.sw % 4) || a.out.sh != a.out.w * a.out.sw || a.out.sn != a.out.h * a.out.sh || !aligned16(a.out.p)) return false;
+    if (!aligned16(a.wfrag) || (a.bias && !aligned16(a.bias))) return false;
+    const TensorArg& x = p.pin;
+    if (x.p == nullptr || x.f16 || x.f8 || x.sc != 1 || x.c != a.in.c || x.n != a.in.n || x.h != 2 * a.in.h || x.w != 2 * a.in.w) return false;
+    if ((x.sw % 4) || x.sw < x.c || x.sh != x.w * x.sw || x.sn != x.h * x.sh || !aligned16(x.p)) return false;
+    if ((p.pool_scale == nullptr) != (p.pool_shift == nullptr)) return false;
+    if (p.pool_scale && (!aligned16(p.pool_scale) || !aligned16(p.pool_shift))) return false;
+    const int64_t M = int64_t(a.out.n) * a.out.h * a.out.w;
+    if (M <= 0 || M > (int64_t(1) << 22) || a.out.h > 512 || a.out.w > 512) return false;
+    const int64_t px_span = (int64_t(x.n) + 33) * x.h * x.w;
+    if (px_span >= (int64_t(1) << 24) || x.sw * 4 >= (int64_t(1) << 24) || px_span * x.sw * 4 >= (int64_t(1) << 32)) return false;
+    if (int64_t(x.n) * x.h * x.w * x.sw * 4 >= (int64_t(1) << 31)) return false;
+    if (a.out.sw >= (int64_t(1) << 22) || (M + 32) * a.out.sw * 4 >= (int64_t(1) << 31) || int64_t(a.out.c) * a.in.c * 4 >= (int64_t(1) << 31)) return false;
+    if (lds_bytes(a, t, chain, Knobs().as_pad) > size_t(160) * 1024) return false;
+    if (!chain) return true;
+    const TensorArg& o2 = p.out2;
+    if (p.wfrag2 == nullptr || !aligned16(p.wfrag2) || p.scale2 == nullptr || p.shift2 == nullptr || !aligned16(p.scale2) || !aligned16(p.shift2)) return false;
+    if (p.bias2 && !aligned16(p.bias2)) return false;
+    if (o2.p == nullptr || o2.f16 || o2.f8 || o2.sc != 1 || o2.n != a.out.n || o2.h != a.out.h || o2.w != a.out.w) return false;
+    if ((o2.sw % 4) || o2.sh != o2.w * o2.sw || o2.sn != o2.h * o2.sh || !aligned16(o2.p)) return false;
+    if (o2.sw >= (int64_t(1) << 22) || (M + 32) * o2.sw * 4 >= (int64_t(1) << 31)) return false;
+    return true;
+}
+
+hipError_t LaunchConvPooled(const ConvArgs& a, const PooledArgs& p, int tile, bool chain, hipStream_t stream) {
+    if (!ConvPooledEligible(a, p, tile, chain)) return hipErrorInvalidValue;
+    switch (tile) {
+        case 0: return launch_t<0>(a, p, chain, stream);
+        case 1: return launch_t<1>(a, p, chain, stream);
+        case 2: return launch_t<2>(a, p, chain, stream);
+        case 3: return launch_t<3>(a, p, chain, stream);
+        case 4: return launch_t<4>(a, p, chain, stream);
+        case 5: return launch_t<5>(a, p, chain, stream);
+        case 6: return launch_t<6>(a, p, chain, stream);
+        case 7: return launch_t<7>(a, p, chain, stream);
+        default: return hipErrorInvalidValue;
+    }
+}
+
+hipError_t InitKernelsTrans() {
+    hipError_t e;
+    if ((e = init_t<0>()) != hipSuccess) return e;
+    if ((e = init_t<1>()) != hipSuccess) return e;
+    if ((e = init_t<2>()) != hipSuccess) return e;
+    if ((e = init_t<3>()) != hipSuccess) return e;
+    if ((e = init_t<4>()) != hipSuccess) return e;
+    if ((e = init_t<5>()) != hipSuccess) return e;
+    if ((e = init_t<6>()) != hipSuccess) return e;
+    return init_t<7>();
+}
+
+}
```

After: 16550 images/sec, median of 6. +2.4%, better.
